# sml2004/CUDA-powered-mesh-handling-and-Iterative-solvers

Measured on AMD Instinct MI355X. Metric: CG iterations/sec + DOFs/sec (assembly+solve), 10M P1-tet Poisson, 1/2/4/8 MI355X, higher is better.
Workload: dtype f64; 1 GPU; 10,110,954-tet P1 poisson Kuhn cube n=119, Jacobi-PCG fixed iterations; tets=10110954, nodes=1728000, dofs=1728000, nnz_blocks=25575838, parallelism=single GPU

## Files before the change

### cuda-powered-mesh-handling-and-iterative-solvers_amd/_capi.py

```python
from __future__ import annotations

import atexit
import ctypes
import functools
import inspect
import os
import threading

import torch

PKG_DIR = os.path.dirname(os.path.abspath(__file__))
LIB_PATH = os.environ.get("FEM355_LIB", os.path.join(PKG_DIR, "lib", "libfem355.so"))

FEM_OK, FEM_EBADTYPE, FEM_ESINGULAR, FEM_EHIP, FEM_ERCCL, FEM_EARG, FEM_ESTATE = range(7)
(PCG_RUNNING, PCG_CONVERGED, PCG_MAXITER, PCG_BREAKDOWN, PCG_ALPHA_NAN, PCG_BETA_NAN, PCG_SYNC_TIMEOUT,
 PCG_BAD_WINDOW) = range(8)
MODE_CG_STABLE, MODE_PCG, MODE_CG_CONSTRAINED = 0, 1, 2
TUNE_UPD1 = 1024
TUNE_U2_HOLD, TUNE_U2_SMALL = 2048, 4096
TUNE_MF_GATHER = 8192
TUNE_PK_GV = 16384
TUNE_DEFAULT = 1 | 2 | 4 | 8 | 128 | TUNE_UPD1
KIND_ELASTIC, KIND_POISSON, KIND_MASS = 0, 1, 2
ISO_SUM, ISO_STACK, ISO_VOLUME, ISO_MASS = 0, 1, 2, 3
MASS_SELL, MASS_DIAG = 0, 1
MODAL_OUT_GM, MODAL_OUT_NORMS, MODAL_OUT_LEN = 576, 1152, 1168

_P = ctypes.c_void_p
_I = ctypes.c_int
_L = ctypes.c_int64
_D = ctypes.c_double

SIGNATURES = {
    "fem_last_error": (ctypes.c_char_p, []),
    "fem_version": (_I, []),
    "fem_tet4_ke": (_I, [_P, _P, _L, _D, _D, _I, _P, _P, _P]),
    "fem_tet4_geom": (_I, [_P, _P, _L, _P, _P, _P, _P, _P]),
    "fem_iso_ke": (_I, [_P, _P, _L, _I, _D, _D, _P, _P, _I, _I, _P, _P]),
    "fem_iso_geom": (_I, [_P, _P, _L, _I, _P, _P, _P, _P, _P]),
    "fem_ke_sym_stride": (_I, [_I]),
    "fem_iso_ke_sym": (_I, [_P, _P, _L, _I, _D, _D, _P, _P, _I, _I, _P, _P]),
    "fem_assemble_from_ke_sym": (_I, [_P, _P, _I, _P, _P, _L, _P, _P, _P, _I, _I, _I, _P, _P]),
    "fem_assemble_from_ke_mass_sl": (_I, [_P, _P, _P, _I, _P, _P, _L, _P, _P, _P, _I, _I, _P, _P, _P]),
    "fem_iso_mass": (_I, [_P, _P, _L, _I, _D, _P, _P, _P, _I, _P, _P]),
    "fem_iso_mass_scalar": (_I, [_P, _P, _L, _I, _D, _P, _P, _P, _I, _P, _P]),
    "fem_pcg_scalars": (_I, [_P, ctypes.POINTER(_D)]),
    "fem_scan_work_len": (_L, [_L]),
    "fem_incidence_work_bytes": (_L, [_L, _L]),
    "fem_incidence": (_I, [_P, _L, _I, _L, _P, _P, _P, _P]),
    "fem_incidence_checked": (_I, [_P, _L, _I, _L, _P, _P, _P, _P, _P]),
    "fem_rcm_work_len": (_L, [_L]),
    "fem_rcm": (_I, [_P, _P, _L, _P, _P, _P, _P, _P]),
    "fem_graph_count": (_I, [_P, _I, _P, _P, _L, _P, _P, _P]),
    "fem_graph_fill": (_I, [_P, _I, _P, _P, _L, _P, _P, _P, _P]),
    "fem_graph_tmp_len": (_L, [_L]),
    "fem_graph_count2": (_I, [_P, _I, _P, _P, _L, _P, _P, _P, _P]),
    "fem_graph_fill2": (_I, [_P, _I, _P, _P, _L, _P, _P, _P, _P, _P]),
    "fem_graph_sell_fill": (_I, [_P, _I, _P, _P, _L, _P, _P, _P, _P, _P, _P, _P, _P, _P, _P]),
    "fem_graph_sell_fill_sl": (_I, [_P, _I, _P, _P, _L, _P, _P, _P, _P, _P, _P, _P, _I, _P, _P, _P, _P, _P]),
    "fem_scan_i32": (_I, [_P, _L, _P, _P, _P]),
    "fem_scan_i64": (_I, [_P, _L, _P, _P, _P]),
    "fem_sell_widths": (_I, [_P, _L, _P, _P]),
    "fem_graph_sizes": (_I, [_P, _P, _P, _L, _P, _P, _P, _P]),
    "fem_sell_fill": (_I, [_P, _P, _L, _P, _P, _P, _P]),
    "fem_sell_csr2sell": (_I, [_P, _L, _P, _P, _P]),
    "fem_assemble_from_ke": (_I, [_P, _P, _I, _I, _P, _P, _L, _P, _P, _P, _P, _P, _P]),
    "fem_assemble_from_ke_ex": (_I, [_P, _P, _I, _I, _P, _P, _L, _P, _P, _P, _P, _L, _L, _I, _P, _P]),
    "fem_assemble_from_ke_ex2": (_I, [_P, _P, _I, _I, _P, _P, _L, _P, _P, _P, _P, _L, _L, _I, _I, _P, _P]),
    "fem_assemble_tet4": (_I, [_P, _P, _D, _D, _I, _P, _P, _L, _P, _P, _P, _P, _P, _P, _P]),
    "fem_assemble_tet4_ex": (_I, [_P, _P, _D, _D, _I, _P, _P, _L, _P, _P, _P, _P, _I, _P, _P, _P]),
    "fem_assemble_tet4_ex2": (_I, [_P, _P, _D, _D, _I, _P, _P, _L, _P, _P, _P, _P, _I, _I, _P, _P, _P]),
    "fem_sell_to_csr_vals": (_I, [_P, _I, _P, _L, _P, _P, _P, _P]),
    "fem_jacobi": (_I, [_P, _I, _P, _P, _P, _P, _L, _P, _P, _P]),
    "fem_ebe_apply": (_I, [_P, _P, _I, _I, _P, _P, _L, _P, _P, _P]),
    "fem_ebe_diag": (_I, [_P, _P, _I, _I, _P, _P, _L, _I, _P, _P]),
    "fem_invert_diag": (_I, [_P, _L, _P, _P]),
    "fem_tet4_stress": (_I, [_P, _P, _L, _P, _D, _D, _P, _P, _P, _P]),
    "fem_iso_stress": (_I, [_P, _P, _L, _I, _P, _D, _D, _P, _P, _I, _I, _P, _P, _P]),
    "fem_voigt_to_tensor": (_I, [_P, _L, _P, _P]),
    "fem_von_mises": (_I, [_P, _L, _P, _P]),
    "fem_node_average": (_I, [_P, _I, _P, _P, _L, _P, _P]),
    "fem_face_forces": (_I, [_P, _P, _L, _I, _P, _P]),
    "fem_shared_face_sum": (_I, [_P, _P, _I, _L, _P, _P]),
    "fem_topo_create": (_I, [_P, _L, _I, _P, _I, _I, _L, _P, ctypes.POINTER(_P)]),
    "fem_topo_counts": (_I, [_P, ctypes.POINTER(_L), ctypes.POINTER(_L), ctypes.POINTER(_L)]),
    "fem_topo_pairs": (_I, [_P, _P]),
    "fem_topo_unique": (_I, [_P, _P]),
    "fem_topo_boundary": (_I, [_P, _P, _I, _P, _P, _P, _P, _P, ctypes.POINTER(_L)]),
    "fem_topo_destroy": (None, [_P]),
    "fem_sub_elements": (_I, [_P, _L, _I, _P, _I, _I, _P, _P]),
    "fem_element_face_normals": (_I, [_P, _P, _L, _I, _P, _P, _P, _P, _I, _D, _I, _I, _P, _P]),
    "fem_surface_normals": (_I, [_P, _P, _P, _L, _I, _I, _P, _P]),
    "fem_solid_ke": (_I, [_I, _P, _P, _L, _D, _D, _P, _P, _I, _I, _P, _P]),
    "fem_csr_pattern": (_I, [_P, _L, _I, _I, _L, _P, _P, _P, ctypes.POINTER(_L), _P]),
    "fem_csr_fill": (_I, [_P, _P, _L, _I, _I, _L, _P, _P, _P, _P]),
    "fem_spmv_csr": (_I, [_P, _P, _P, _P, _P, _L, _P]),
    "fem_pcg_csr": (_I, [_P, _P, _P, _L, _P, _P, _P, _P, _D, _I, _D, _I, ctypes.POINTER(_I), ctypes.POINTER(_I), _P,
                         _P]),
    "fem_vtk_read": (_I, [ctypes.c_char_p, ctypes.POINTER(_P)]),
    "fem_vtk_sizes": (_I, [_P, ctypes.POINTER(_L), ctypes.POINTER(_L), ctypes.POINTER(_L), ctypes.POINTER(_L)]),
    "fem_vtk_copy": (_I, [_P, _P, _P, _P]),
    "fem_vtk_free": (None, [_P]),
    "fem_spmv": (_I, [_L, _I, _P, _P, _P, _P, _P, _P]),
    "fem_sell_delta16": (_I, [_P, _L, _P, _P, _P, _P]),
    "fem_spmv16": (_I, [_L, _I, _P, _P, _P, _P, _P, _P]),
    "fem_pcg_set_cols16": (_I, [_P, _P]),
    "fem_pcg_set_tuning": (_I, [_P, _I]),
    "fem_stream_copy": (_I, [_P, _P, _L, _I, _P]),
    "fem_stream_read": (_I, [_P, _P, _L, _I, _P]),
    "fem_pcg_create": (_I, [_L, _I, _P, _P, _P, _P, _P, _P, _I, _D, _D, _P, _L, _P, ctypes.POINTER(_P)]),
    "fem_pcg_start": (_I, [_P]),
    "fem_pcg_iterate": (_I, [_P, _I]),
    "fem_pcg_poll": (_I, [_P, ctypes.POINTER(_I), ctypes.POINTER(_I), ctypes.POINTER(_D)]),
    "fem_pcg_sync_site": (_I, [_P, ctypes.POINTER(_I)]),
    "fem_pcg_debug_window": (_I, [_P, _I, _I, _I]),
    "fem_pcg_solve": (_I, [_P, _I, _I, ctypes.POINTER(_I), ctypes.POINTER(_I), ctypes.POINTER(_D)]),
    "fem_pcg_use_graph": (_I, [_P, _I]),
    "fem_pcg_set_schedule": (_I, [_P, _I]),
    "fem_pcg_set_entries": (_I, [_P, _L]),
    "fem_pcg_get_schedule": (_I, [_P]),
    "fem_pcg_uniform_slices": (_I, [_P, _L, _L, _P, _P, _P]),
    "fem_pcg_persist_build": (_I, [_P, ctypes.POINTER(_I), ctypes.POINTER(_I), ctypes.POINTER(_I)]),
    "fem_pcg_pipelined": (_I, [_P, ctypes.POINTER(_I)]),
    "fem_sell_sl_pattern": (_I, [_L, _P, _P, _I, _P, _P, _P, _P, _P]),
    "fem_assemble_tet4_sl": (_I, [_P, _P, _D, _D, _I, _P, _P, _L, _P, _P, _P, _P, _P, _I, _I, _P, _P, _P]),
    "fem_assemble_from_ke_sl": (_I, [_P, _P, _I, _P, _P, _L, _P, _P, _P, _I, _I, _P, _P]),
    "fem_jacobi_sl": (_I, [_P, _I, _P, _P, _P, _P, _P, _L, _P, _P, _P]),
    "fem_spmv_sl": (_I, [_L, _I, _P, _P, _P, _P, _P, _P, _P, _P]),
    "fem_sell_sl_unpair": (_I, [_L, _I, _P, _P, _P, _P, _P, _P, _P, _P]),
    "fem_pcg_set_layout": (_I, [_P, _P, _P, _P, _P, _P, _I]),
    "fem_pcg_persist_profile": (_I, [_P, _I, _P, ctypes.POINTER(_I)]),
    "fem_pcg_set_constraints": (_I, [_P, _I, _L, _P, _P, _L, _P, _P, _L, _P, _P, _P, _P, _P]),
    "fem_enforce_constraints": (_I, [_P, _P, _L, _I, _L, _P, _P, _L, _P, _P, _L, _P, _P, _P, _P, _P, _P]),
    "fem_pcg_finish": (_I, [_P]),
    "fem_pcg_profile": (_I, [_P, _I, _I, ctypes.POINTER(_D), ctypes.POINTER(_I)]),
    "fem_pcg_destroy": (None, [_P]),
    "fem_pcg_release_cache": (_I, []),
    "fem_release_scratch": (_I, []),
    "fem_pcg_set_rows": (_I, [_P, _I, _I, _P, _I]),
    "fem_pcg_comm_block": (_I, [_P, ctypes.POINTER(_P), ctypes.POINTER(_L)]),
    "fem_pcg_col_window": (_I, [_P, ctypes.POINTER(_L), ctypes.POINTER(_L)]),
    "fem_pcg_set_peers": (_I, [_P, _P, _P, _P]),
    "fem_pcg_dist_debug": (_I, [_P, _I, _P, _L]),
    "fem_stream_create_cu": (_I, [_I, _I, ctypes.POINTER(_P)]),
    "fem_stream_destroy": (_I, [_P]),
    "fem_pcg_set_prof": (_I, [_P, _P]),
    "fem_ipc_handle": (_I, [_P, ctypes.c_char_p]),
    "fem_ipc_open": (_I, [ctypes.c_char_p, ctypes.POINTER(_P)]),
    "fem_ipc_close": (_I, [_P]),
    "fem_sell_diag": (_I, [_P, _I, _P, _P, _L, _P, _P]),
    "fem_jacobi_from_diag": (_I, [_P, _L, _P, _P, _P]),
    "fem_mf_create": (_I, [_P, _P, _L, _L, _I, _D, _D, ctypes.POINTER(_L), _P, ctypes.POINTER(_P)]),
    "fem_mf_destroy": (_I, [_P]),
    "fem_mf_apply": (_I, [_P, _P, _P, _P]),
    "fem_mf_diag": (_I, [_P, _P, _P]),
    "fem_mf_info": (_I, [_P, ctypes.POINTER(_L)]),
    "fem_mf_order": (_I, [_P, _P, _P, _P, _P, _P]),
    "fem_pcg_set_operator_mf": (_I, [_P, _P]),
    "fem_comm_unique_id": (_I, [ctypes.c_char_p]),
    "fem_comm_init": (_I, [_I, _I, ctypes.c_char_p, ctypes.POINTER(_P)]),
    "fem_comm_destroy": (_I, [_P]),
    "fem_allreduce_sum": (_I, [_P, _P, _L, _P]),
    "fem_halo_sum": (_I, [_P, _P, _I, _P, _L, _P, _L, _P, _P]),
    "fem_halo_pack": (_I, [_P, _I, _P, _L, _P, _P]),
    "fem_halo_unpack": (_I, [_P, _I, _P, _L, _P, _P]),
    "fem_pcg_set_dist": (_I, [_P, _I, _P, _L, _P, _P, _P]),
    "fem_pcg_set_dist_variant": (_I, [_P, _I]),
    "fem_pcg_set_p2p": (_I, [_P, _I, _I, _P, _P, _P, _P]),
    "fem_pcg_p2p_buffers": (_I, [_P, ctypes.POINTER(_P), ctypes.POINTER(_P), ctypes.POINTER(_L)]),
    "fem_p2p_deliver": (_I, [_P, _I, _P]),
    "fem_pcg_dist_phase": (_I, [_P, _I]),
    "fem_pcg_dist_buffer": (_I, [_P, _I, ctypes.POINTER(_P), ctypes.POINTER(_L)]),
    "fem_group_allreduce": (_I, [_P, _I, _L, _P]),
    "fem_spmm": (_I, [_L, _I, _I, _P, _P, _P, _P, _P, _P, _P]),
    "fem_mpcg_create": (_I, [_L, _I, _I, _I, _P, _P, _P, _P, _P, _P, _P, _I, ctypes.POINTER(_D), _D, _P, _L, _P,
                             ctypes.POINTER(_P)]),
    "fem_mpcg_solve": (_I, [_P, _I, _I, ctypes.POINTER(_I), ctypes.POINTER(_I), ctypes.POINTER(_D)]),
    "fem_mpcg_scalars": (_I, [_P, ctypes.POINTER(_D)]),
    "fem_mpcg_destroy": (None, [_P]),
    "fem_spmm_km": (_I, [_L, _I, _I, _P, _P, _P, _P, _P, _I, _P, _P, _P, _P]),
    "fem_modal_work_len": (_L, []),
    "fem_modal_gram": (_I, [_L, _I, _I, ctypes.POINTER(_P), _P, _P, _P]),
    "fem_modal_residual": (_I, [_L, _I, _P, _P, _P, _P, _P, _P, _P, _P]),
    "fem_modal_rotate": (_I, [_L, _I, _I, ctypes.POINTER(_P), _P, _P]),
    "fem_pcg_set_tol": (_I, [_P, _D]),
    "fem_sell_axpby_mass": (_I, [_L, _I, _I, _L, _P, _P, _P, _P, _P, _I, _D, _D, _P, _P]),
    "fem_newmark_rhs": (_I, [_L, _I, _I, _P, _P, _P, _P, _P, _I, _D, _P, _P, _P, _P]),
    "fem_newmark_update": (_I, [_L, ctypes.POINTER(_D), _I, _P, _P, _P, _P, _P, _P, _P]),
    "fem_transient_work_len": (_L, []),
    "fem_quadform_km": (_I, [_L, _I, _I, _P, _P, _P, _P, _P, _I, _P, _P, _P, _P]),
}

_lib = None
_lock = threading.Lock()


class FemError(RuntimeError):
    pass


def load_library(path: str = LIB_PATH):
    global _lib
    with _lock:
        if _lib is None:
            if not os.path.exists(path):
                raise FemError(f"fem355: HIP library not built: {path} (run `python -c 'import __graft_entry__ as g; g.build()'`)")
            lib = ctypes.CDLL(path)
            for name, (res, args) in SIGNATURES.items():
                fn = getattr(lib, name)
                fn.restype = res
                fn.argtypes = args
            _lib = lib
    return _lib


def lib():
    if not torch.cuda.is_available():
        raise FemError("fem355 requires a HIP (MI355X) device; none is visible. There is no CPU fallback.")
    return load_library()


def check(rc: int, what: str = ""):
    if rc == FEM_OK:
        return
    msg = (_lib.fem_last_error() or b"").decode(errors="replace") if _lib else ""
    if rc == FEM_EBADTYPE:
        raise ValueError(f"{what}: {msg}")
    if rc == FEM_ESINGULAR:
        raise ValueError("Singular matrix encountered while computing B matrix.")
    raise FemError(f"fem355 {what} failed (code {rc}): {msg}")


def ptr(t):
    if t is None:
        return None
    if not t.is_cuda:
        raise FemError(f"fem355: a {t.device} tensor was passed where device memory is required")
    return ctypes.c_void_p(t.data_ptr())


def stream(dev=None):
    return ctypes.c_void_p(torch.cuda.current_stream(dev).cuda_stream)


def compute_device(device=None) -> torch.device:
    if device is not None:
        d = torch.device(device)
        if d.type == "cuda":
            return d if d.index is not None else torch.device("cuda", torch.cuda.current_device())
    return torch.device("cuda", torch.cuda.current_device())


def device_scope(dev):
    d = torch.device(dev)
    if d.type != "cuda" or d.index is None or d.index == torch.cuda.current_device():
        return _NULL_SCOPE
    return torch.cuda.device(d)


class _NullScope:
    def __enter__(self):
        return self

    def __exit__(self, *exc):
        return False


_NULL_SCOPE = _NullScope()


def on_device(fn):
    sig = inspect.signature(fn)
    if "device" not in sig.parameters:
        return fn
# ... 41 lines not shown
```

### cuda-powered-mesh-handling-and-iterative-solvers_amd/csrc/pcg.hip

```cpp
#include <rccl/rccl.h>
#include <stddef.h>

#include <atomic>
#include <mutex>
#include <vector>

#include "sell_pair.hpp"
#include "sell_pair3.hpp"
#include "matfree.hpp"

namespace fem {

template <typename T, bool NT>
__device__ __forceinline__ T ld(const T* p) {
    if constexpr (NT) return __builtin_nontemporal_load(p);
    else return *p;
}

struct VecPlain {
    const double* x;
    __device__ __forceinline__ double operator()(int64_t i) const { return x[i]; }
};
struct VecFusedP {
    const double* r;
// ... 1562 lines not shown
    };
    auto spc = [&]() {
        for (int64_t t = t0; t < c.S; t += 256) {
            x[c.spc_dof[t]] = c.spc_val[t];
            if (r) r[c.spc_dof[t]] = 0.0;
        }
        __syncthreads();
    };
    if (c.order == 0) {
        rbe2();
        spc();
    } else {
        spc();
        rbe2();
        for (int64_t g = 0; g < c.G; ++g) {
            double v = 0.0;
            for (int64_t e = c.r3_ptr[g] + t0; e < c.r3_ptr[g + 1]; e += 256) v += c.r3_w[e] * x[c.r3_slave[e]];
            v = block_sum256(v, lds4);
            if (t0 == 0) x[c.r3_master[g]] = v / (c.r3_wsum[g] + 1e-30);
            __syncthreads();
        }
    }
}

enum { CON_GATHER = 0, CON_SCATTER = 1, CON_SPC = 2 };
template <int PH>
__global__ void __launch_bounds__(256) k_con_phase(double* __restrict__ x, double* __restrict__ r, Constraints c,
                                                   const PcgState* st, int always) {
    if (!always && !st->xupd) return;
    const int64_t m = PH == CON_SPC ? c.S : c.R;
    for (int64_t t = (int64_t)blockIdx.x * 256 + threadIdx.x; t < m; t += (int64_t)gridDim.x * 256) {
        if (PH == CON_GATHER) {
            c.tmp[t] = x[c.rbe2_master[t]];
        } else if (PH == CON_SCATTER) {
            x[c.rbe2_slave[t]] = c.tmp[t];
            if (r) r[c.rbe2_slave[t]] = 0.0;
        } else {
            x[c.spc_dof[t]] = c.spc_val[t];
            if (r) r[c.spc_dof[t]] = 0.0;
        }
    }
}

__global__ void k_check_range(const int64_t* __restrict__ v, int64_t m, int64_t lo, int64_t hi, int* __restrict__ bad) {
    for (int64_t i = (int64_t)blockIdx.x * blockDim.x + threadIdx.x; i < m; i += (int64_t)gridDim.x * blockDim.x)
        if (v[i] < lo || v[i] >= hi) atomicOr(bad, 1);
}

__global__ void k_check_ptr(const int64_t* __restrict__ ptr, int64_t g, int* __restrict__ bad) {
    for (int64_t i = (int64_t)blockIdx.x * blockDim.x + threadIdx.x; i < g; i += (int64_t)gridDim.x * blockDim.x)
        if (ptr[i + 1] < ptr[i] || (i == 0 && ptr[0] != 0)) atomicOr(bad, 1);
}

__global__ void __launch_bounds__(256) k_stream_copy(const double2* __restrict__ src, double2* __restrict__ dst,
                                                     int64_t n2) {
    for (int64_t i = (int64_t)blockIdx.x * 256 + threadIdx.x; i < n2; i += (int64_t)gridDim.x * 256) dst[i] = src[i];
}

__global__ void __launch_bounds__(256) k_stream_read(const double2* __restrict__ src, int64_t n2, double* __restrict__ out) {
    double acc = 0.0;
    for (int64_t i = (int64_t)blockIdx.x * 256 + threadIdx.x; i < n2; i += (int64_t)gridDim.x * 256) {
        const double2 v = src[i];
        acc += v.x + v.y;
    }
    if (acc == 12345.678) out[0] = acc;
}

__global__ void k_zero_fixed(int64_t n, double* __restrict__ x, const double* __restrict__ w) {
    for (int64_t i = (int64_t)blockIdx.x * blockDim.x + threadIdx.x; i < n; i += (int64_t)gridDim.x * blockDim.x)
        if (w[i] == 0.0) x[i] = 0.0;
}

}

using namespace fem;

struct fem_pcg {
    int64_t nrows, nslices, n;
    int bs;
    const int64_t* slice_ptr;
    const int32_t* cols;
    const double* vals;
    const double* b;
    double* x;
    const double* w;
    double* hist;
    int64_t hist_len;
    int mode;
    double tol, eps;
    hipStream_t stream;
    int fused;
    int deferred;
    int64_t launched;
    int64_t sell_ent;
    const int16_t* cols16;
    int has_con;
    int tune;
    int paired;
    double* pvals;
    int16_t* pcols16;
    int32_t* puoff;
    int16_t* pucol;
    int pext;
    const int32_t* pwin_ext;
    int pwin_G;
    Constraints con;
    double* r;
    double* p0;
    double* p1;
    double* q;
    RedBuf red;
    PcgState* st;
    PcgState* st_host;
    int grid_spmv, grid_vec;
    hipGraphExec_t graph;
    int graph_k;
    int max_iter;
    int dist;
    ncclComm_t comm;
    int64_t nI;
    const int32_t* imap;
    const int32_t* ipos;
    const uint8_t* own;
    double* hbuf;
    int cg1;
    double* cg1_s;
    double* cg1_u;
    double* cg1_send;
    double* cg1_recv;
    int p2p;
    int p2p_nranks;
    std::vector<int> peer_rank;
    std::vector<int64_t> peer_off, peer_cnt;
    int64_t p2p_total;
    const int32_t* p2p_csrc;
    const int32_t* p2p_ssrc;
    double* psend;
    double* precv;
    int c1f;
    int c1f_grid;
    int c1f_win_ok;
    int32_t* c1f_win;
    unsigned* c1f_flags;
    int persist_req;
    int persist_fit_only;
    int persist;
    int pk_grid;
    int pk_win_ok;
    int32_t* pk_win;
    double* pk_part;
    unsigned* pk_sync;
    int pk_ovf;
    double* pk_v;
    int pk_coop;
    int pk_gv;
    double* gv_buf;
    int64_t gv_cap;
    int gv_init_pending;
    int64_t pk_epochs;
    hipEvent_t pev[2];
    int pd;
    int pd_rank, pd_nranks, pd_grid_req;
    int64_t pd_split[PK_MAX_RANKS + 1];
    char* pd_block;
    int64_t pd_block_bytes, pd_off_flag, pd_off_red, pd_off_rflag;
    int64_t pd_off_m1;
    char* pd_peer[PK_MAX_RANKS];
    int pd_peers_ok;
    int32_t* pd_pub;
    int pd_init_pending;
    unsigned long long* pd_prof;
    int upd1;
    int u2_grid;
    unsigned* u2_sync;
    fem_mf* mf;
    double* mf_sl;
    int64_t mf_sl_cap;
    int mf_nogather;
    int mf_qfuse;
};

#define FEM_NCCL(call)                                                                         \
    do {                                                                                       \
        ncclResult_t _r = (call);                                                              \
        if (_r != ncclSuccess) {                                                               \
            ::fem::set_error("%s:%d %s -> %s", __FILE__, __LINE__, #call, ncclGetErrorString(_r)); \
            return FEM_ERCCL;                                                                  \
        }                                                                                      \
    } while (0)

static const int16_t* pcols(const fem_pcg* s) { return s->bs == 1 ? s->pcols16 : s->cols16; }

static double* st_red(fem_pcg* s, int k) {
    return reinterpret_cast<double*>(reinterpret_cast<char*>(s->st) + offsetof(PcgState, red)) + k;
}

template <int BS>
__global__ void __launch_bounds__(MF_BLOCK) k_pcg_mf_dot(MfOp op, const double* __restrict__ p,
                                                         double* __restrict__ slots, PcgState* __restrict__ st,
                                                         RedBuf red) {
    __shared__ MfLds<BS> L;
    __shared__ double lds4[MF_BLOCK / 64];
    __shared__ int flag;
    if (blockIdx.x == 0 && threadIdx.x == 0) st->xupd = 0;
    if (st->halt || st->iter >= st->max_iter) return;
    double dot = mf_walk<BS, MF_DOT>(op, p, slots, L);
    dot = block_sum<MF_BLOCK>(dot, lds4);
    double pq;
    if (reduce_grid<MF_BLOCK>(dot, red.part(RED_K1), red.cnt(RED_K1), &pq, lds4, &flag) && threadIdx.x == 0)
        finish_pq(st, pq);
}

template <int BS>
__global__ void __launch_bounds__(MF_BLOCK) k_cg1_mf_slots(MfOp op, const double* __restrict__ u,
                                                           double* __restrict__ slots, const PcgState* __restrict__ st,
                                                           int always, P2PArgs xp, const double* __restrict__ recv,
                                                           const double* __restrict__ send, int64_t off) {
    __shared__ MfLds<BS> L;
    if (!always) {
        const Cg1Step k = cg1_eval(st, cg1_scalar(recv, send, off, 0, xp), cg1_scalar(recv, send, off, 1, xp));
        if (!k.go) return;
    }
    (void)mf_walk<BS, MF_APPLY>(op, u, slots, L);
}

template <int BS>
__global__ void __launch_bounds__(MF_BLOCK) k_cg1_mf_slots_dot(MfOp op, const double* __restrict__ u,
                                                               double* __restrict__ slots, PcgState* __restrict__ st,
                                                               int always, P2PArgs xp, const double* __restrict__ recv,
                                                               const double* __restrict__ send, int64_t off,
                                                               RedBuf red) {
    __shared__ MfLds<BS> L;
    __shared__ double lds4[MF_BLOCK / 64];
    __shared__ int flag;
    if (!always) {
        const Cg1Step k = cg1_eval(st, cg1_scalar(recv, send, off, 0, xp), cg1_scalar(recv, send, off, 1, xp));
        if (!k.go) return;
    }
    double dot = mf_walk<BS, MF_DOT>(op, u, slots, L);
    dot = block_sum<MF_BLOCK>(dot, lds4);
    double d;
    if (reduce_grid<MF_BLOCK>(dot, red.part(RED_K1), red.cnt(RED_K1), &d, lds4, &flag) && threadIdx.x == 0)
        st->red[0] = d;
}

template <int BS>
__global__ void __launch_bounds__(PCG_BLOCK) k_cg1_mf_iface(MfOp op, const double* __restrict__ slots,
                                                            const int32_t* __restrict__ imap, int64_t nI,
                                                            double* __restrict__ send, int64_t off,
                                                            PcgState* __restrict__ st, RedBuf red, int always,
                                                            P2PArgs xp, const double* __restrict__ recv, double* hist,
                                                            int64_t hist_len) {
    __shared__ double lds4[4];
    __shared__ int flag;
    Cg1Step k{};
    if (!always) {
        k = cg1_eval(st, cg1_scalar(recv, send, off, 0, xp), cg1_scalar(recv, send, off, 1, xp));
        if (!k.go) {
            if (blockIdx.x == 0 && threadIdx.x == 0) cg1_commit(st, k, hist, hist_len);
            return;
        }
    }
    for (int64_t j = (int64_t)blockIdx.x * PCG_BLOCK + threadIdx.x; j < nI; j += (int64_t)gridDim.x * PCG_BLOCK) {
        const int32_t a = imap[j];
        if (a < 0) continue;
#pragma unroll
        for (int c = 0; c < BS; ++c) {
            const double o = mf_q_dof<BS>(op, slots, (int64_t)a * BS + c);
            if (xp.P) {
                for (int q = 0; q < xp.P; ++q) {
                    const int dst = xp.csrc[j * xp.P + q];
                    if (dst >= 0) xp.psend[dst + c] = o;
                }
            } else {
                send[j * BS + c] = o;
            }
        }
    }
    double unused;
    if (reduce_grid(0.0, red.part(RED_INIT), red.cnt(RED_INIT), &unused, lds4, &flag) && threadIdx.x == 0) {
        if (!always) cg1_commit(st, k, hist, hist_len);
        const double d = st->red[0];
        send[off] = st->red[1];
        send[off + 1] = d;
        for (int q = 0; q < xp.P; ++q) {
            const int dst = xp.ssrc[q];
            if (dst >= 0) {
                xp.psend[dst] = st->red[1];
                xp.psend[dst + 1] = d;
            }
        }
    }
}

template <int BS>
__global__ void __launch_bounds__(PCG_BLOCK) k_cg1_mf_gather(MfOp op, const double* __restrict__ slots,
                                                             const double* __restrict__ u, double* __restrict__ v,
                                                             const int32_t* __restrict__ ipos, double* __restrict__ send,
                                                             int64_t off, PcgState* __restrict__ st, RedBuf red,
                                                             int always, P2PArgs xp, const double* __restrict__ recv,
                                                             double* hist, int64_t hist_len) {
    __shared__ double lds4[4];
    __shared__ int flag;
    Cg1Step k{};
    if (!always) {
        k = cg1_eval(st, cg1_scalar(recv, send, off, 0, xp), cg1_scalar(recv, send, off, 1, xp));
// ... 804 lines not shown
    }
    FEM_LAUNCHED();
    return FEM_OK;
}

static int make_constraints(const char* fn, int64_t n, hipStream_t stream, int order, int64_t R,
                            const int64_t* rbe2_slave, const int64_t* rbe2_master, int64_t S, const int64_t* spc_dof,
                            const double* spc_val, int64_t G, const int64_t* r3_ptr, const int64_t* r3_master,
                            const double* r3_wsum, const int64_t* r3_slave, const double* r3_w, Constraints* c) {
    if (R < 0 || S < 0 || G < 0 || (R && (!rbe2_slave || !rbe2_master)) || (S && (!spc_dof || !spc_val)) ||
        (G && (!r3_ptr || !r3_master || !r3_wsum)) || (order != 0 && order != 1) || (order == 0 && G)) {
        set_error("%s: bad sizes / pointers / order", fn);
        return FEM_EARG;
    }
    int* bad = nullptr;
    FEM_HIP(::fem::malloc_async((void**)&bad, sizeof(int) * 2, stream));
    FEM_HIP(hipMemsetAsync(bad, 0, sizeof(int) * 2, stream));
    auto chk = [&](const int64_t* v, int64_t m) {
        if (m > 0)
            hipLaunchKernelGGL(k_check_range, dim3(stream_grid(m, 256)), dim3(256), 0, stream, v, m, (int64_t)0, n, bad);
    };
    chk(rbe2_slave, R);
    chk(rbe2_master, R);
    chk(spc_dof, S);
    chk(r3_master, G);
    int64_t E = 0;
    if (G) {
        hipLaunchKernelGGL(k_check_ptr, dim3(stream_grid(G, 256)), dim3(256), 0, stream, r3_ptr, G, bad + 1);
        FEM_HIP(hipMemcpyAsync(&E, r3_ptr + G, sizeof(int64_t), hipMemcpyDeviceToHost, stream));
    }
    int hbad[2] = {0, 0};
    FEM_HIP(hipMemcpyAsync(hbad, bad, sizeof(hbad), hipMemcpyDeviceToHost, stream));
    FEM_HIP(hipStreamSynchronize(stream));
    if (!hbad[1] && E > 0) {
        if (!r3_slave || !r3_w) hbad[1] = 1;
        else {
            chk(r3_slave, E);
            FEM_HIP(hipMemcpyAsync(hbad, bad, sizeof(int), hipMemcpyDeviceToHost, stream));
            FEM_HIP(hipStreamSynchronize(stream));
        }
    }
    FEM_HIP(hipFreeAsync(bad, stream));
    if (hbad[0] || hbad[1]) {
        set_error("%s: %s", fn, hbad[0] ? "a constraint dof is outside [0, n)" : "RBE3 group pointer is not a CSR offset array");
        return FEM_EARG;
    }
    *c = Constraints{};
    c->R = R;
    c->S = S;
    c->G = G;
    c->rbe2_slave = rbe2_slave;
    c->rbe2_master = rbe2_master;
    c->spc_dof = spc_dof;
    c->spc_val = spc_val;
    c->r3_ptr = r3_ptr;
    c->r3_master = r3_master;
    c->r3_wsum = r3_wsum;
    c->r3_slave = r3_slave;
    c->r3_w = r3_w;
    c->order = order;
    return FEM_OK;
}

int fem_pcg_set_constraints(fem_pcg* s, int order, int64_t R, const int64_t* rbe2_slave, const int64_t* rbe2_master,
                            int64_t S, const int64_t* spc_dof, const double* spc_val, int64_t G, const int64_t* r3_ptr,
                            const int64_t* r3_master, const double* r3_wsum, const int64_t* r3_slave,
                            const double* r3_w) {
    if (s->mode != FEM_MODE_CG_CONSTRAINED || s->dist || s->fused || s->deferred || s->graph || s->mf) {
        set_error("fem_pcg_set_constraints: needs a CG_CONSTRAINED, single-GPU, 3-kernel context without a graph "
                  "over an assembled matrix");
        return FEM_EARG;
    }
    Constraints c;
    const int rc = make_constraints("fem_pcg_set_constraints", s->n, s->stream, order, R, rbe2_slave, rbe2_master, S,
                                    spc_dof, spc_val, G, r3_ptr, r3_master, r3_wsum, r3_slave, r3_w, &c);
    if (rc != FEM_OK) return rc;
    if (s->con.tmp) (void)hipFree(s->con.tmp);
    s->con.tmp = nullptr;
    if (R > 0) FEM_HIP(hipMalloc(&c.tmp, sizeof(double) * (size_t)R));
    s->con = c;
    s->has_con = 1;
    return FEM_OK;
}

int fem_enforce_constraints(double* x, double* r, int64_t n, int order, int64_t R, const int64_t* rbe2_slave,
                            const int64_t* rbe2_master, int64_t S, const int64_t* spc_dof, const double* spc_val,
                            int64_t G, const int64_t* r3_ptr, const int64_t* r3_master, const double* r3_wsum,
                            const int64_t* r3_slave, const double* r3_w, fem_stream_t stream) {
    if (!x || n < 0) {
        set_error("fem_enforce_constraints: null x / negative n");
        return FEM_EARG;
    }
    const hipStream_t st = reinterpret_cast<hipStream_t>(stream);
    Constraints c;
    const int rc = make_constraints("fem_enforce_constraints", n, st, order, R, rbe2_slave, rbe2_master, S, spc_dof,
                                    spc_val, G, r3_ptr, r3_master, r3_wsum, r3_slave, r3_w, &c);
    if (rc != FEM_OK) return rc;
    if (R > 0) FEM_HIP(::fem::malloc_async((void**)&c.tmp, sizeof(double) * (size_t)R, st));
    const int lrc = launch_constraints(st, x, r, c, nullptr, 1);
    if (lrc != FEM_OK) return lrc;
    if (c.tmp) FEM_HIP(hipFreeAsync(c.tmp, st));
    return FEM_OK;
}

int fem_pcg_set_tuning(fem_pcg* s, int flags) {
    if (s->graph) {
        set_error("fem_pcg_set_tuning: drop the captured graph first");
        return FEM_EARG;
    }
    s->tune = flags;
    return FEM_OK;
}

int fem_pcg_set_cols16(fem_pcg* s, const int16_t* dcols) {
    if (s->graph) {
        set_error("fem_pcg_set_cols16: drop the captured graph first");
        return FEM_EARG;
    }
    s->cols16 = dcols;
    if (!dcols) s->paired = 0;
    return FEM_OK;
}

int fem_stream_copy(const double* src, double* dst, int64_t n, int grid, fem_stream_t stream) {
    if (grid <= 0) grid = 2048;
    hipLaunchKernelGGL(k_stream_copy, dim3(grid), dim3(256), 0, S(stream), (const double2*)src, (double2*)dst, n / 2);
    FEM_LAUNCHED();
    return FEM_OK;
}

int fem_stream_read(const double* src, double* out, int64_t n, int grid, fem_stream_t stream) {
    if (grid <= 0) grid = 4096;
    hipLaunchKernelGGL(k_stream_read, dim3(grid), dim3(256), 0, S(stream), (const double2*)src, n / 2, out);
    FEM_LAUNCHED();
    return FEM_OK;
}

int fem_pcg_create(int64_t nrows, int bs, const int64_t* slice_ptr, const int32_t* cols, const double* vals,
                   const double* b, double* x, const double* w, int mode, double tol, double eps, double* hist,
                   int64_t hist_len, fem_stream_t stream, fem_pcg** out) {
    if (bs != 1 && bs != 3) {
        set_error("fem_pcg_create: block size %d unsupported", bs);
        return FEM_EARG;
    }
    if (mode != FEM_MODE_CG_STABLE && mode != FEM_MODE_PCG && mode != FEM_MODE_CG_CONSTRAINED) {
        set_error("fem_pcg_create: unknown mode %d", mode);
        return FEM_EARG;
    }
    if (((uintptr_t)b | (uintptr_t)x | (uintptr_t)w) & 15) {
        set_error("fem_pcg_create: vectors must be 16-byte aligned");
        return FEM_EARG;
    }
    fem_pcg* s = new fem_pcg();
    s->tune = FEM_TUNE_REVERSE | FEM_TUNE_PAIR | FEM_TUNE_PK_SC1 | FEM_TUNE_PK_PACK | FEM_TUNE_PK_UNI | FEM_TUNE_UPD1;
    s->nrows = nrows;
    s->bs = bs;
    s->nslices = cdiv(nrows, 64);
    s->n = nrows * bs;
    s->sell_ent = -1;
    s->slice_ptr = slice_ptr;
    s->cols = cols;
    s->vals = vals;
    s->b = b;
    s->x = x;
    s->w = w;
    s->hist = hist;
    s->hist_len = hist ? hist_len : 0;
    s->mode = mode;
    s->tol = tol;
    s->eps = eps;
    s->stream = S(stream);
    s->fused = 0;
    s->graph = nullptr;
    s->graph_k = 0;
    s->max_iter = 0x7fffffff;
    s->grid_spmv = grid_multiple_of_xcd(cdiv(s->nslices, 4), 2048);
    s->grid_vec = grid_multiple_of_xcd(cdiv(s->n / 2 + 1, PCG_BLOCK), 1024);
    size_t vec = sizeof(double) * (size_t)(s->n + 2);
    hipError_t e = hipSuccess;
    if (e == hipSuccess) e = pool_alloc((void**)&s->r, vec, s->stream, s->bs == 1);
    if (e == hipSuccess) e = pool_alloc((void**)&s->p0, vec, s->stream, s->bs == 1);
    if (e == hipSuccess) e = pool_alloc((void**)&s->p1, vec, s->stream, s->bs == 1);
    if (e == hipSuccess) e = pool_alloc((void**)&s->q, vec, s->stream, s->bs == 1);
    if (e == hipSuccess)
        e = pool_alloc((void**)&s->red.partials, sizeof(double) * RED_N * MAX_PARTIALS, s->stream, s->bs == 1);
    if (e == hipSuccess)
        e = pool_alloc((void**)&s->red.counters, sizeof(unsigned) * RED_N * RED_COUNTER_WORDS, s->stream, s->bs == 1);
    if (e == hipSuccess) e = hipMemsetAsync(s->red.counters, 0, sizeof(unsigned) * RED_N * RED_COUNTER_WORDS, s->stream);
    if (e == hipSuccess) e = pool_alloc((void**)&s->st, sizeof(PcgState), s->stream, s->bs == 1);
    if (e == hipSuccess) e = host_state_alloc((void**)&s->st_host, sizeof(PcgState));
    if (e != hipSuccess) {
        set_error("fem_pcg_create: allocation failed: %s", hipGetErrorString(e));
        fem_pcg_destroy(s);
        return FEM_EHIP;
    }
    *out = s;
    return FEM_OK;
}

int fem_pcg_set_operator_mf(fem_pcg* s, fem_mf* m) {
    if (!s || !m || mf_bs(m) != s->bs || mf_nodes(m) != s->nrows) {
        set_error("fem_pcg_set_operator_mf: the operator's block size / node count do not match the context");
        return FEM_EARG;
    }
    if (s->pd || s->has_con || s->graph || s->mode == FEM_MODE_CG_CONSTRAINED) {
        set_error("fem_pcg_set_operator_mf: contexts without constraints (CG_STABLE / PCG mode), the row-partitioned "
                  "schedule or a captured graph only");
        return FEM_EARG;
    }
    if (s->dist && !s->cg1) {
        set_error("fem_pcg_set_operator_mf: a distributed context runs the element-chunk operator in the "
                  "single-reduction variant only (fem_pcg_set_dist_variant(s, 1))");
        return FEM_EARG;
    }
    const int64_t need = (int64_t)mf_bs(m) * (int64_t)mf_nslots(m);
    if (need > s->mf_sl_cap) {
        if (s->mf_sl) FEM_HIP(hipFree(s->mf_sl));
        s->mf_sl = nullptr;
        s->mf_sl_cap = 0;
        FEM_HIP(hipMalloc(&s->mf_sl, sizeof(double) * (size_t)need));
        s->mf_sl_cap = need;
    }
    s->mf = m;
    {
        const char* e = getenv("FEM355_MF_NOGATHER");
        s->mf_nogather = e ? (atoi(e) != 0) : (int)(mf_nodes(m) >= MF_NOGATHER_MIN_NODES);
    }
    s->fused = s->deferred = s->persist_req = s->persist_fit_only = s->persist = 0;
    s->cols16 = nullptr;
    s->pext = 0;
    return FEM_OK;
}

int fem_pcg_set_entries(fem_pcg* s, int64_t entries) {
    if (entries < 0) {
        set_error("fem_pcg_set_entries: negative entry count %lld", (long long)entries);
        return FEM_EARG;
    }
    s->sell_ent = entries;
    return FEM_OK;
}

int fem_pcg_set_tol(fem_pcg* s, double tol) {
    if (!s || !(tol >= 0.0)) {
        set_error("fem_pcg_set_tol: needs a context and a tolerance >= 0");
        return FEM_EARG;
    }
    s->tol = tol;
    return FEM_OK;
}

int fem_pcg_set_schedule(fem_pcg* s, int sched) {
    if (s->graph) {
        set_error("fem_pcg_set_schedule: drop the captured graph first (fem_pcg_use_graph(s, 0))");
        return FEM_EARG;
    }
    if (sched < 0 || sched > 4) {
        set_error("fem_pcg_set_schedule: unknown schedule %d", sched);
        return FEM_EARG;
    }
    if (s->mf) {
        if (sched != 0 && sched != 4) {
            set_error("fem_pcg_set_schedule: the element-chunk operator runs the 3-kernel schedule");
            return FEM_EARG;
        }
        s->fused = s->deferred = s->persist_req = s->persist_fit_only = s->persist = 0;
        return FEM_OK;
    }
    const bool auto3 = sched == 4 && s->bs == 3;
    if (sched == 4) sched = (s->dist || s->mode == FEM_MODE_CG_CONSTRAINED) ? 0 : 3;
    if (sched != 0 && s->dist) {
        set_error("fem_pcg_set_schedule: the distributed path runs the 3-kernel schedule");
        return FEM_EARG;
    }
    if (sched != 0 && s->mode == FEM_MODE_CG_CONSTRAINED) {
        set_error("fem_pcg_set_schedule: the constrained CG runs the 3-kernel schedule (projection after K3)");
        return FEM_EARG;
    }
    s->fused = sched == 1;
    s->deferred = (sched == 2 || sched == 3) && !auto3;
    s->persist_req = sched == 3;
    s->persist_fit_only = auto3 ? 1 : 0;
    s->persist = 0;
    return FEM_OK;
}

int fem_pcg_persist_profile(fem_pcg* s, int k, unsigned long long* host_out, int* grid) {
    if (!s->persist || s->pk_ovf || k <= 0) {
        set_error("fem_pcg_persist_profile: the context does not run the (register-resident) persistent schedule");
        return FEM_EARG;
    }
    const size_t nb = sizeof(unsigned long long) * (size_t)s->pk_grid * (PK_NPROF + PK_WAVES);
    unsigned long long* d = nullptr;
    FEM_HIP(hipMalloc(&d, nb));
    FEM_HIP(hipMemsetAsync(d, 0, nb, s->stream));
    int rc = launch_persist(s, k, d);
    if (!rc) {
        const hipError_t e1 = hipMemcpyAsync(host_out, d, nb, hipMemcpyDeviceToHost, s->stream);
        const hipError_t e2 = hipStreamSynchronize(s->stream);
        if (e1 != hipSuccess || e2 != hipSuccess) {
            set_error("fem_pcg_persist_profile: %s", hipGetErrorString(e1 != hipSuccess ? e1 : e2));
            rc = FEM_EHIP;
        }
    }
    (void)hipFree(d);
    if (grid) *grid = s->pk_grid;
    return rc;
}

int fem_pcg_get_schedule(fem_pcg* s) {
    if (s->persist) return 3;
    if (s->fused) return 1;
    return s->deferred ? 2 : 0;
}

__global__ void k_sell_sl_pattern(int64_t nslices, int64_t nrows, const int64_t* __restrict__ slice_ptr,
                                  const int16_t* __restrict__ cin, int16_t* __restrict__ pout,
                                  int16_t* __restrict__ ucol, int32_t* __restrict__ uoff, int G, int* __restrict__ win,
                                  int2* __restrict__ span);

int fem_sell_sl_pattern(int64_t nrows, const int64_t* slice_ptr, const int16_t* dcols, int G, int16_t* pcols,
                        int16_t* ucol, int32_t* uoff, int32_t* win, fem_stream_t stream) {
    const int64_t ns = cdiv(nrows, 64);
    if (ns <= 0) return FEM_OK;
    hipStream_t st = S(stream);
    int2* span = nullptr;
    if (G > 0) FEM_HIP(::fem::stream_scratch((void**)&span, sizeof(int2) * (size_t)ns, st));
    hipLaunchKernelGGL(k_sell_sl_pattern, dim3((unsigned)cdiv(ns, 4)), dim3(256), 0, st, ns, nrows, slice_ptr,
                       dcols, pcols, ucol, uoff, G > 0 ? G : 0, win, span);
    FEM_LAUNCHED();
    if (G > 0) {
        hipLaunchKernelGGL(k_win_from_spans, dim3((unsigned)cdiv((int64_t)G * 64, 256)), dim3(256), 0, st, G, ns,
                           (const int2*)span, win);
        FEM_LAUNCHED();
    }
    return FEM_OK;
}

int fem_sell_sl_unpair(int64_t nrows, int bs, const int64_t* slice_ptr, const int16_t* dcols, const int32_t* uoff,
                       const int16_t* ucol, const int32_t* rowptr, const double* svals, double* vals,
                       fem_stream_t stream) {
    const int64_t ns = cdiv(nrows, 64);
    if (ns <= 0) return FEM_OK;
    if (bs == 3) {
        hipLaunchKernelGGL(k_sell3_from_a, dim3(stream_grid(ns * 64, 256)), dim3(256), 0, S(stream), ns, slice_ptr,
                           svals, vals);
        FEM_LAUNCHED();
        return FEM_OK;
    }
    hipLaunchKernelGGL(k_sell_sl_unpair, dim3(stream_grid(ns * 64, 256)), dim3(256), 0, S(stream), ns, slice_ptr, dcols,
                       uoff, ucol, rowptr, nrows, svals, vals);
    FEM_LAUNCHED();
    return FEM_OK;
}

int fem_spmv_sl(int64_t nrows, int bs, const int64_t* slice_ptr, const int16_t* pcols, const double* svals,
                const int32_t* uoff, const int16_t* ucol, const double* x, double* y, fem_stream_t stream) {
    const int64_t ns = cdiv(nrows, 64);
    if (ns <= 0) return FEM_OK;
    if (bs == 3) {
        hipLaunchKernelGGL(k_spmv_a, dim3(grid_multiple_of_xcd(cdiv(ns, 4), 2048)), dim3(256), 0, S(stream), ns, nrows,
                           slice_ptr, pcols, svals, x, y);
        FEM_LAUNCHED();
        return FEM_OK;
    }
    hipLaunchKernelGGL(k_spmv_pair<SPMV_UP>, dim3(grid_multiple_of_xcd(cdiv(ns, 4), 2048)), dim3(256), 0, S(stream), ns, nrows,
                       slice_ptr, pcols, svals, uoff, ucol, x, y);
    FEM_LAUNCHED();
    return FEM_OK;
}

int fem_pcg_set_layout(fem_pcg* s, const double* svals, const int16_t* pcols, const int32_t* uoff,
                       const int16_t* ucol, const int32_t* win, int G) {
    if ((s->bs != 1 && s->bs != 3) || !s->cols16 || s->dist || s->pd || (s->bs == 1 && !pcols)) {
        set_error("fem_pcg_set_layout: single-GPU contexts with 16-bit columns only (fem_pcg_set_cols16 first); "
                  "bs = 1 needs the paired columns");
        return FEM_EARG;
    }
    if (!s->pext) {
        pool_free(s->pvals, s->stream);
        pool_free(s->pcols16, s->stream);
        pool_free(s->puoff, s->stream);
        pool_free(s->pucol, s->stream);
    }
    s->pext = 1;
    s->pvals = const_cast<double*>(svals);
    s->pcols16 = s->bs == 1 ? const_cast<int16_t*>(pcols) : nullptr;
    s->puoff = s->bs == 1 ? const_cast<int32_t*>(uoff) : nullptr;
    s->pucol = s->bs == 1 ? const_cast<int16_t*>(ucol) : nullptr;
    s->pwin_ext = win;
    s->pwin_G = win ? G : 0;
    s->pk_win_ok = 0;
    return FEM_OK;
}

int fem_pcg_uniform_slices(fem_pcg* s, int64_t s_begin, int64_t s_end, int64_t* uniform, int64_t* nslices,
                           int64_t* index_bytes) {
    if (s_end < 0 || s_end > s->nslices) s_end = s->nslices;
    if (s_begin < 0) s_begin = 0;
    if (s_begin > s_end) s_begin = s_end;
    *uniform = 0;
    *nslices = s_end - s_begin;
    *index_bytes = 0;
    if (s->nslices == 0) return FEM_OK;
    std::vector<int64_t> sp((size_t)s->nslices + 1);
    std::vector<int32_t> h((size_t)s->nslices, -1);
    FEM_HIP(hipMemcpyAsync(sp.data(), s->slice_ptr, sizeof(int64_t) * sp.size(), hipMemcpyDeviceToHost, s->stream));
    const bool uni = s->paired && s->puoff && (s->tune & FEM_TUNE_PK_UNI) && s->bs == 1;
    if (uni) FEM_HIP(hipMemcpyAsync(h.data(), s->puoff, sizeof(int32_t) * h.size(), hipMemcpyDeviceToHost, s->stream));
    FEM_HIP(hipStreamSynchronize(s->stream));
    const int64_t idx = s->cols16 ? 2 : 4;
    int64_t c = 0, ib = 0;
    for (int64_t i = s_begin; i < s_end; ++i) {
        const int64_t wdt = (sp[i + 1] - sp[i]) / 64;
        if (h[i] >= 0) {
            ++c;
            ib += 2 * ((wdt + 1) & ~int64_t(1));
        } else {
            ib += idx * 64 * wdt;
        }
    }
    *uniform = c;
    *index_bytes = ib;
    return FEM_OK;
}

static size_t pk_sync_words(int G) { return (size_t)(18 + G) * PK_LINE; }

constexpr int PK_MAXS_DIST = 4;
static const void* persist_fn_dist(bool prof, int maxs) {
    if (!prof && maxs <= 1) return (const void*)k_pcg_persist<1, false, true, false, true>;
    if (!prof && maxs == 2) return (const void*)k_pcg_persist<2, false, true, false, true>;
    if (maxs <= PK_MAXS_DIST)
        return prof ? (const void*)k_pcg_persist<PK_MAXS_DIST, true, true, false, true>
                    : (const void*)k_pcg_persist<PK_MAXS_DIST, false, true, false, true>;
    return prof ? (const void*)k_pcg_persist<PK_MAXS, true, true, false, true>
                : (const void*)k_pcg_persist<PK_MAXS, false, true, false, true>;
}
static int dist_maxs(const fem_pcg* s) {
    const int64_t nloc = s->pd_split[s->pd_rank + 1] - s->pd_split[s->pd_rank];
    const int64_t maxL = (nloc + s->pk_grid - 1) / s->pk_grid;
    return (int)((maxL + PK_WAVES - 1) / PK_WAVES);
}

static const void* persist_fn(bool prof, bool gsc1, bool ovf = false, int small = 0) {
    if (small >= 1 && small <= 4 && !prof && !ovf && gsc1)
        return small == 1 ? (const void*)k_pcg_persist<1, false, true>
             : small == 2 ? (const void*)k_pcg_persist<2, false, true>
                          : (const void*)k_pcg_persist<4, false, true>;
    if (ovf) return gsc1 ? (const void*)k_pcg_persist<PK_MAXS, false, true, true>
                         : (const void*)k_pcg_persist<PK_MAXS, false, false, true>;
    if (prof) return gsc1 ? (const void*)k_pcg_persist<PK_MAXS, true, true> : (const void*)k_pcg_persist<PK_MAXS, true, false>;
    return gsc1 ? (const void*)k_pcg_persist<PK_MAXS, false, true> : (const void*)k_pcg_persist<PK_MAXS, false, false>;
}

static const void* persist3_fn(bool ovf, bool dist) {
    if (dist) return (const void*)k_pcg_persist3<P3_MAXS, false, true>;
    return ovf ? (const void*)k_pcg_persist3<P3_MAXS, true> : (const void*)k_pcg_persist3<P3_MAXS, false>;
}
static size_t persist_lds(const fem_pcg* s) { return s->bs == 3 ? P3_LDS : PK_LDS; }
static int persist_maxs(const fem_pcg* s) { return s->bs == 3 ? P3_MAXS : PK_MAXS; }

static int persist_setup_dist(fem_pcg* s);

static int persist_setup(fem_pcg* s) {
    s->persist = 0;
    if (s->pd) return persist_setup_dist(s);
    if (!s->persist_req) return FEM_OK;
    if ((s->bs != 1 && s->bs != 3) || !s->paired || s->dist || s->mode == FEM_MODE_CG_CONSTRAINED || s->nslices == 0)
        return FEM_OK;
    int dev = 0, ncu = 0;
    FEM_HIP(hipGetDevice(&dev));
    FEM_HIP(hipDeviceGetAttribute(&ncu, hipDeviceAttributeMultiprocessorCount, dev));
    const int G = (ncu / NXCD) * NXCD;
    if (G < NXCD) return FEM_OK;
    const bool ovf = s->nslices > (int64_t)G * PK_WAVES * persist_maxs(s);
    if (ovf && (!(s->tune & FEM_TUNE_PK_PACK) || s->persist_fit_only)) return FEM_OK;
    static std::mutex occ_mu;
    static int occ_cache[2][64] = {};
    int occ;
    {
        std::lock_guard<std::mutex> lk(occ_mu);
        int& slot = occ_cache[s->bs == 3][dev & 63];
        if (slot == 0) {
            int res = 1;
            for (int v = 0; v < (s->bs == 3 ? 2 : 9) && res == 1; ++v) {
                const void* f = s->bs == 3 ? persist3_fn(v == 1, false)
                              : v >= 6 ? persist_fn(false, true, false, v == 8 ? 4 : v - 5)
                                       : persist_fn((v & 1) && v < 4, v & 2, v >= 4);
                FEM_HIP(hipFuncSetAttribute(f, hipFuncAttributeMaxDynamicSharedMemorySize, (int)persist_lds(s)));
                int nb = 0;
                FEM_HIP(hipOccupancyMaxActiveBlocksPerMultiprocessor(&nb, f, PK_T, persist_lds(s)));
                if (nb < 1) res = 2;
            }
            slot = res;
        }
        occ = slot;
    }
    if (occ != 1) return FEM_OK;
    if (s->pk_grid != G) {
        pool_free(s->pk_win, s->stream);
        pool_free(s->pk_part, s->stream);
        pool_free(s->pk_sync, s->stream);
        s->pk_win = nullptr;
        s->pk_part = nullptr;
        s->pk_sync = nullptr;
        FEM_HIP(pool_alloc((void**)&s->pk_win, sizeof(int32_t) * 2 * G, s->stream, s->bs == 1));
        FEM_HIP(pool_alloc((void**)&s->pk_part, sizeof(double) * 4 * G, s->stream, s->bs == 1));
        FEM_HIP(pool_alloc((void**)&s->pk_sync, sizeof(unsigned) * pk_sync_words(G), s->stream, s->bs == 1));
        s->pk_grid = G;
        s->pk_win_ok = 0;
    }
    if (!s->pk_win_ok && s->pwin_ext && s->pwin_G == G) {
        FEM_HIP(hipMemcpyAsync(s->pk_win, s->pwin_ext, sizeof(int32_t) * 2 * G, hipMemcpyDeviceToDevice, s->stream));
        s->pk_win_ok = 1;
    }
    if (!s->pk_win_ok) {
        hipLaunchKernelGGL(k_pk_window_init, dim3(cdiv(G, 256)), dim3(256), 0, s->stream, G, G, s->pk_win);
        FEM_LAUNCHED();
        hipLaunchKernelGGL(k_pk_window, dim3(stream_grid(s->nslices * 64, 256)), dim3(256), 0, s->stream, s->nslices,
                           s->nrows, s->slice_ptr, s->cols16, G, s->pk_win, s->pk_win + G);
        FEM_LAUNCHED();
        s->pk_win_ok = 1;
    }
    if (ovf && !s->pk_v) FEM_HIP(pool_alloc((void**)&s->pk_v, sizeof(double) * (size_t)s->n, s->stream, s->bs == 1));
    s->pk_ovf = ovf ? 1 : 0;
    s->persist = 1;
    s->pk_gv = 0;
    if ((s->tune & FEM_TUNE_PK_GV) && (s->tune & FEM_TUNE_PK_SC1) && s->bs == 1 && !ovf && s->mode == FEM_MODE_PCG) {
        const int64_t maxL = (s->nslices + G - 1) / G;
        const int pack = (int)((maxL + PK_WAVES - 1) / PK_WAVES);
        if (pack <= GV_MAXS) {
            static std::mutex gv_mu;
            static int gv_ok[64] = {};
            std::lock_guard<std::mutex> lk(gv_mu);
            int& slot = gv_ok[dev & 63];
            if (slot == 0) {
                int res = 1;
                for (int v = 0; v < 2 && res == 1; ++v) {
                    const void* f = v ? (const void*)k_pcg_persist_gv<2> : (const void*)k_pcg_persist_gv<1>;
                    FEM_HIP(hipFuncSetAttribute(f, hipFuncAttributeMaxDynamicSharedMemorySize, (int)GV_LDS));
                    int nb = 0;
                    FEM_HIP(hipOccupancyMaxActiveBlocksPerMultiprocessor(&nb, f, PK_T, GV_LDS));
                    if (nb < 1) res = 2;
                }
                slot = res;
            }
            s->pk_gv = slot == 1;
        }
    }
    return FEM_OK;
}

static int persist_setup_dist(fem_pcg* s) {
    if ((s->bs != 1 && s->bs != 3) || !s->paired || s->dist || s->mode == FEM_MODE_CG_CONSTRAINED) {
        set_error("distributed persistent PCG: needs bs = 1 or 3, 16-bit columns with the paired copy, no element "
                  "partition, no constraints");
        return FEM_EARG;
    }
    if (!s->pd_peers_ok) {
        set_error("distributed persistent PCG: fem_pcg_set_peers first");
        return FEM_EARG;
    }
    const int G = s->pk_grid;
    const int64_t nloc = s->pd_split[s->pd_rank + 1] - s->pd_split[s->pd_rank];
    if ((nloc + G - 1) / G > (int64_t)PK_WAVES * persist_maxs(s)) {
        set_error("distributed persistent PCG: %lld slices on this rank exceed the register capacity of %d workgroups",
                  (long long)nloc, G);
        return FEM_EARG;
    }
    for (int v = 0; v < (s->bs == 3 ? 1 : 2); ++v) {
        const void* f = s->bs == 3 ? persist3_fn(false, true) : persist_fn_dist(v == 1, dist_maxs(s));
        FEM_HIP(hipFuncSetAttribute(f, hipFuncAttributeMaxDynamicSharedMemorySize, (int)persist_lds(s)));
        int nb = 0;
        FEM_HIP(hipOccupancyMaxActiveBlocksPerMultiprocessor(&nb, f, PK_T, persist_lds(s)));
        if (nb < 1) {
            set_error("distributed persistent PCG: kernel does not fit one workgroup per CU");
            return FEM_EARG;
        }
    }
    s->pk_ovf = 0;
    s->persist = 1;
    s->pk_gv = 0;
    if (s->pd_off_m1 > 0 && s->mode == FEM_MODE_PCG && dist_maxs(s) <= GV_MAXS) {
        int res = 1;
        for (int v = 0; v < 2 && res == 1; ++v) {
            const void* f = v ? (const void*)k_pcg_persist_gv<2, true> : (const void*)k_pcg_persist_gv<1, true>;
            FEM_HIP(hipFuncSetAttribute(f, hipFuncAttributeMaxDynamicSharedMemorySize, (int)GV_LDS));
            int nb = 0;
            FEM_HIP(hipOccupancyMaxActiveBlocksPerMultiprocessor(&nb, f, PK_T, GV_LDS));
            if (nb < 1) res = 2;
        }
        s->pk_gv = res == 1;
    }
    return FEM_OK;
}

static int persist_reset_sync(fem_pcg* s) {
    FEM_HIP(hipMemsetAsync(s->pk_sync, 0, sizeof(unsigned) * pk_sync_words(s->pk_grid), s->stream));
    FEM_HIP(hipMemsetAsync(&s->st->pk_epoch, 0, sizeof(unsigned), s->stream));
    s->pk_epochs = 0;
    return FEM_OK;
}

static int launch_persist(fem_pcg* s, int k, unsigned long long* prof) {
    const int G = s->pk_grid;
    if (s->pk_epochs + k + 1 > (int64_t(1) << 24)) {
        if (s->pd) {
            set_error("distributed persistent PCG: 2^24 iterations since fem_pcg_start; restart the solve");
            return FEM_EARG;
        }
        const int rc = persist_reset_sync(s);
        if (rc) return rc;
    }
    s->pk_epochs += k + 1;
    PkArgs a;
    a.nslices = s->nslices;
    a.nrows = s->nrows;
    a.slice_ptr = s->slice_ptr;
    a.cols = s->pcols16;
    a.vals = s->pvals;
    const bool uni = (s->tune & FEM_TUNE_PK_UNI) && s->puoff;
    a.uoff = uni ? s->puoff : nullptr;
    a.ucol = uni ? s->pucol : nullptr;
    a.x = s->x;
    a.r = s->r;
    a.p = s->p0;
    a.s = s->p1;
    a.u = s->q;
    a.w = s->w;
    a.win = s->pk_win;
    a.part = s->pk_part;
    a.sync = s->pk_sync;
    a.st = s->st;
    a.hist = s->hist;
    a.hist_len = s->hist_len;
    a.kmax = k;
    a.rev = (s->tune & FEM_TUNE_REVERSE) ? 1 : 0;
    a.prof = prof;
    a.v = s->pk_ovf ? s->pk_v : nullptr;
    {
        const int64_t maxL = (s->nslices + G - 1) / G;
        a.pack = (s->tune & FEM_TUNE_PK_PACK) ? (int)((maxL + PK_WAVES - 1) / PK_WAVES) : 0;
    }
    a.sbase = 0;
    a.rank = 0;
    a.nranks = 1;
    for (int q = 0; q < PK_MAX_RANKS; ++q) a.peer[q] = nullptr;
    a.off_flag = a.off_red = a.off_rflag = 0;
    a.pub = nullptr;
    a.b = s->b;
    a.init = 0;
    if (s->pd) {
        const int64_t S0 = s->pd_split[s->pd_rank], S1 = s->pd_split[s->pd_rank + 1];
        a.nslices = S1 - S0;
        a.sbase = S0;
        a.rank = s->pd_rank;
        a.nranks = s->pd_nranks;
        for (int q = 0; q < s->pd_nranks; ++q) a.peer[q] = s->pd_peer[q];
        a.off_flag = s->pd_off_flag;
        a.off_red = s->pd_off_red;
        a.off_rflag = s->pd_off_rflag;
        a.pub = s->pd_pub;
        a.u = reinterpret_cast<double*>(s->pd_block);
        a.init = s->pd_init_pending;
        s->pd_init_pending = 0;
        const int64_t maxL = (a.nslices + G - 1) / G;
        a.pack = (int)((maxL + PK_WAVES - 1) / PK_WAVES);
    }
    if (s->pk_gv && s->bs == 1) {
        if (prof) {
            set_error("persistent PCG: no instrumented (PROF) build of the pipelined iteration");
            return FEM_EARG;
        }
        if (!s->pd) {
            const int64_t maxL = (s->nslices + G - 1) / G;
            a.pack = (int)((maxL + PK_WAVES - 1) / PK_WAVES);
        }
        const int64_t n = s->n;
        GvArgs g;
        g.u = s->gv_buf;
        g.w = s->gv_buf + n;
        g.q = s->gv_buf + 2 * n;
        g.z = s->gv_buf + 3 * n;
        if (s->pd) {
            g.m[0] = reinterpret_cast<double*>(s->pd_block);
            g.m[1] = reinterpret_cast<double*>(s->pd_block + s->pd_off_m1);
            g.moff[0] = 0;
            g.moff[1] = s->pd_off_m1;
            g.init = 0;
        } else {
            g.m[0] = s->gv_buf + 4 * n;
            g.m[1] = s->gv_buf + 5 * n;
            g.moff[0] = g.moff[1] = 0;
            g.init = s->gv_init_pending;
            s->gv_init_pending = 0;
        }
        s->pk_epochs += 2;
        void* gargs[] = {&a, &g};
        const void* gfn = s->pd ? (a.pack <= 1 ? (const void*)k_pcg_persist_gv<1, true> : (const void*)k_pcg_persist_gv<2, true>)
                                : (a.pack <= 1 ? (const void*)k_pcg_persist_gv<1> : (const void*)k_pcg_persist_gv<2>);
        if (s->pk_coop || (s->tune & FEM_TUNE_PK_COOP))
            FEM_HIP(hipLaunchCooperativeKernel(gfn, dim3(G), dim3(PK_T), gargs, GV_LDS, s->stream));
        else
            FEM_HIP(hipLaunchKernel(gfn, dim3(G), dim3(PK_T), gargs, GV_LDS, s->stream));
        FEM_LAUNCHED();
        s->launched += k;
        return FEM_OK;
    }
    void* args[] = {&a};
    if (s->pd && !prof && s->pd_prof) a.prof = prof = s->pd_prof;
    if (s->bs == 3) {
        if (prof && !s->pd) {
            set_error("persistent PCG: no instrumented (PROF) build for bs = 3");
            return FEM_EARG;
        }
        a.cols = s->cols16;
        a.uoff = nullptr;
        a.ucol = nullptr;
        a.prof = nullptr;
        if (!s->pd) {
            const int64_t maxL = (s->nslices + G - 1) / G;
            a.pack = (int)((maxL + PK_WAVES - 1) / PK_WAVES);
        }
    }
    const void* fn = s->bs == 3 ? persist3_fn(s->pk_ovf != 0, s->pd != 0)
                   : s->pd ? persist_fn_dist(prof != nullptr, a.pack)
                           : persist_fn(prof != nullptr && !s->pk_ovf, (s->tune & FEM_TUNE_PK_SC1) != 0, s->pk_ovf != 0,
                                        (a.pack <= 4 && !(s->tune & FEM_TUNE_PK_WIDE)) ? a.pack : 0);
    if (s->pk_coop || (s->tune & FEM_TUNE_PK_COOP))
        FEM_HIP(hipLaunchCooperativeKernel(fn, dim3(G), dim3(PK_T), args, persist_lds(s), s->stream));
    else
        FEM_HIP(hipLaunchKernel(fn, dim3(G), dim3(PK_T), args, persist_lds(s), s->stream));
    FEM_LAUNCHED();
    s->launched += k;
    return FEM_OK;
}

int fem_pcg_pipelined(fem_pcg* s, int* on) {
    *on = (s && s->persist && s->pk_gv) ? 1 : 0;
    return FEM_OK;
}

int fem_pcg_persist_build(fem_pcg* s, int* slots, int* overflow, int* pack) {
    *slots = 0;
    *overflow = 0;
    *pack = 0;
    if (!s->persist || s->pk_grid <= 0) return FEM_OK;
    const int G = s->pk_grid;
    int64_t ns = s->nslices;
    if (s->pd) ns = s->pd_split[s->pd_rank + 1] - s->pd_split[s->pd_rank];
    const int64_t maxL = (ns + G - 1) / G;
    const int pk = (int)((maxL + PK_WAVES - 1) / PK_WAVES);
    *overflow = s->pk_ovf;
    *pack = (s->bs == 3 || s->pd || (s->tune & FEM_TUNE_PK_PACK)) ? pk : 0;
    if (s->bs == 3) {
        *slots = P3_MAXS;
    } else if (s->pd) {
        *slots = pk <= 1 ? 1 : pk == 2 ? 2 : pk <= PK_MAXS_DIST ? PK_MAXS_DIST : PK_MAXS;
    } else {
        const int small = (*pack <= 4 && !(s->tune & FEM_TUNE_PK_WIDE)) ? *pack : 0;
        *slots = (small >= 1 && small <= 4 && !s->pk_ovf && (s->tune & FEM_TUNE_PK_SC1))
                     ? (small == 1 ? 1 : small == 2 ? 2 : 4) : PK_MAXS;
    }
    return FEM_OK;
}

__global__ void __launch_bounds__(256) k_sell_sl_pattern(int64_t nslices, int64_t nrows,
                                                         const int64_t* __restrict__ slice_ptr,
                                                         const int16_t* __restrict__ cin, int16_t* __restrict__ pout,
                                                         int16_t* __restrict__ ucol, int32_t* __restrict__ uoff, int G,
                                                         int* __restrict__ win, int2* __restrict__ span) {
    __shared__ int cand_all[4][SU_MAXW];
    const int64_t s = ((int64_t)blockIdx.x * blockDim.x + threadIdx.x) >> 6;
    if (s >= nslices) return;
    const int l = threadIdx.x & 63;
    const int64_t p0 = slice_ptr[s];
    sl_pattern_slice(s, l, nslices, nrows, slice_ptr, [&](int k) { return (int)cin[p0 + 64 * k + l]; }, pout, ucol,
                     uoff, G, win, cand_all[(threadIdx.x >> 6) & 3], span);
}

static PcgState state_view(const fem_pcg* s) {
    PcgState h = *s->st_host;
    if (s->deferred && !s->dist && !s->persist) {
        const PcgState::Bank& b = h.bank[s->launched & 1];
        h.iter = b.iter;
        h.status = b.status;
        h.halt = b.halt;
        h.stop_iter = b.stop_iter;
        h.rz = b.rz;
        h.rz_new = b.rz_new;
        h.pq = b.pq;
        h.alpha = b.alpha;
        h.beta = b.beta;
    }
    return h;
}

static int refresh_pairing(fem_pcg* s) {
    const bool want = (s->bs == 1 || s->bs == 3) && s->cols16 && (s->tune & FEM_TUNE_PAIR) && !s->fused;
    s->paired = 0;
    if (s->pext) {
        if (!want) {
            set_error("PCG: a solver-layout matrix needs the paired schedules (FEM_TUNE_PAIR, 16-bit columns, not fused)");
            return FEM_EARG;
        }
        s->paired = 1;
        return FEM_OK;
    }
    if (!want || s->nslices == 0) return FEM_OK;
    int64_t ent = s->sell_ent;
    if (ent < 0) {
        FEM_HIP(hipMemcpyAsync(&ent, s->slice_ptr + s->nslices, sizeof(int64_t), hipMemcpyDeviceToHost, s->stream));
        FEM_HIP(hipStreamSynchronize(s->stream));
    }
    if (s->bs == 3) {
        if (!s->pvals) FEM_HIP(pool_alloc((void**)&s->pvals, sizeof(double) * 9 * (size_t)ent, s->stream, s->bs == 1));
        s->pcols16 = nullptr;
        hipLaunchKernelGGL(k_sell3_to_a, dim3(stream_grid(s->nslices * 64, 256)), dim3(256), 0, s->stream, s->nslices,
                           s->slice_ptr, s->vals, s->pvals);
        FEM_LAUNCHED();
        s->paired = 1;
        return FEM_OK;
    }
    if (!s->pvals) {
        FEM_HIP(pool_alloc((void**)&s->pvals, sizeof(double) * (size_t)ent, s->stream, s->bs == 1));
        FEM_HIP(pool_alloc((void**)&s->pcols16, sizeof(int16_t) * (size_t)ent, s->stream, s->bs == 1));
    }
    s->paired = 1;
    if ((s->tune & FEM_TUNE_PK_UNI) && 2 * (ent / 64) + 2 < (int64_t)INT32_MAX) {
        if (!s->puoff) {
            FEM_HIP(pool_alloc((void**)&s->puoff, sizeof(int32_t) * (size_t)s->nslices, s->stream, true));
            FEM_HIP(pool_alloc((void**)&s->pucol, sizeof(int16_t) * (size_t)(2 * (ent / 64) + 2), s->stream, true));
        }
        hipLaunchKernelGGL(k_sell_uniform, dim3((unsigned)cdiv(s->nslices, 4)), dim3(256), 0, s->stream, s->nslices,
                           s->nrows, s->slice_ptr, s->vals, s->cols16, s->pvals, s->pcols16, s->pucol, s->puoff, 1);
        FEM_LAUNCHED();
        return FEM_OK;
    }
    hipLaunchKernelGGL(k_sell_pair, dim3(stream_grid(s->nslices * 64, 256)), dim3(256), 0, s->stream, s->nslices,
                       s->slice_ptr, s->vals, s->cols16, s->pvals, s->pcols16);
    FEM_LAUNCHED();
    return FEM_OK;
}

int fem_pcg_start(fem_pcg* s) {
    if (s->mf && s->dist && !s->cg1) {
        set_error("fem_pcg_start: a distributed element-chunk context needs the single-reduction variant "
                  "(fem_pcg_set_dist_variant(s, 1))");
        return FEM_EARG;
    }
    {
        int prc = refresh_pairing(s);
        if (!prc) prc = persist_setup(s);
        if (!prc) prc = c1f_setup(s);
        if (!prc) prc = u2_setup(s);
        if (prc) return prc;
    }
    PcgState h{};
    h.tol = s->tol;
    h.eps = s->eps;
    h.mode = s->mode;
    h.max_iter = s->max_iter;
    h.x_done = 1;
    h.dist = s->dist;
    *s->st_host = h;
    FEM_HIP(hipMemcpyAsync(s->st, s->st_host, sizeof(PcgState), hipMemcpyHostToDevice, s->stream));
    int rc;
    if (s->dist) {
        if (!s->comm) return FEM_OK;
        if (s->cg1) {
            if ((rc = dist_phase(s, 10)) || (rc = dist_exchange(s, 10)) || (rc = dist_phase(s, 20)) ||
                (rc = dist_exchange(s, 20)))
                return rc;
            return FEM_OK;
        }
        if ((rc = dist_phase(s, 10)) || (rc = dist_exchange(s, 10)) || (rc = dist_phase(s, 11)) ||
            (rc = dist_exchange(s, 11)) || (rc = dist_phase(s, 12)))
            return rc;
        return FEM_OK;
    }
    if (s->mode == FEM_MODE_CG_STABLE) {
// ... 621 lines not shown
            set_error("fem_pcg_set_peers: no comm block for rank %d", q);
            return FEM_EARG;
        }
    }
    const int64_t S0 = s->pd_split[r], nloc = s->pd_split[r + 1] - S0;
    auto owner = [&](int64_t row) {
        const int64_t sl = row >> 6;
        int q = 0;
        while (q + 1 < N && s->pd_split[q + 1] <= sl) ++q;
        const int64_t S = s->pd_split[q + 1] - s->pd_split[q], tl = sl - s->pd_split[q];
        const int64_t L = ((tl + 1) * G - 1) / S;
        return (int64_t)q * G + (L < G ? L : G - 1);
    };
    std::vector<int32_t> pub((size_t)G * N * 2, -1);
    for (int q = 0; q < N && !(s->tune & FEM_TUNE_DIST_DROP); ++q) {
        if (q == r || need_hi[q] < need_lo[q]) continue;
        const int64_t glo = owner(need_lo[q]), ghi = owner(need_hi[q]);
        for (int L = 0; L < G; ++L) {
            const int64_t Lg = (int64_t)r * G + L;
            if (Lg < glo || Lg > ghi) continue;
            const int64_t rlo = (S0 + (int64_t)L * nloc / G) * 64;
            const int64_t rhi = std::min<int64_t>((S0 + (int64_t)(L + 1) * nloc / G) * 64, s->nrows);
            const int64_t lo = std::max<int64_t>(rlo, need_lo[q]), hi = std::min<int64_t>(rhi, need_hi[q] + 1);
            pub[((size_t)L * N + q) * 2] = (int32_t)std::max<int64_t>(lo, 0);
            pub[((size_t)L * N + q) * 2 + 1] = (int32_t)std::max<int64_t>(hi, std::max<int64_t>(lo, 0));
        }
    }
    if (!s->pd_pub) FEM_HIP(hipMalloc((void**)&s->pd_pub, sizeof(int32_t) * pub.size()));
    FEM_HIP(hipMemcpyAsync(s->pd_pub, pub.data(), sizeof(int32_t) * pub.size(), hipMemcpyHostToDevice, s->stream));
    FEM_HIP(hipStreamSynchronize(s->stream));
    s->pd_peers_ok = 1;
    return FEM_OK;
}

int fem_pcg_dist_debug(fem_pcg* s, int which, int32_t* host_out, int64_t n) {
    if (!s->pd) {
        set_error("fem_pcg_dist_debug: not a distributed persistent context");
        return FEM_EARG;
    }
    const int G = s->pk_grid, N = s->pd_nranks;
    if (which == 0) {
        FEM_HIP(hipMemcpyAsync(host_out, s->pk_win, sizeof(int32_t) * std::min<int64_t>(n, 2 * G + 2),
                               hipMemcpyDeviceToHost, s->stream));
    } else if (which == 1) {
        for (int64_t i = 0; i < std::min<int64_t>(n, (int64_t)N * G); ++i)
            FEM_HIP(hipMemcpyAsync(host_out + i, s->pd_block + s->pd_off_flag + i * sizeof(unsigned) * PK_LINE,
                                   sizeof(int32_t), hipMemcpyDeviceToHost, s->stream));
    } else if (which == 2) {
        FEM_HIP(hipMemcpyAsync(host_out, s->pd_pub, sizeof(int32_t) * std::min<int64_t>(n, (int64_t)G * N * 2),
                               hipMemcpyDeviceToHost, s->stream));
    } else if (which == 3) {
        for (int64_t i = 0; i < std::min<int64_t>(n, (int64_t)N * NXCD); ++i)
            FEM_HIP(hipMemcpyAsync(host_out + i, s->pd_block + s->pd_off_rflag + i * sizeof(unsigned) * PK_LINE,
                                   sizeof(int32_t), hipMemcpyDeviceToHost, s->stream));
    } else if (which == 4) {
        for (int64_t i = 0; i < std::min<int64_t>(n, 18); ++i)
            FEM_HIP(hipMemcpyAsync(host_out + i, s->pk_sync + i * PK_LINE, sizeof(int32_t), hipMemcpyDeviceToHost,
                                   s->stream));
    }
    FEM_HIP(hipStreamSynchronize(s->stream));
    return FEM_OK;
}

int fem_stream_create_cu(int part, int nparts, void** stream) {
    int dev = 0, ncu = 0;
    FEM_HIP(hipGetDevice(&dev));
    FEM_HIP(hipDeviceGetAttribute(&ncu, hipDeviceAttributeMultiprocessorCount, dev));
    if (nparts < 1 || part < 0 || part >= nparts) {
        set_error("fem_stream_create_cu: part %d of %d", part, nparts);
        return FEM_EARG;
    }
    std::vector<uint32_t> mask((size_t)(ncu + 31) / 32, 0u);
    for (int cu = 0; cu < ncu; ++cu)
        if (cu % nparts == part) mask[(size_t)cu / 32] |= 1u << (cu % 32);
    hipStream_t st = nullptr;
    FEM_HIP(hipExtStreamCreateWithCUMask(&st, (uint32_t)mask.size(), mask.data()));
    *stream = st;
    return FEM_OK;
}

int fem_stream_destroy(void* stream) {
    FEM_HIP(hipStreamDestroy(reinterpret_cast<hipStream_t>(stream)));
    return FEM_OK;
}

int fem_pcg_set_prof(fem_pcg* s, unsigned long long* dev_buf) {
    if (!s->pd) {
        set_error("fem_pcg_set_prof: distributed persistent contexts only (single GPU: fem_pcg_persist_profile)");
        return FEM_EARG;
    }
    s->pd_prof = dev_buf;
    return FEM_OK;
}

int fem_ipc_handle(void* ptr, char* out64) {
    hipIpcMemHandle_t h;
    FEM_HIP(hipIpcGetMemHandle(&h, ptr));
    static_assert(sizeof(h) <= 64, "IPC handle size");
    memset(out64, 0, 64);
    memcpy(out64, &h, sizeof h);
    return FEM_OK;
}

int fem_ipc_open(const char* h64, void** ptr) {
    hipIpcMemHandle_t h;
    memcpy(&h, h64, sizeof h);
    FEM_HIP(hipIpcOpenMemHandle(ptr, h, hipIpcMemLazyEnablePeerAccess));
    return FEM_OK;
}

int fem_ipc_close(void* ptr) {
    FEM_HIP(hipIpcCloseMemHandle(ptr));
    return FEM_OK;
}

void fem_pcg_destroy(fem_pcg* s) {
    if (!s) return;
    if (s->pev[0]) (void)hipEventDestroy(s->pev[0]);
    if (s->pd_block) (void)hipFree(s->pd_block);
    if (s->pd_pub) (void)hipFree(s->pd_pub);
    if (s->pev[1]) (void)hipEventDestroy(s->pev[1]);
    if (s->graph) (void)hipGraphExecDestroy(s->graph);
    pool_free(s->r, s->stream);
    pool_free(s->p0, s->stream);
    pool_free(s->p1, s->stream);
    pool_free(s->q, s->stream);
    pool_free(s->red.partials, s->stream);
    pool_free(s->red.counters, s->stream);
    if (s->hbuf) (void)hipFree(s->hbuf);
    if (s->cg1_s) (void)hipFree(s->cg1_s);
    if (s->cg1_u) (void)hipFree(s->cg1_u);
    if (s->cg1_send) (void)hipFree(s->cg1_send);
    if (s->cg1_recv) (void)hipFree(s->cg1_recv);
    if (s->psend) (void)hipFree(s->psend);
    if (s->precv) (void)hipFree(s->precv);
    if (s->c1f_win) (void)hipFree(s->c1f_win);
    if (s->c1f_flags) (void)hipFree(s->c1f_flags);
    if (s->con.tmp) (void)hipFree(s->con.tmp);
    if (s->mf_sl) (void)hipFree(s->mf_sl);
    if (s->pext) {
        s->pvals = nullptr;
        s->pcols16 = nullptr;
        s->puoff = nullptr;
        s->pucol = nullptr;
    }
    pool_free(s->pvals, s->stream);
    pool_free(s->pcols16, s->stream);
    pool_free(s->puoff, s->stream);
    pool_free(s->pucol, s->stream);
    pool_free(s->pk_win, s->stream);
    pool_free(s->pk_part, s->stream);
    pool_free(s->pk_sync, s->stream);
    pool_free(s->pk_v, s->stream);
    pool_free(s->gv_buf, s->stream);
    pool_free(s->u2_sync, s->stream);
    pool_free(s->st, s->stream);
    host_state_free(s->st_host, s->stream);
    delete s;
}

}
```

### cuda-powered-mesh-handling-and-iterative-solvers_amd/csrc/pcg_persist.hpp

```cpp
#pragma once
#include "sell_pair.hpp"

namespace fem {

constexpr int PK_MAXS = 7;
constexpr int PK_U = 2;
template <int MAXS, bool PROF>
constexpr int pk_u() { return MAXS <= 1 ? 8 : (MAXS <= 4 && !PROF) ? 4 : PK_U; }
constexpr int PK_LINE = 32;
enum { PK_GRP = 0, PK_TOP = 8 * PK_LINE, PK_GEN = 9 * PK_LINE, PK_TMO = 17 * PK_LINE, PK_UFLAG = 18 * PK_LINE };
constexpr uint64_t PK_WAIT_TICKS = 200000000ull;
constexpr uint64_t PK_RANK_WAIT_TICKS = 500000000ull;
__device__ __forceinline__ uint64_t pk_now() { return __builtin_amdgcn_s_memrealtime(); }
__device__ __forceinline__ bool pk_expired(uint64_t t0, uint64_t ticks) { return pk_now() - t0 > ticks; }
constexpr int PK_NPROF = 8;
constexpr size_t PK_LDS_HEAD = 256;
constexpr int PK_VL = 5;
constexpr size_t PK_LDS = PK_LDS_HEAD + sizeof(double) * (2 * PK_MAXS + PK_VL) * PK_WAVES * 64;
static_assert(PK_LDS <= 160 * 1024, "persistent PCG: LDS over the 160 KB of a CU");

template <class T>
__device__ __forceinline__ T* pk_launder(T* p) {
    __attribute__((address_space(1))) T* q = (__attribute__((address_space(1))) T*)p;
    asm volatile("" : "+s"(q));
    return (T*)q;
}

__device__ __forceinline__ unsigned pk_ld(const unsigned* p) {
    return __hip_atomic_load(p, __ATOMIC_RELAXED, __HIP_MEMORY_SCOPE_AGENT);
}
__device__ __forceinline__ void pk_st(unsigned* p, unsigned v) {
    __hip_atomic_store(p, v, __ATOMIC_RELAXED, __HIP_MEMORY_SCOPE_AGENT);
}

__device__ __forceinline__ bool pk_wait_ge(const unsigned* p, unsigned target, unsigned* tmo) {
    const uint64_t t0 = pk_now();
    for (unsigned spins = 0;; ++spins) {
        if (pk_ld(p) >= target) return true;
        if ((spins & 63) == 63 && pk_ld(tmo)) return false;
        if ((spins & 63) == 63 && pk_expired(t0, PK_WAIT_TICKS)) {
            pk_st(tmo, 1u + 16u * (target / NXCD));
            return false;
        }
        __builtin_amdgcn_s_sleep(2);
    }
}

__device__ __forceinline__ double pk_sum(const double* part, int n) {
    const int lane = threadIdx.x & 63;
    double v = 0.0;
    for (int i = lane; i < n; i += 64) v += __hip_atomic_load(part + i, __ATOMIC_RELAXED, __HIP_MEMORY_SCOPE_AGENT);
    return wave_sum(v);
}

__device__ __forceinline__ bool pk_barrier(unsigned* sy, int grp, unsigned nper, unsigned e, int* lds_ok,
                                           const double* pd, const double* pg, int G, double* out,
                                           bool entry_sync = true) {
    if (entry_sync) __syncthreads();
    if (threadIdx.x < 64) {
        int okv = 0;
        if (threadIdx.x == 0) {
            asm volatile("s_waitcnt vmcnt(0)" ::: "memory");
            unsigned* tmo = sy + PK_TMO;
            bool ok;
            const unsigned old = __hip_atomic_fetch_add(sy + PK_GRP + grp * PK_LINE, 1u, __ATOMIC_RELAXED,
                                                        __HIP_MEMORY_SCOPE_AGENT);
            if (old == e * nper - 1)
                for (int r = 0; r < NXCD; ++r)
                    __hip_atomic_fetch_add(sy + PK_GEN + r * PK_LINE, 1u, __ATOMIC_RELAXED, __HIP_MEMORY_SCOPE_AGENT);
            ok = pk_wait_ge(sy + PK_GEN + grp * PK_LINE, e * NXCD, tmo);
            okv = ok ? 1 : 0;
        }
        okv = __builtin_amdgcn_readfirstlane(okv);
        if (okv && pd) {
            const int lane = threadIdx.x & 63;
            double vd = 0.0, vg = 0.0;
            if (pg) {
#pragma unroll 4
                for (int i = lane; i < G; i += 64) {
                    const double a = __hip_atomic_load(pd + i, __ATOMIC_RELAXED, __HIP_MEMORY_SCOPE_AGENT);
                    const double b = __hip_atomic_load(pg + i, __ATOMIC_RELAXED, __HIP_MEMORY_SCOPE_AGENT);
                    vd += a;
                    vg += b;
                }
            } else {
#pragma unroll 4
                for (int i = lane; i < G; i += 64) vd += __hip_atomic_load(pd + i, __ATOMIC_RELAXED, __HIP_MEMORY_SCOPE_AGENT);
            }
            const double d = wave_sum(vd);
            const double g = pg ? wave_sum(vg) : 0.0;
            if (threadIdx.x == 0) {
                out[0] = d;
                out[1] = g;
            }
        }
        if (threadIdx.x == 0) *lds_ok = okv;
    }
    __syncthreads();
    return *lds_ok != 0;
}

__device__ __forceinline__ double pk_block_sum(double v, double* lds16) {
    v = wave_sum(v);
    const int w = threadIdx.x >> 6;
    if ((threadIdx.x & 63) == 0) lds16[w] = v;
    __syncthreads();
    double t = 0.0;
    if (threadIdx.x == 0) {
#pragma unroll
        for (int i = 0; i < PK_WAVES; ++i) t += lds16[i];
    }
    return t;
}

constexpr int PK_MAX_RANKS = 8;

struct PkArgs {
    int64_t nslices, nrows;
    const int64_t* slice_ptr;
    const int16_t* cols;
    const double* vals;
    const int32_t* uoff;
    const int16_t* ucol;
    double* x;
    double* r;
    double* p;
    double* s;
    double* u;
    const double* w;
    const int32_t* win;
    double* part;
    unsigned* sync;
    PcgState* st;
    double* hist;
    int64_t hist_len;
    int kmax;
    int rev;
    int pack;
    double* v;
    unsigned long long* prof;
    int64_t sbase;
    int rank, nranks;
    char* peer[PK_MAX_RANKS];
    int64_t off_flag, off_red, off_rflag;
    const int32_t* pub;
    const double* b;
    int init;
};

__device__ __forceinline__ bool pk_barrier_dist(const PkArgs& a, unsigned* sy, int grp, unsigned nper, unsigned e,
                                                int* lds_ok, const double* pd, const double* pg, int G, double* out,
                                                bool entry_sync = true) {
    if (entry_sync) __syncthreads();
    if (threadIdx.x < 64) {
        const int lane = threadIdx.x;
        unsigned* tmo = sy + PK_TMO;
        int last = 0;
        if (lane == 0) {
            asm volatile("s_waitcnt vmcnt(0)" ::: "memory");
            const unsigned old = __hip_atomic_fetch_add(sy + PK_GRP + grp * PK_LINE, 1u, __ATOMIC_RELAXED,
                                                        __HIP_MEMORY_SCOPE_AGENT);
            if (old == e * nper - 1) {
                const unsigned old2 = __hip_atomic_fetch_add(sy + PK_GEN, 1u, __ATOMIC_RELAXED, __HIP_MEMORY_SCOPE_AGENT);
                last = old2 == e * NXCD - 1;
            }
        }
        last = __builtin_amdgcn_readfirstlane(last);
        const int bank = (int)(e & 1u);
        if (last) {
            double vd = 0.0, vg = 0.0;
#pragma unroll 4
            for (int i = lane; i < G; i += 64) {
                vd += __hip_atomic_load(pd + i, __ATOMIC_RELAXED, __HIP_MEMORY_SCOPE_AGENT);
                if (pg) vg += __hip_atomic_load(pg + i, __ATOMIC_RELAXED, __HIP_MEMORY_SCOPE_AGENT);
            }
            const double d = wave_sum(vd), g = wave_sum(vg);
            if (lane < a.nranks) {
                double* red = reinterpret_cast<double*>(a.peer[lane] + a.off_red) + (bank * PK_MAX_RANKS + a.rank) * 2;
                __hip_atomic_store(red, d, __ATOMIC_RELAXED, __HIP_MEMORY_SCOPE_SYSTEM);
                __hip_atomic_store(red + 1, g, __ATOMIC_RELAXED, __HIP_MEMORY_SCOPE_SYSTEM);
            }
            __builtin_amdgcn_fence(__ATOMIC_RELEASE, "");
            asm volatile("s_waitcnt vmcnt(0)" ::: "memory");
            if (lane < a.nranks * NXCD)
                __hip_atomic_store(reinterpret_cast<unsigned*>(a.peer[lane / NXCD] + a.off_rflag) +
                                       (a.rank * NXCD + lane % NXCD) * PK_LINE,
                                   e, __ATOMIC_RELAXED, __HIP_MEMORY_SCOPE_SYSTEM);
        }
        const unsigned* rf = reinterpret_cast<const unsigned*>(a.peer[a.rank] + a.off_rflag);
        int okv = 1;
        bool done = lane >= a.nranks;
        const uint64_t t0 = pk_now();
        for (unsigned spins = 0; !__all(done); ++spins) {
            if (!done)
                done = __hip_atomic_load(rf + (lane * NXCD + grp) * PK_LINE, __ATOMIC_RELAXED,
                                         __HIP_MEMORY_SCOPE_SYSTEM) >= e;
            if ((spins & 63) == 63 && pk_ld(tmo)) {
                okv = 0;
                break;
            }
            if ((spins & 63) == 63 && pk_expired(t0, PK_RANK_WAIT_TICKS)) {
                pk_st(tmo, 3u + 16u * e);
                okv = 0;
                break;
            }
            __builtin_amdgcn_s_sleep(1);
        }
        if (okv) {
            const double* red = reinterpret_cast<const double*>(a.peer[a.rank] + a.off_red) + bank * PK_MAX_RANKS * 2;
            double d = 0.0, g = 0.0;
            for (int q = 0; q < a.nranks; ++q) {
                d += __hip_atomic_load(red + 2 * q, __ATOMIC_RELAXED, __HIP_MEMORY_SCOPE_SYSTEM);
                g += __hip_atomic_load(red + 2 * q + 1, __ATOMIC_RELAXED, __HIP_MEMORY_SCOPE_SYSTEM);
            }
            if (lane == 0) {
                out[0] = d;
                out[1] = g;
            }
        }
        if (lane == 0) *lds_ok = okv;
    }
    __syncthreads();
    return *lds_ok != 0;
}

__device__ __forceinline__ void pk_publish_row(const PkArgs& a, int L, unsigned pubmask, unsigned row, double v) {
    for (int q = 0; q < a.nranks; ++q) {
        if (!(pubmask & (1u << q))) continue;
        const int32_t* pr = a.pub + (L * a.nranks + q) * 2;
        if ((int)row >= pr[0] && (int)row < pr[1])
            __hip_atomic_store(reinterpret_cast<double*>(a.peer[q]) + row, v, __ATOMIC_RELAXED,
                               __HIP_MEMORY_SCOPE_SYSTEM);
    }
}

__device__ __forceinline__ void pk_publish_flag(const PkArgs& a, int Lg, unsigned pubmask, unsigned e) {
    for (int q = 0; q < a.nranks; ++q)
        if (pubmask & (1u << q))
            __hip_atomic_store(reinterpret_cast<unsigned*>(a.peer[q] + a.off_flag) + Lg * PK_LINE, e, __ATOMIC_RELAXED,
                               __HIP_MEMORY_SCOPE_SYSTEM);
}


#define PK_ON(j) ((j) < nreg && lane < nrows - (s0 + (j)) * 64)

template <int MAXS, bool PROF, bool GSC1, bool OVF = false, bool DIST = false>
__global__ void __launch_bounds__(PK_T) k_pcg_persist(PkArgs a) {
    static_assert(!DIST || (GSC1 && !OVF), "distributed persistent PCG: sc1 gathers, no overflow build");
    unsigned long long pacc[PROF ? PK_NPROF : 1] = {};
    unsigned long long pt = 0, wspmv = 0;
    if constexpr (PROF) pt = __builtin_amdgcn_s_memtime();
#define PK_MARK(i)                                                         \
    __builtin_amdgcn_sched_barrier(0);                                     \
    if constexpr (PROF) {                                                  \
        const unsigned long long now = __builtin_amdgcn_s_memtime();       \
        pacc[i] += now - pt;                                               \
        pt = now;                                                          \
    }
    extern __shared__ __attribute__((aligned(16))) double pk_lds_raw[];
    double* lds16 = pk_lds_raw;
    int& lds_ok = *reinterpret_cast<int*>(pk_lds_raw + PK_WAVES);
    double* lds_dg = pk_lds_raw + PK_WAVES + 2;
    double* pk_lds = pk_lds_raw + PK_LDS_HEAD / sizeof(double);
    const int G = gridDim.x;
    const unsigned nper = (unsigned)(G / NXCD);
    const int L = (blockIdx.x % NXCD) * (G / NXCD) + blockIdx.x / NXCD;
    const int grp = L / (int)nper;
    const int lane = threadIdx.x & 63;
    const int wv = __builtin_amdgcn_readfirstlane(threadIdx.x >> 6);
    int s0, nsl;
    if (a.pack) {
        const int m = a.pack;
        const int sL0 = (int)((int64_t)L * a.nslices / G);
        const int nL = (int)((int64_t)(L + 1) * a.nslices / G) - sL0;
        const int lo = wv * m < nL ? wv * m : nL;
        s0 = sL0 + lo + (DIST ? (int)a.sbase : 0);
        nsl = nL - lo < m ? nL - lo : m;
    } else {
        const int64_t W = (int64_t)G * PK_WAVES;
        const int64_t gw = (int64_t)L * PK_WAVES + wv;
        s0 = (int)(gw * a.nslices / W);
        nsl = (int)((gw + 1) * a.nslices / W) - s0;
    }
    const int nreg = (OVF && nsl > MAXS) ? MAXS : nsl;
    const int nov = nsl - nreg;
    const int nrows = (int)a.nrows;
    const unsigned rb = (unsigned)s0 * 64u + (unsigned)lane;
    double* xl = pk_lds + wv * MAXS * 64 + lane;
    double* wl = pk_lds + PK_WAVES * MAXS * 64 + wv * MAXS * 64 + lane;
    double* vl = pk_lds + 2 * PK_WAVES * MAXS * 64 + wv * PK_VL * 64 + lane;
    unsigned* sy = a.sync;
    PcgState* st = a.st;
    unsigned* uf = DIST ? reinterpret_cast<unsigned*>(a.peer[a.rank] + a.off_flag) : sy + PK_UFLAG;
    const int Lg = DIST ? a.rank * G + L : L;
    const int olo = DIST ? (int)(a.sbase * 64) : 0;
    const int ohi = DIST ? (int)((a.sbase + a.nslices) * 64 < a.nrows ? (a.sbase + a.nslices) * 64 : a.nrows) : 0;
    unsigned pubmask = 0;
    bool ghost = false;
    if constexpr (DIST) {
        for (int q = 0; q < a.nranks; ++q)
            if (q != a.rank && a.pub[(L * a.nranks + q) * 2] >= 0) pubmask |= 1u << q;
        ghost = a.win[L] < a.rank * G || a.win[G + L] >= (a.rank + 1) * G;
    }

    const bool cg = st->mode != FEM_MODE_PCG;
    const double tol = st->tol, eps = st->eps;
    const int max_iter = st->max_iter;
    int it = st->iter, halt = st->halt, status = st->status, stop_iter = st->stop_iter;
    double rz = st->rz, alpha_prev = st->alpha, beta = st->beta, pq = st->pq, rz_new = st->rz_new;
    double g = st->red[1];
    unsigned ebase = st->pk_epoch;
    unsigned elast = ebase;

    double rr[MAXS], pp[MAXS], ss[MAXS], vv[MAXS], uo[MAXS];
#pragma unroll
    for (int j = 0; j < MAXS; ++j) {
        const unsigned row = rb + 64u * j;
        const bool on = PK_ON(j);
        rr[j] = on ? a.r[row] : 0.0;
        pp[j] = on ? a.p[row] : 0.0;
        ss[j] = on ? a.s[row] : 0.0;
        vv[j] = 0.0;
        xl[j * 64] = on ? a.x[row] : 0.0;
        if (j < PK_VL) vl[j * 64] = 0.0;
        const double wj = on ? a.w[row] : 0.0;
        wl[j * 64] = wj;
        uo[j] = wj * rr[j];
    }
    const int nflags = (DIST ? a.nranks : 1) * G;
    const int wraw0 = a.win[L], wraw1 = a.win[G + L];
    const int wlo = max(wraw0, 0), whi = min(wraw1, nflags - 1);
    bool fail = false;
    if (pk_window_bad(wraw0, wraw1, nflags)) {
        if (threadIdx.x == 0) pk_st(sy + PK_TMO, PK_SITE_WINDOW);
        fail = true;
    }
    bool st_loaded = !halt;
    int k = 0;
    if constexpr (DIST) {
        if (a.init && !halt) {
            const int64_t* slp = pk_launder(a.slice_ptr);
            const int16_t* cop = pk_launder(a.cols);
            const double* vap = pk_launder(a.vals);
            const double* xvp = pk_launder(a.x);
            double gp = 0.0;
#pragma unroll
            for (int j = 0; j < MAXS; ++j) {
                if (j < nreg) {
                    const double q = sell_row_pair<pk_u<MAXS, PROF>(), 0>(s0 + j, lane, slp, cop, vap, xvp, 0, 0, a.uoff, a.ucol);
                    const unsigned row = rb + 64u * j;
                    const bool on = PK_ON(j);
                    double rv = on ? a.b[row] - q : 0.0;
                    const double wj = wl[j * 64];
                    if (cg && wj == 0.0) rv = 0.0;
                    rr[j] = rv;
                    pp[j] = 0.0;
                    ss[j] = 0.0;
                    xl[j * 64] = on ? a.x[row] : 0.0;
                    const double ui = wj * rv;
                    uo[j] = ui;
                    gp += rv * ui;
                    if (on) {
                        __hip_atomic_store(a.u + row, ui, __ATOMIC_RELAXED, __HIP_MEMORY_SCOPE_AGENT);
                        if (pubmask) pk_publish_row(a, L, pubmask, row, ui);
                    }
                }
                asm volatile("" ::: "memory");
            }
            {
                const double gw = wave_sum(gp);
                if (lane == 0) lds16[wv] = gw;
            }
            asm volatile("s_waitcnt vmcnt(0)" ::: "memory");
            __syncthreads();
            const unsigned e0 = ebase + 1;
            double* pg0 = a.part + 2 * (size_t)G;
            if (threadIdx.x == 0) {
                double gsum = 0.0;
#pragma unroll
                for (int i = 0; i < PK_WAVES; ++i) gsum += lds16[i];
                __hip_atomic_store(pg0 + L, gsum, __ATOMIC_RELAXED, __HIP_MEMORY_SCOPE_AGENT);
                pk_st(uf + Lg * PK_LINE, e0);
                if (pubmask) {
                    __builtin_amdgcn_fence(__ATOMIC_RELEASE, "");
                    asm volatile("s_waitcnt vmcnt(0)" ::: "memory");
                    pk_publish_flag(a, Lg, pubmask, e0);
                }
            }
            st_loaded = true;
            if (!pk_barrier_dist(a, sy, grp, nper, e0, &lds_ok, pg0, nullptr, G, lds_dg)) {
                fail = true;
            } else {
                g = lds_dg[0];
                rz = g;
                ebase = e0;
                elast = e0;
            }
        }
    }
    if constexpr (PROF) {
        __syncthreads();
        const unsigned long long now = __builtin_amdgcn_s_memtime();
        pacc[6] += now - pt;
        pt = now;
    }
    if (!halt && !fail) {
        for (k = 0; k < a.kmax; ++k) {
            const unsigned e = ebase + (unsigned)k + 1;
            if (k > 0 || (DIST && a.init)) {
                if (wv == 0) {
                    bool ok = true;
                    for (int b0 = wlo; b0 <= whi && ok; b0 += 64) {
                        const int jw = b0 + lane;
                        bool done = jw > whi;
                        const uint64_t t0 = pk_now();
                        for (unsigned spins = 0; !__all(done); ++spins) {
                            if (!done)
                                done = (DIST ? __hip_atomic_load(uf + jw * PK_LINE, __ATOMIC_RELAXED,
                                                                 __HIP_MEMORY_SCOPE_SYSTEM)
                                             : pk_ld(uf + jw * PK_LINE)) >= e - 1;
                            if ((spins & 63) == 63 && pk_ld(sy + PK_TMO)) {
                                ok = false;
                                break;
                            }
                            if ((spins & 63) == 63 && pk_expired(t0, PK_WAIT_TICKS)) {
                                pk_st(sy + PK_TMO, 2u + 16u * e);
                                ok = false;
                                break;
                            }
                            __builtin_amdgcn_s_sleep(1);
                        }
                    }
                    if (lane == 0) {
                        lds_ok = ok;
                        if constexpr (!GSC1) __builtin_amdgcn_fence(__ATOMIC_ACQUIRE, "agent");
                        asm volatile("s_waitcnt vmcnt(0)" ::: "memory");
                    }
                }
                __syncthreads();
                if (!lds_ok) {
                    fail = true;
                    break;
                }
            }
            PK_MARK(0);
            const bool rv = a.rev && ((it & 1) != 0);
            unsigned long long tw0 = 0;
            if constexpr (PROF) tw0 = __builtin_amdgcn_s_memtime();
            const int64_t* slp = pk_launder(a.slice_ptr);
            const int16_t* cop = pk_launder(a.cols);
            const double* vap = pk_launder(a.vals);
            const double* uvp = pk_launder(a.u);
            const int32_t* uop = a.uoff ? pk_launder(a.uoff) : nullptr;
            const int16_t* ucp = a.uoff ? pk_launder(a.ucol) : nullptr;
#define PK_SPMV(MODE)                                                                              \
    if (!rv) {                                                                                     \
        _Pragma("unroll") for (int j = 0; j < MAXS; ++j) {                                         \
            if (j < nreg) {                                                                        \
                const double v = sell_row_pair<pk_u<MAXS, PROF>(), MODE>(s0 + j, lane, slp, cop, vap, uvp, olo, ohi, uop, ucp); \
                if (j < PK_VL) vl[j * 64] = v; else vv[j] = v;                                     \
            }                                                                                      \
            asm volatile("" ::: "memory");                                                         \
        }                                                                                          \
    } else {                                                                                       \
        _Pragma("unroll") for (int jj = 0; jj < MAXS; ++jj) {                                      \
            const int j = MAXS - 1 - jj;                                                           \
            if (j < nreg) {                                                                        \
                const double v = sell_row_pair<pk_u<MAXS, PROF>(), MODE>(s0 + j, lane, slp, cop, vap, uvp, olo, ohi, uop, ucp); \
                if (j < PK_VL) vl[j * 64] = v; else vv[j] = v;                                     \
            }                                                                                      \
            asm volatile("" ::: "memory");                                                         \
        }                                                                                          \
    }
            if (DIST && ghost) {
                PK_SPMV(3)
            } else {
                PK_SPMV((GSC1 ? 1 : 0))
            }
#undef PK_SPMV
            if constexpr (PROF) {
                asm volatile("s_waitcnt vmcnt(0) lgkmcnt(0)" ::: "memory");
                wspmv += __builtin_amdgcn_s_memtime() - tw0;
            }
            double dp = 0.0;
#pragma unroll
            for (int j = 0; j < MAXS; ++j) dp += uo[j] * (j < PK_VL ? vl[j * 64] : vv[j]);
            if constexpr (OVF) {
                __builtin_amdgcn_sched_barrier(0);
                for (int q = 0; q < nov; ++q) {
                    const int sq = s0 + MAXS + q;
                    const double v = sell_row_pair<pk_u<MAXS, PROF>(), GSC1>(sq, lane, slp, cop, vap, uvp, 0, 0, uop, ucp);
                    const int row = sq * 64 + lane;
                    if (row < nrows) {
                        a.v[row] = v;
                        dp += a.u[row] * v;
                    }
                }
            }
            const int bank = k & 1;
            double* pd = a.part + (size_t)bank * 2 * G;
            PK_MARK(1);
            const double dsum = pk_block_sum(dp, lds16);
            PK_MARK(2);
            if (threadIdx.x == 0) __hip_atomic_store(pd + L, dsum, __ATOMIC_RELAXED, __HIP_MEMORY_SCOPE_AGENT);
            if (!(DIST ? pk_barrier_dist(a, sy, grp, nper, e, &lds_ok, pd, k > 0 ? pd + G : nullptr, G, lds_dg, false)
                       : pk_barrier(sy, grp, nper, e, &lds_ok, pd, k > 0 ? pd + G : nullptr, G, lds_dg, false))) {
                fail = true;
                break;
            }
            elast = e;
            const double d = lds_dg[0];
            if (k > 0) g = lds_dg[1];
            PK_MARK(3);
            double bnew = 0.0;
            bool stop = false;
            if (it > 0) {
                rz_new = g;
                const double nrm = sqrt(g);
                if (L == 0 && threadIdx.x == 0 && a.hist && it - 1 < a.hist_len) a.hist[it - 1] = nrm;
                if (nrm < tol) {
                    status = FEM_PCG_CONVERGED;
                    stop_iter = it;
                    stop = true;
                } else {
                    bnew = cg ? g / (rz + eps) : g / rz;
                    if (cg && (isnan(bnew) || isinf(bnew))) {
                        status = FEM_PCG_BETA_NAN;
                        stop_iter = it;
                        stop = true;
                    }
                }
            }
            if (!stop && it >= max_iter) stop = true;
            double al = 0.0;
            if (!stop) {
                pq = (it == 0) ? d : d - bnew * g / alpha_prev;
                if (cg) {
                    if (fabs(pq) < eps || pq < 0.0) {
                        status = FEM_PCG_BREAKDOWN;
                        stop_iter = it + 1;
                        stop = true;
                    } else {
                        al = g / (pq + eps);
                        if (isnan(al) || isinf(al)) {
                            status = FEM_PCG_ALPHA_NAN;
                            stop_iter = it + 1;
                            stop = true;
                        }
                    }
                } else {
                    al = g / pq;
                }
            }
            if (stop) {
                halt = 1;
                break;
            }
            rz = g;
            alpha_prev = al;
            beta = bnew;
            it += 1;
            PK_MARK(4);
            double gp = 0.0;
            unsigned rbi = rb;
            double* ust = pk_launder(a.u);
            asm volatile("" : "+v"(rbi));
#pragma unroll
            for (int j = 0; j < MAXS; ++j) {
                if (j < nreg) {
                    const double pi = uo[j] + bnew * pp[j];
                    const double si = (j < PK_VL ? vl[j * 64] : vv[j]) + bnew * ss[j];
                    pp[j] = pi;
                    ss[j] = si;
                    xl[j * 64] += al * pi;
                    double ri = rr[j] - al * si;
                    const double wi = wl[j * 64];
                    if (cg && wi == 0.0) ri = 0.0;
                    rr[j] = ri;
                    const double ui = wi * ri;
                    uo[j] = ui;
                    if (PK_ON(j)) {
                        __hip_atomic_store(ust + (rbi + 64u * j), ui, __ATOMIC_RELAXED, __HIP_MEMORY_SCOPE_AGENT);
                        if constexpr (DIST) {
                            if (pubmask) pk_publish_row(a, L, pubmask, rbi + 64u * j, ui);
                        }
                    }
                    gp += ri * ui;
                }
            }
            if constexpr (OVF) {
                __builtin_amdgcn_sched_barrier(0);
                for (int q = 0; q < nov; ++q) {
                    const int row = (s0 + MAXS + q) * 64 + lane;
                    if (row < nrows) {
                        const double pi = a.u[row] + bnew * a.p[row];
                        const double si = a.v[row] + bnew * a.s[row];
                        a.p[row] = pi;
                        a.s[row] = si;
                        a.x[row] += al * pi;
                        double ri = a.r[row] - al * si;
                        const double wi = a.w[row];
                        if (cg && wi == 0.0) ri = 0.0;
                        a.r[row] = ri;
                        const double ui = wi * ri;
                        __hip_atomic_store(ust + row, ui, __ATOMIC_RELAXED, __HIP_MEMORY_SCOPE_AGENT);
                        gp += ri * ui;
                    }
                }
            }
            {
                const double gw = wave_sum(gp);
                if (lane == 0) lds16[wv] = gw;
            }
            asm volatile("s_waitcnt vmcnt(0)" ::: "memory");
            __syncthreads();
            if (threadIdx.x == 0) {
                double gsum = 0.0;
#pragma unroll
                for (int i = 0; i < PK_WAVES; ++i) gsum += lds16[i];
                __hip_atomic_store(a.part + (size_t)(bank ^ 1) * 2 * G + G + L, gsum, __ATOMIC_RELAXED,
                                   __HIP_MEMORY_SCOPE_AGENT);
                pk_st(uf + Lg * PK_LINE, e);
                if constexpr (DIST) {
                    if (pubmask) {
                        __builtin_amdgcn_fence(__ATOMIC_RELEASE, "");
                        asm volatile("s_waitcnt vmcnt(0)" ::: "memory");
                        pk_publish_flag(a, Lg, pubmask, e);
                    }
                }
            }
            PK_MARK(5);
        }
    }
    auto store_state = [&]() {
        if (!st_loaded) return;
#pragma unroll
        for (int j = 0; j < MAXS; ++j) {
            if (PK_ON(j)) {
                const unsigned row = rb + 64u * j;
                a.r[row] = rr[j];
                a.p[row] = pp[j];
                a.s[row] = ss[j];
                a.x[row] = xl[j * 64];
            }
        }
    };
    if (wv != 0) store_state();
    if (!fail && !halt && k == a.kmax && a.kmax > 0) {
        const unsigned e = ebase + (unsigned)a.kmax + 1;
        const double* pgl = a.part + (size_t)(a.kmax & 1) * 2 * G + G;
        const bool okb = DIST ? pk_barrier_dist(a, sy, grp, nper, e, &lds_ok, pgl, nullptr, G, lds_dg)
                              : pk_barrier(sy, grp, nper, e, &lds_ok, pgl, nullptr, G, lds_dg);
        if (!okb) {
            fail = true;
        } else {
            elast = e;
            g = lds_dg[0];
            if (it > 0) {
                const double nrm = sqrt(g);
                const bool conv = nrm < tol;
                rz_new = g;
                if (conv || it >= max_iter) {
                    if (L == 0 && threadIdx.x == 0 && a.hist && it - 1 < a.hist_len) a.hist[it - 1] = nrm;
                    if (conv) {
                        status = FEM_PCG_CONVERGED;
                        stop_iter = it;
                    }
                    halt = 1;
                }
            }
        }
    }
    if (wv == 0) store_state();
    if constexpr (PROF) {
        asm volatile("s_waitcnt vmcnt(0)" ::: "memory");
        __syncthreads();
        pacc[7] += __builtin_amdgcn_s_memtime() - pt;
        if (threadIdx.x == 0)
            for (int i = 0; i < PK_NPROF; ++i) a.prof[(size_t)L * PK_NPROF + i] = pacc[i];
        if (lane == 0) a.prof[(size_t)G * PK_NPROF + (size_t)L * PK_WAVES + wv] = wspmv;
    }
    if (L == 0 && threadIdx.x == 0) {
        if (fail) {
            stop_iter = (int)pk_ld(sy + PK_TMO);
            status = pk_fail_status((unsigned)stop_iter);
            halt = 1;
        }
        st->iter = it;
        st->halt = halt;
        st->status = status;
        st->stop_iter = stop_iter;
        st->rz = rz;
        st->rz_new = rz_new;
        st->alpha = alpha_prev;
        st->beta = beta;
        st->pq = pq;
        st->red[1] = g;
        st->pk_epoch = elast;
    }
}
#undef PK_ON
#undef PK_MARK

__global__ void k_pk_window_init(int G, int lo_empty, int* __restrict__ win) {
    const int i = blockIdx.x * blockDim.x + threadIdx.x;
    if (i < G) {
        win[i] = lo_empty;
        win[G + i] = -1;
    }
}

__global__ void k_pk_window(int64_t nslices, int64_t nrows, const int64_t* __restrict__ slice_ptr,
                            const int16_t* __restrict__ dcols, int G, int* __restrict__ lo, int* __restrict__ hi) {
    const int64_t W = (int64_t)G * PK_WAVES;
    for (int64_t t = (int64_t)blockIdx.x * blockDim.x + threadIdx.x; t < nslices * 64;
         t += (int64_t)gridDim.x * blockDim.x) {
        const int64_t s = t >> 6;
        const int l = (int)(t & 63);
        const int64_t row = s * 64 + l;
        const int64_t p0 = slice_ptr[s];
        const int w = (int)((slice_ptr[s + 1] - p0) >> 6);
        int dmin = 0, dmax = 0;
        if (row < nrows) {
#pragma unroll 8
            for (int kk = 0; kk < w; ++kk) {
                const int d = dcols[p0 + 64 * kk + l];
                dmin = d < dmin ? d : dmin;
                dmax = d > dmax ? d : dmax;
            }
        }
        int64_t cmin, cmax;
        pk_slice_span(s, nrows, dmin, dmax, &cmin, &cmax);
        auto owner = [&](int64_t r) {
            const int64_t sl = r >> 6;
            const int64_t gw = ((sl + 1) * W - 1) / nslices;
            return (int)(gw / PK_WAVES);
        };
        if (l == 0) {
            const int me = owner(row);
            atomicMin(lo + me, owner(cmin));
            atomicMax(hi + me, owner(cmax));
        }
    }
}

struct PkSplit {
    int64_t b[PK_MAX_RANKS + 1];
};
__global__ void k_pk_window_dist(int64_t sbase, int64_t nloc, int64_t nrows, const int64_t* __restrict__ slice_ptr,
                                 const int32_t* __restrict__ cols, int G, PkSplit split, int nranks,
                                 int* __restrict__ lo, int* __restrict__ hi, int* __restrict__ cwin) {
    for (int64_t t = (int64_t)blockIdx.x * blockDim.x + threadIdx.x; t < nloc * 64; t += (int64_t)gridDim.x * blockDim.x) {
        const int64_t s = sbase + (t >> 6);
        const int l = (int)(t & 63);
        const int64_t row = s * 64 + l;
        const int64_t p0 = slice_ptr[s];
        const int w = (int)((slice_ptr[s + 1] - p0) >> 6);
        int dmin = 0, dmax = 0;
        if (row < nrows)
            for (int kk = 0; kk < w; ++kk) {
                const int d = (int)(cols[p0 + 64 * kk + l] - row);
                dmin = d < dmin ? d : dmin;
                dmax = d > dmax ? d : dmax;
            }
        int64_t cmin, cmax;
        pk_slice_span(s, nrows, dmin, dmax, &cmin, &cmax);
        auto owner = [&](int64_t r) {
            const int64_t sl = r >> 6;
            int q = 0;
            while (q + 1 < nranks && split.b[q + 1] <= sl) ++q;
            const int64_t S = split.b[q + 1] - split.b[q];
            const int64_t tl = sl - split.b[q];
            const int64_t L = S > 0 ? ((tl + 1) * G - 1) / S : 0;
            return (int)(q * G + (L < G ? L : G - 1));
        };
        const int me = owner(s * 64) - (int)(owner(sbase * 64) / G) * G;
        if (l == 0) {
            atomicMin(lo + me, owner(cmin));
            atomicMax(hi + me, owner(cmax));
            atomicMin(cwin, (int)cmin);
            atomicMax(cwin + 1, (int)cmax);
        }
    }
}

}
```

### cuda-powered-mesh-handling-and-iterative-solvers_amd/csrc/sell_pair.hpp

```cpp
#pragma once
#include "common.hpp"

namespace fem {

static __global__ void k_sell_pair(int64_t nslices, const int64_t* __restrict__ slice_ptr, const double* __restrict__ vin,
                            const int16_t* __restrict__ cin, double* __restrict__ vout, int16_t* __restrict__ cout) {
    for (int64_t t = (int64_t)blockIdx.x * blockDim.x + threadIdx.x; t < nslices * 64;
         t += (int64_t)gridDim.x * blockDim.x) {
        const int64_t s = t >> 6;
        const int l = (int)(t & 63);
        const int64_t p0 = slice_ptr[s];
        const int w = (int)((slice_ptr[s + 1] - p0) >> 6);
        const int np = w >> 1;
        for (int k = 0; k < w; ++k) {
            const int64_t src = p0 + 64 * k + l;
            const int64_t dst = k < 2 * np ? p0 + (int64_t)(k >> 1) * 128 + 2 * l + (k & 1) : p0 + (int64_t)np * 128 + l;
            vout[dst] = vin[src];
            cout[dst] = cin[src];
        }
    }
}


template <int SC1>
// ... 159 lines not shown
                                                             const int64_t* __restrict__ slice_ptr,
                                                             const double* __restrict__ vin,
                                                             const int16_t* __restrict__ cin, double* __restrict__ vout,
                                                             int16_t* __restrict__ cout, int16_t* __restrict__ ucol,
                                                             int32_t* __restrict__ uoff, int pair_rest) {
    __shared__ int cand_all[4][SU_MAXW];
    const int64_t s = ((int64_t)blockIdx.x * blockDim.x + threadIdx.x) >> 6;
    const int l = threadIdx.x & 63;
    int* cand = cand_all[(threadIdx.x >> 6) & 3];
    if (s >= nslices) return;
    const int64_t p0 = slice_ptr[s];
    const int w = (int)((slice_ptr[s + 1] - p0) >> 6);
    const int64_t row = s * 64 + l;
    bool ok = (s + 1) * 64 <= nrows && w > 0 && w <= SU_MAXW;
    int len = 0;
    if (ok) {
        int prev = -(1 << 30);
        for (int k = 0; k < w; ++k) {
            const int d = cin[p0 + 64 * k + l];
            if (len == k && d > prev) {
                ++len;
                prev = d;
            } else if (d != 0 || vin[p0 + 64 * k + l] != 0.0) {
                ok = false;
            }
        }
    }
    ok = __all(ok);
    const unsigned long long full = __ballot(ok && len == w);
    if (ok && full) {
        const int c = __builtin_ctzll(full);
        for (int k = 0; k < w; ++k) {
            const int d = __shfl((int)cin[p0 + 64 * k + l], c, 64);
            if (l == 0) cand[k] = d;
            const int64_t col = row + d;
            if (col < 0 || col >= nrows) ok = false;
        }
        __builtin_amdgcn_fence(__ATOMIC_RELEASE, "wavefront");
        __builtin_amdgcn_wave_barrier();
        __builtin_amdgcn_fence(__ATOMIC_ACQUIRE, "wavefront");
        int i = 0;
        for (int k = 0; k < len && ok; ++k) {
            const int d = cin[p0 + 64 * k + l];
            while (i < w && cand[i] < d) ++i;
            if (i == w || cand[i] != d) ok = false;
            ++i;
        }
    } else {
        ok = false;
    }
    ok = __all(ok);
    const int32_t uo = (int32_t)(2 * (p0 >> 6));
    const int np = w >> 1;
    if (!ok) {
        if (l == 0) uoff[s] = -1;
        if (pair_rest) {
            for (int k = 0; k < w; ++k) {
                const int64_t src = p0 + 64 * k + l;
                const int64_t dst = k < 2 * np ? p0 + (int64_t)(k >> 1) * 128 + 2 * l + (k & 1) : p0 + (int64_t)np * 128 + l;
                vout[dst] = vin[src];
                cout[dst] = cin[src];
            }
        }
        return;
    }
    int kr = 0;
    for (int k = 0; k < w; ++k) {
        const int d = cand[k];
        double v = 0.0;
        if (kr < len && (int)cin[p0 + 64 * kr + l] == d) {
            v = vin[p0 + 64 * kr + l];
            ++kr;
        }
        const int64_t dst = k < 2 * np ? p0 + (int64_t)(k >> 1) * 128 + 2 * l + (k & 1) : p0 + (int64_t)np * 128 + l;
        vout[dst] = v;
        cout[dst] = (int16_t)d;
    }
    for (int k = l; k < w; k += 64) ucol[uo + k] = (int16_t)cand[k];
    if (l == 0) uoff[s] = uo;
}

__attribute__((unused)) static __global__ void __launch_bounds__(256) k_sell_sl_unpair(int64_t nslices,
                                                               const int64_t* __restrict__ slice_ptr,
                                                               const int16_t* __restrict__ cin,
                                                               const int32_t* __restrict__ uoff,
                                                               const int16_t* __restrict__ ucol,
                                                               const int32_t* __restrict__ rowptr, int64_t nrows,
                                                               const double* __restrict__ vin,
                                                               double* __restrict__ vout) {
    for (int64_t t = (int64_t)blockIdx.x * blockDim.x + threadIdx.x; t < nslices * 64;
         t += (int64_t)gridDim.x * blockDim.x) {
        const int64_t s = t >> 6;
        const int l = (int)(t & 63);
        const int64_t p0 = slice_ptr[s];
        const int w = (int)((slice_ptr[s + 1] - p0) >> 6);
        const int64_t row = s * 64 + l;
        const int len = row < nrows ? rowptr[row + 1] - rowptr[row] : 0;
        const int uo = uoff[s];
        int u = 0;
        for (int k = 0; k < w; ++k) {
            double v = 0.0;
            if (k < len) {
                int pos = k;
                if (uo >= 0) {
                    const int d = cin[p0 + 64 * k + l];
                    while (u < w && (int)ucol[uo + u] < d) ++u;
                    pos = u++;
                }
                v = vin[p0 + pair_pos(pos, w, l)];
            }
            vout[p0 + 64 * k + l] = v;
        }
    }
}

template <int U, int SC1, bool UNI>
__device__ __forceinline__ double sell_row_pair_body(int64_t p0, int w, int base, int lane,
                                                     const int16_t* __restrict__ cols, const int16_t* __restrict__ ucl,
                                                     const double* __restrict__ vals, const double* __restrict__ x,
                                                     int own_lo, int own_hi) {
    const int np = w >> 1;
    const double2* v2 = reinterpret_cast<const double2*>(vals + p0) + lane;
    const int32_t* c2 = UNI ? reinterpret_cast<const int32_t*>(ucl) : reinterpret_cast<const int32_t*>(cols + p0) + lane;
    double acc = 0.0;
    for (int j0 = 0; j0 < np; j0 += U) {
        int32_t cc[U];
        double2 vv[U];
        double x0[U], x1[U];
#pragma unroll
        for (int j = 0; j < U; ++j) cc[j] = (j0 + j < np) ? c2[UNI ? (j0 + j) : 64 * (j0 + j)] : 0;
#pragma unroll
        for (int j = 0; j < U; ++j) vv[j] = (j0 + j < np) ? v2[64 * (j0 + j)] : double2{0.0, 0.0};
#pragma unroll
        for (int j = 0; j < U; ++j) {
            const int lo = (int)(int16_t)(cc[j] & 0xffff), hi = (int)(int16_t)(cc[j] >> 16);
            x0[j] = (j0 + j < np) ? ldx_col<SC1>(x, base + lo, own_lo, own_hi) : 0.0;
            x1[j] = (j0 + j < np) ? ldx_col<SC1>(x, base + hi, own_lo, own_hi) : 0.0;
        }
#pragma unroll
        for (int j = 0; j < U; ++j)
            if (j0 + j < np) {
                acc += vv[j].x * x0[j];
                acc += vv[j].y * x1[j];
            }
    }
    if (w & 1) {
        const int64_t t = p0 + (int64_t)np * 128 + lane;
        const int d = UNI ? (int)ucl[w - 1] : (int)cols[t];
        acc += vals[t] * ldx_col<SC1>(x, base + d, own_lo, own_hi);
    }
    return acc;
}

template <int U, int SC1 = 0>
__device__ __forceinline__ double sell_row_pair(int64_t s, int lane, const int64_t* __restrict__ slice_ptr,
                                                const int16_t* __restrict__ cols, const double* __restrict__ vals,
                                                const double* __restrict__ x, int own_lo = 0, int own_hi = 0,
                                                const int32_t* __restrict__ uoff = nullptr,
                                                const int16_t* __restrict__ ucol = nullptr) {
    const int64_t p0 = slice_ptr[s];
    const int w = (int)((slice_ptr[s + 1] - p0) >> 6);
    const int base = (int)(s * 64 + lane);
    if (uoff) {
        const int uo = __builtin_amdgcn_readfirstlane(uoff[s]);
        if (uo >= 0) return sell_row_pair_body<U, SC1, true>(p0, w, base, lane, cols, ucol + uo, vals, x, own_lo, own_hi);
    }
    return sell_row_pair_body<U, SC1, false>(p0, w, base, lane, cols, nullptr, vals, x, own_lo, own_hi);
}

}
```

### cuda-powered-mesh-handling-and-iterative-solvers_amd/system.py

```python
from __future__ import annotations

import ctypes
import os
from dataclasses import dataclass

import torch

from . import _capi as C

I32, I64, F64 = torch.int32, torch.int64, torch.float64


def _scoped(cls):
    import functools

    def wrap(fn):
        @functools.wraps(fn)
        def w(self, *args, **kwargs):
            dev = getattr(self, "device", None)
            if dev is None:
                a0 = args[0] if args else None
                dev = getattr(a0, "device", None) or getattr(getattr(a0, "cols", None), "device", None)
            if dev is None or not torch.cuda.is_available():
                return fn(self, *args, **kwargs)
# ... 937 lines not shown
        d = self.diag()
        w = torch.empty_like(d)
        C.check(C.lib().fem_jacobi_from_diag(C.ptr(d), self.n, C.ptr(fixed_mask), C.ptr(w), C.stream(self.device)),
                "fem_jacobi_from_diag")
        return w

    def check_singular(self):
        return None

    def create_context(self, b, x, w, mode, tol, eps, hist, hist_len, stream, h):
        lib = C.lib()
        if mode == C.MODE_CG_CONSTRAINED:
            raise ValueError("the element-chunk operator has no constrained CG (SPC / RBE2 / RBE3 projections need "
                             "the assembled matrix: SellMatrix.pcg(..., constraints=...))")
        C.check(lib.fem_pcg_create(self.n_nodes, self.bs, None, None, None, C.ptr(b), C.ptr(x), C.ptr(w), mode,
                                   float(tol), float(eps), C.ptr(hist), hist_len, stream, ctypes.byref(h)),
                "fem_pcg_create")
        rc = lib.fem_pcg_set_operator_mf(h, self.h)
        if rc != C.FEM_OK:
            lib.fem_pcg_destroy(h)
            C.check(rc, "fem_pcg_set_operator_mf")

    def pcg(self, b, x0=None, w=None, mode=C.MODE_PCG, tol=1e-8, max_iter=1000, eps=1e-30, history=False, chunk=32):
        lib = C.lib()
        b = b.to(device=self.device, dtype=F64).contiguous().view(-1)
        x = (torch.zeros(self.n, dtype=F64, device=self.device) if x0 is None
             else x0.to(device=self.device, dtype=F64).clone().contiguous().view(-1))
        w = w.to(device=self.device, dtype=F64).contiguous().view(-1)
        hist = torch.full((max(max_iter, 1),), float("nan"), dtype=F64, device=self.device) if history else None
        h = ctypes.c_void_p()
        self.create_context(b, x, w, mode, tol, eps, hist, hist.numel() if hist is not None else 0,
                            C.stream(self.device), h)
        try:
            it, stt, rz = ctypes.c_int(), ctypes.c_int(), ctypes.c_double()
            C.check(lib.fem_pcg_solve(h, int(max_iter), int(chunk), ctypes.byref(it), ctypes.byref(stt),
                                      ctypes.byref(rz)), "fem_pcg_solve")
            sc = (ctypes.c_double * 6)()
            C.check(lib.fem_pcg_scalars(h, sc), "fem_pcg_scalars")
            ran = int(lib.fem_pcg_get_schedule(h))
            _check_sync(stt.value)
        finally:
            lib.fem_pcg_destroy(h)
        if hist is not None:
            hist = hist[: min(it.value, hist.numel())]
        return PcgResult(x, it.value, stt.value, rz.value, sc[1], hist, ran)

    def close(self):
        if getattr(self, "h", None):
            C.lib().fem_mf_destroy(self.h)
            self.h = ctypes.c_void_p()

    def __del__(self):
        try:
            self.close()
        except Exception:
            pass


def _check_sync(status):
    if status == C.PCG_SYNC_TIMEOUT:
        raise RuntimeError("persistent PCG: an in-launch wait gave up (grid synchronisation timed out); "
                           "the iterate is not meaningful")


class _DistMarker:
    """Mixin marking distributed runners (they run the 3-kernel schedule)."""


@_scoped
class PcgRunner:

    def __init__(self, A: SellMatrix, b, w, x0=None, mode=C.MODE_PCG, tol=0.0, eps=1e-30, fused=False,
                 schedule=None, constraints=None, tune=None):
        self.lib = C.lib()
        self.A = A
        self.device = A.device
        self.b = b.to(device=A.device, dtype=F64).contiguous().view(-1)
        self.w = w.to(device=A.device, dtype=F64).contiguous().view(-1)
        self.x = (torch.zeros(A.n, dtype=F64, device=A.device) if x0 is None
                  else x0.to(device=A.device, dtype=F64).clone().contiguous().view(-1))
        self.stream = torch.cuda.Stream(device=A.device)
        self.stream.wait_stream(torch.cuda.current_stream(A.device))
        self.h = ctypes.c_void_p()
        if getattr(A, "is_matfree", False):
            if constraints is not None:
                raise ValueError("the element-chunk operator has no constrained CG (constraints= needs a SellMatrix)")
            if fused or (schedule is not None and int(schedule) not in (SCHED_THREE, SCHED_AUTO)):
                raise ValueError("the element-chunk operator runs the three-kernel schedule (no fused / deferred / "
                                 "persistent form)")
        self.schedule = (0 if isinstance(self, _DistMarker) or getattr(A, "is_matfree", False)
                         else _schedule(fused, schedule, A.bs))
        self.constraints = constraints
        self._mode, self._tol, self._eps = mode, float(tol), float(eps)
        self._create(isinstance(self, _DistMarker) or self.schedule == SCHED_FUSED or constraints is not None)
        if tune is not None:
            self.set_tuning(tune)

    def _create(self, plain):
        A = self.A
        if getattr(A, "is_matfree", False):
            A.create_context(self.b, self.x, self.w, self._mode, self._tol, self._eps, None, 0,
                             ctypes.c_void_p(self.stream.cuda_stream), self.h)
            self._sl = False
            self.stream.wait_stream(torch.cuda.current_stream(A.device))
            return
        C.check(self.lib.fem_pcg_create(A.g.n_nodes, A.bs, C.ptr(A.g.slice_ptr), C.ptr(A.g.cols),
                                        A.solver_vals_ptr(plain), C.ptr(self.b), C.ptr(self.x), C.ptr(self.w),
                                        self._mode, self._tol, self._eps, None, 0,
                                        ctypes.c_void_p(self.stream.cuda_stream), ctypes.byref(self.h)),
                "fem_pcg_create")
        C.check(self.lib.fem_pcg_set_schedule(self.h, self.schedule), "fem_pcg_set_schedule")
        C.check(self.lib.fem_pcg_set_entries(self.h, A.g.sell_entries), "fem_pcg_set_entries")
        A.attach_cols16(self.h)
        A.attach_layout(self.h, plain)
        self._sl = A.solver_layout and not plain
        if self.constraints is not None:
            C.check(self.lib.fem_pcg_set_constraints(self.h, *self.constraints.args()), "fem_pcg_set_constraints")
        self.stream.wait_stream(torch.cuda.current_stream(A.device))

    def set_tuning(self, flags):
        if self._sl and not (int(flags) & 2):
            self.lib.fem_pcg_destroy(self.h)
            self.h = ctypes.c_void_p()
            self._create(True)
        C.check(self.lib.fem_pcg_set_tuning(self.h, int(flags)), "fem_pcg_set_tuning")

    def finish(self):
        C.check(self.lib.fem_pcg_finish(self.h), "fem_pcg_finish")

    def start(self):
        C.check(self.lib.fem_pcg_start(self.h), "fem_pcg_start")

    def use_graph(self, k):
        C.check(self.lib.fem_pcg_use_graph(self.h, int(k)), "fem_pcg_use_graph")

    def iterate(self, k):
        C.check(self.lib.fem_pcg_iterate(self.h, int(k)), "fem_pcg_iterate")

    def poll(self):
        it, stt, rz = ctypes.c_int(), ctypes.c_int(), ctypes.c_double()
        C.check(self.lib.fem_pcg_poll(self.h, ctypes.byref(it), ctypes.byref(stt), ctypes.byref(rz)), "fem_pcg_poll")
        _check_sync(stt.value)
        return it.value, stt.value, rz.value

    def debug_window(self, L, lo, hi):
        C.check(self.lib.fem_pcg_debug_window(self.h, int(L), int(lo), int(hi)), "fem_pcg_debug_window")

    def effective_schedule(self):
        return int(self.lib.fem_pcg_get_schedule(self.h))

    def uniform_slices(self, s_begin=0, s_end=-1):
        return uniform_slices(self.lib, self.h, s_begin, s_end)

    def pipelined(self):
        on = ctypes.c_int()
        C.check(self.lib.fem_pcg_pipelined(self.h, ctypes.byref(on)), "fem_pcg_pipelined")
        return bool(on.value)

    def persist_build(self):
        sl, ov, pk = ctypes.c_int(), ctypes.c_int(), ctypes.c_int()
        C.check(self.lib.fem_pcg_persist_build(self.h, ctypes.byref(sl), ctypes.byref(ov), ctypes.byref(pk)),
                "fem_pcg_persist_build")
        return sl.value, ov.value, pk.value

    def profile(self, k, every=1):
        ms = (ctypes.c_double * 3)()
        n = (ctypes.c_int * 3)()
        C.check(self.lib.fem_pcg_profile(self.h, int(k), int(every), ms, n), "fem_pcg_profile")
        return list(ms), list(n)

    def close(self):
        if self.h:
            self.lib.fem_pcg_destroy(self.h)
            self.h = ctypes.c_void_p()

    def __del__(self):
        try:
            self.close()
        except Exception:
            pass


def newmark_constants(dt, beta=0.25, gamma=0.5, damping=(0.0, 0.0)):
    dt, beta, gamma = float(dt), float(beta), float(gamma)
    if not dt > 0.0:
        raise ValueError(f"Newmark: dt must be > 0, got {dt}")
    if not beta > 0.0 or not gamma >= 0.5:
        raise ValueError(f"Newmark: needs beta > 0 and gamma >= 1/2 (the explicit beta = 0 scheme is out of scope), "
                         f"got beta = {beta}, gamma = {gamma}")
    try:
        alpha, beta_r = (float(d) for d in damping)
    except (TypeError, ValueError):
        raise ValueError(f"Newmark: damping must be the pair (alpha, beta_R), got {damping!r}") from None
    if not alpha >= 0.0 or not beta_r >= 0.0:
        raise ValueError(f"Newmark: the Rayleigh factors must be >= 0, got alpha = {alpha}, beta_R = {beta_r}")
    a0, a1, a2 = 1.0 / (beta * dt * dt), gamma / (beta * dt), 1.0 / (beta * dt)
    a3, a4, a5 = 1.0 / (2.0 * beta) - 1.0, gamma / beta - 1.0, 0.5 * dt * (gamma / beta - 2.0)
    c = dict(dt=dt, beta=beta, gamma=gamma, alpha=alpha, beta_r=beta_r, a0=a0, a1=a1, a2=a2, a3=a3, a4=a4, a5=a5,
             cK=1.0 + a1 * beta_r, cM=a0 + a1 * alpha)
    c["coef"] = [a0, a2, a3, dt * (1.0 - gamma), dt * gamma,
                 a0 + alpha * a1, a2 + alpha * a4, a3 + alpha * a5,
                 beta_r * a1, beta_r * a4, beta_r * a5, dt]
    return c


@dataclass
class TransientResult:
    times: torch.Tensor
    iterations: list
    status: list
    steps_done: int
    rec_u: torch.Tensor = None
    rec_v: torch.Tensor = None
    rec_a: torch.Tensor = None
    energy_steps: list = None
    energies: torch.Tensor = None

    @property
    def converged(self):
        return all(s == C.PCG_CONVERGED for s in self.status)


@_scoped
class NewmarkIntegrator:

    def __init__(self, A: SellMatrix, mass, fixed_mask, dt, beta=0.25, gamma=0.5, damping=(0.0, 0.0), tol=1e-8,
                 rtol=None, max_iter=1000, schedule=None, predictor=False, chunk=32):
        self.c = newmark_constants(dt, beta, gamma, damping)
        self.form, mass = A._mass_form("NewmarkIntegrator", mass)
        if rtol is not None and not float(rtol) > 0.0:
            raise ValueError(f"NewmarkIntegrator: rtol must be > 0, got {rtol}")
        self.lib = C.lib()
        self.A, self.mass, self.device = A, mass, A.device
        self.tol, self.rtol, self.max_iter, self.chunk = float(tol), rtol, int(max_iter), int(chunk)
        self.predictor = bool(predictor)
        self.events = None
        dev, n = A.device, A.n
        self._mv = A._mass_values(self.form, mass)
        self._kv, self._la = A._held_values()
        self.Keff = A.scaled_add_mass(mass, self.c["cK"], self.c["cM"])
        fixed_mask = fixed_mask.to(device=dev, dtype=torch.uint8).contiguous().view(-1)
        if fixed_mask.numel() != n:
            raise ValueError(f"NewmarkIntegrator: fixed_mask must hold {n} values, got {fixed_mask.numel()}")
        self.fixed_mask = fixed_mask
        self.w = self.Keff.jacobi(fixed_mask)
        self.free = self.w != 0
        z = lambda *s: torch.zeros(s, dtype=F64, device=dev)
        self.b, self.x, self.u, self.v, self.a, self.Y = z(n), z(n), z(n), z(n), z(n), z(n, 2)
        self._coef = (ctypes.c_double * 12)(*self.c["coef"])
        self.t, self.step_no = 0.0, 0
        self.h = ctypes.c_void_p()
        K = self.Keff
        self.schedule = _schedule(False, schedule, K.bs)
        plain = self.schedule == SCHED_FUSED
        self._stream = C.stream(dev)
        C.check(self.lib.fem_pcg_create(K.g.n_nodes, K.bs, C.ptr(K.g.slice_ptr), C.ptr(K.g.cols),
                                        K.solver_vals_ptr(plain), C.ptr(self.b), C.ptr(self.x), C.ptr(self.w),
                                        C.MODE_PCG, self.tol, 1e-30, None, 0, self._stream, ctypes.byref(self.h)),
                "fem_pcg_create")
        C.check(self.lib.fem_pcg_set_schedule(self.h, self.schedule), "fem_pcg_set_schedule")
        C.check(self.lib.fem_pcg_set_entries(self.h, K.g.sell_entries), "fem_pcg_set_entries")
        K.attach_cols16(self.h)
        K.attach_layout(self.h, plain)

    def _vec(self, x, what):
        if x is None:
            return torch.zeros(self.A.n, dtype=F64, device=self.device)
        x = x.to(device=self.device, dtype=F64).reshape(-1)
        if x.numel() != self.A.n:
            raise ValueError(f"NewmarkIntegrator: {what} must hold {self.A.n} values, got {x.numel()}")
        return x

    def _mass_times(self, x):
        if self.form == C.MASS_DIAG:
            return self._mv * x
        bs, N = self.A.bs, self.A.g.n_nodes
        return self.mass.matvec_multi(x.view(N, bs).contiguous()).reshape(-1)

    def start(self, u0=None, v0=None, f0=None):
        A, c, free = self.A, self.c, self.free
        u0, v0, f0 = self._vec(u0, "u0") * free, self._vec(v0, "v0") * free, self._vec(f0, "f0")
        r = f0 - A.matvec(u0 + c["beta_r"] * v0)
        if c["alpha"] != 0.0:
            r = r - c["alpha"] * self._mass_times(v0)
        r = r * free
        if self.form == C.MASS_DIAG:
            a0 = torch.where(free, r / self._mv, torch.zeros_like(r))
        else:
            bs, N = A.bs, A.g.n_nodes
            fm = self.fixed_mask.view(N, bs)
            if bs > 1 and bool((fm != fm[:, :1]).any()):
                raise ValueError("NewmarkIntegrator: with the SELL mass a node is fixed in all its components or none")
            wm = self.mass.jacobi(fm[:, 0].contiguous())
            R = r.view(N, bs).contiguous()
            nrm = torch.sqrt((R * (wm[:, None] * R)).sum(0)).cpu()
            a0 = torch.zeros_like(R)
            nz = [j for j in range(bs) if float(nrm[j]) > 0.0]
            if nz:
                res = self.mass.pcg_multi(R[:, nz].contiguous(), None, w=wm, mode=C.MODE_PCG,
                                          tol=[1e-12 * float(nrm[j]) for j in nz], max_iter=10000)
                if any(s != C.PCG_CONVERGED for s in res.status):
                    raise C.FemError(f"NewmarkIntegrator: the mass solve for a_0 stopped with status {res.status}")
                a0[:, nz] = res.x
            a0 = a0.reshape(-1) * free
        self.u.copy_(u0)
        self.v.copy_(v0)
# ... 134 lines not shown
```

### include/fem355.h

```cpp
#ifndef FEM355_H
#define FEM355_H

#include <stdint.h>

#ifdef __cplusplus
extern "C" {
#endif

typedef void* fem_stream_t;

enum {
    FEM_OK = 0,
    FEM_EBADTYPE = 1,
    FEM_ESINGULAR = 2,
    FEM_EHIP = 3,
    FEM_ERCCL = 4,
    FEM_EARG = 5,
    FEM_ESTATE = 6,
};

enum {
    FEM_PCG_RUNNING = 0,
    FEM_PCG_CONVERGED = 1,
    FEM_PCG_MAXITER = 2,
// ... 35 lines not shown
                  int32_t* work, fem_stream_t stream);
int fem_incidence_checked(const int64_t* conn, int64_t M, int npe, int64_t N, int32_t* inc_ptr, int32_t* inc,
                          int32_t* work, int32_t* bad, fem_stream_t stream);

int fem_graph_count(const int64_t* conn, int npe, const int32_t* inc_ptr, const int32_t* inc, int64_t N,
                    int32_t* row_len, int32_t* overflow, fem_stream_t stream);
int fem_graph_fill(const int64_t* conn, int npe, const int32_t* inc_ptr, const int32_t* inc, int64_t N,
                   const int32_t* rowptr, int32_t* colidx, int32_t* diagpos, fem_stream_t stream);
int64_t fem_graph_tmp_len(int64_t N);
int fem_graph_count2(const int64_t* conn, int npe, const int32_t* inc_ptr, const int32_t* inc, int64_t N,
                     int32_t* row_len, int32_t* tmp, int32_t* overflow, fem_stream_t stream);
int fem_graph_fill2(const int64_t* conn, int npe, const int32_t* inc_ptr, const int32_t* inc, int64_t N,
                    const int32_t* rowptr, const int32_t* tmp, int32_t* colidx, int32_t* diagpos,
                    fem_stream_t stream);
int fem_graph_sell_fill(const int64_t* conn, int npe, const int32_t* inc_ptr, const int32_t* inc, int64_t N,
                        const int32_t* rowptr, const int32_t* tmp, const int64_t* slice_ptr, int32_t* colidx,
                        int32_t* diagpos, int32_t* cols, int16_t* dcols, int64_t* csr2sell, int32_t* overflow,
                        fem_stream_t stream);
int fem_graph_sell_fill_sl(const int64_t* conn, int npe, const int32_t* inc_ptr, const int32_t* inc, int64_t N,
                           const int32_t* rowptr, const int32_t* tmp, const int64_t* slice_ptr, int32_t* colidx,
                           int32_t* diagpos, int32_t* cols, int16_t* dcols, int G, int16_t* pcols, int16_t* ucol,
                           int32_t* uoff, int32_t* win, fem_stream_t stream);
int fem_scan_i32(const int32_t* in, int64_t n, int32_t* out, int32_t* work, fem_stream_t stream);

int fem_sell_widths(const int32_t* rowptr, int64_t nrows, int64_t* width, fem_stream_t stream);
int fem_graph_sizes(const int32_t* rowptr, const int64_t* slice_ptr, const int64_t* width, int64_t N,
                    const int32_t* bad, const int32_t* ovf, int64_t* out5, fem_stream_t stream);
int fem_sell_csr2sell(const int32_t* rowptr, int64_t nrows, const int64_t* slice_ptr, int64_t* csr2sell,
                      fem_stream_t stream);
int fem_scan_i64(const int64_t* in, int64_t n, int64_t* out, int64_t* work, fem_stream_t stream);
int fem_sell_fill(const int32_t* rowptr, const int32_t* colidx, int64_t nrows, const int64_t* slice_ptr,
                  int32_t* cols, int64_t* csr2sell, fem_stream_t stream);

int64_t fem_rcm_work_len(int64_t N);
int fem_rcm(const int32_t* rowptr, const int32_t* colidx, int64_t N, int32_t* perm, int32_t* inv, int32_t* work,
            int* levels_out, fem_stream_t stream);

int fem_assemble_from_ke(const double* Ke, const int64_t* conn, int npe, int bs, const int32_t* inc_ptr,
                         const int32_t* inc, int64_t N, const int32_t* rowptr, const int32_t* colidx,
                         const int64_t* csr2sell, const int64_t* slice_ptr, double* vals, fem_stream_t stream);
int fem_assemble_from_ke_ex(const double* Ke, const int64_t* conn, int npe, int bs, const int32_t* inc_ptr,
                            const int32_t* inc, int64_t N, const int32_t* rowptr, const int32_t* colidx,
                            const int64_t* csr2sell, const int64_t* slice_ptr, int64_t nnz, int64_t ent, int store,
                            double* vals, fem_stream_t stream);
int fem_assemble_from_ke_ex2(const double* Ke, const int64_t* conn, int npe, int bs, const int32_t* inc_ptr,
                             const int32_t* inc, int64_t N, const int32_t* rowptr, const int32_t* colidx,
                             const int64_t* csr2sell, const int64_t* slice_ptr, int64_t nnz, int64_t ent, int store,
                             int max_width, double* vals, fem_stream_t stream);
int fem_assemble_tet4(const double* coords, const int64_t* conn, double E, double nu, int bs,
                      const int32_t* inc_ptr, const int32_t* inc, int64_t N, const int32_t* rowptr,
                      const int32_t* colidx, const int64_t* csr2sell, const int64_t* slice_ptr, double* vals,
                      int64_t* bad_idx, fem_stream_t stream);
int fem_assemble_tet4_ex(const double* coords, const int64_t* conn, double E, double nu, int bs,
                         const int32_t* inc_ptr, const int32_t* inc, int64_t N, const int32_t* rowptr,
                         const int32_t* colidx, const int64_t* csr2sell, const int64_t* slice_ptr, int store,
                         double* vals, int64_t* bad_idx, fem_stream_t stream);
int fem_assemble_tet4_ex2(const double* coords, const int64_t* conn, double E, double nu, int bs,
                          const int32_t* inc_ptr, const int32_t* inc, int64_t N, const int32_t* rowptr,
                          const int32_t* colidx, const int64_t* csr2sell, const int64_t* slice_ptr, int store,
                          int max_width, double* vals, int64_t* bad_idx, fem_stream_t stream);

int fem_sell_to_csr_vals(const double* vals, int bs, const int32_t* rowptr, int64_t nrows,
                         const int64_t* csr2sell, const int64_t* slice_ptr, double* csr_vals,
                         fem_stream_t stream);

int fem_jacobi(const double* vals, int bs, const int32_t* rowptr, const int32_t* diagpos,
               const int64_t* csr2sell, const int64_t* slice_ptr, int64_t nrows, const uint8_t* mask,
               double* w, fem_stream_t stream);

int fem_sell_diag(const double* vals, int bs, const int32_t* diagpos, const int64_t* csr2sell, int64_t nrows,
                  double* diag, fem_stream_t stream);
int fem_jacobi_from_diag(const double* diag, int64_t n, const uint8_t* mask, double* w, fem_stream_t stream);

int fem_ebe_apply(const double* Ke, const int64_t* conn, int npe, int dpn, const int32_t* inc_ptr,
                  const int32_t* inc, int64_t N, const double* u, double* y, fem_stream_t stream);
int fem_ebe_diag(const double* Ke, const int64_t* conn, int npe, int dpn, const int32_t* inc_ptr,
                 const int32_t* inc, int64_t N, int colzero, double* diag, fem_stream_t stream);
int fem_invert_diag(const double* in, int64_t n, double* out, fem_stream_t stream);

int fem_tet4_stress(const double* coords, const int64_t* conn, int64_t M, const double* u, double E, double nu,
                    double* sig, double* vm, int64_t* bad_idx, fem_stream_t stream);
int fem_iso_stress(const double* coords, const int64_t* conn, int64_t M, int npe, const double* u, double E, double nu,
                   const double* dN, const double* w, int n_ip, int layout, double* sig, double* vm,
                   fem_stream_t stream);
int fem_voigt_to_tensor(const double* voigt, int64_t M, double* tensor, fem_stream_t stream);
int fem_von_mises(const double* tensor, int64_t M, double* vm, fem_stream_t stream);
int fem_node_average(const double* ev, int npe, const int32_t* inc_ptr, const int32_t* inc, int64_t N, double* out,
                     fem_stream_t stream);
int fem_face_forces(const double* normals, const double* sig, int64_t M, int F, double* out, fem_stream_t stream);
int fem_shared_face_sum(const int64_t* idx, const double* face_forces, int F, int64_t S, double* out,
                        fem_stream_t stream);

typedef struct fem_topo fem_topo;
int fem_topo_create(const int64_t* conn, int64_t M, int npe, const int32_t* ftab, int F, int fpn, int64_t N,
                    fem_stream_t stream, fem_topo** out);
int fem_topo_counts(const fem_topo* t, int64_t* n_unique, int64_t* n_single, int64_t* n_pair);
int fem_topo_pairs(fem_topo* t, int64_t* out);
int fem_topo_unique(fem_topo* t, int64_t* out);
int fem_topo_boundary(fem_topo* t, const int64_t* conn, int Fs, const int32_t* smap, const int32_t* stab,
                      const int32_t* xtab, int64_t* faces, int64_t* extra, int64_t* count);
void fem_topo_destroy(fem_topo* t);
int fem_sub_elements(const int64_t* conn, int64_t M, int npe, const int32_t* tab, int T, int spe, int64_t* out,
                     fem_stream_t stream);
int fem_element_face_normals(const double* coords, const int64_t* conn, int64_t M, int npe, const int32_t* edges,
                             const int32_t* cen, const int32_t* ncen, const int32_t* extra, int F, double scale,
                             int flip, int unit, double* out, fem_stream_t stream);
int fem_surface_normals(const double* coords, const int64_t* faces, const int64_t* extra, int64_t K, int fpn, int v2,
                        double* out, fem_stream_t stream);

typedef struct fem_vtk fem_vtk;
int fem_vtk_read(const char* path, fem_vtk** out);
int fem_vtk_sizes(const fem_vtk* v, int64_t* n_points, int64_t* n_cells, int64_t* cells_len, int64_t* n_types);
int fem_vtk_copy(const fem_vtk* v, double* points, int64_t* cells, int64_t* types);
void fem_vtk_free(fem_vtk* v);

int fem_solid_ke(int type, const double* coords, const int64_t* conn, int64_t M, double E, double nu, const double* ip,
                 const double* w, int n_ip, int single, double* Ke, fem_stream_t stream);
int fem_csr_pattern(const int64_t* conn, int64_t M, int npe, int dofs_per_node, int64_t n_nodes, int32_t* rowptr,
                    int32_t* colidx, int32_t* diagpos, int64_t* nnz_out, fem_stream_t stream);
int fem_csr_fill(const double* Ke, const int64_t* conn, int64_t M, int npe, int dpn, int64_t n_nodes,
                 const int32_t* rowptr, const int32_t* colidx, double* vals, fem_stream_t stream);
int fem_spmv_csr(const int32_t* rowptr, const int32_t* colidx, const double* vals, const double* x, double* y,
                 int64_t n, fem_stream_t stream);
int fem_pcg_csr(const int32_t* rowptr, const int32_t* colidx, const double* vals, int64_t n, const double* b,
                double* x, const double* dinv, const uint8_t* fixed_mask, double tol, int max_iter, double eps,
                int mode, int* iters_out, int* status_out, double* res_hist_out, fem_stream_t stream);

int fem_spmv(int64_t nrows, int bs, const int64_t* slice_ptr, const int32_t* cols, const double* vals,
             const double* x, double* y, fem_stream_t stream);
int fem_sell_delta16(const int32_t* cols, int64_t nrows, const int64_t* slice_ptr, int16_t* dcols, int32_t* overflow,
                     fem_stream_t stream);
int fem_spmv16(int64_t nrows, int bs, const int64_t* slice_ptr, const int16_t* dcols, const double* vals,
               const double* x, double* y, fem_stream_t stream);
int fem_stream_copy(const double* src, double* dst, int64_t n, int grid, fem_stream_t stream);
int fem_stream_read(const double* src, double* out, int64_t n, int grid, fem_stream_t stream);

typedef struct fem_pcg fem_pcg;
int fem_pcg_create(int64_t nrows, int bs, const int64_t* slice_ptr, const int32_t* cols, const double* vals,
                   const double* b, double* x, const double* w, int mode, double tol, double eps,
                   double* hist, int64_t hist_len, fem_stream_t stream, fem_pcg** out);
int fem_pcg_start(fem_pcg* s);
int fem_pcg_iterate(fem_pcg* s, int k);
int fem_pcg_poll(fem_pcg* s, int* iters, int* status, double* rz);
int fem_pcg_debug_window(fem_pcg* s, int L, int lo, int hi);
int fem_pcg_sync_site(fem_pcg* s, int* site);
int fem_pcg_scalars(fem_pcg* s, double* out6);
int fem_pcg_solve(fem_pcg* s, int max_iter, int chunk, int* iters, int* status, double* rz);
int fem_pcg_set_schedule(fem_pcg* s, int sched);
int fem_pcg_set_entries(fem_pcg* s, int64_t entries);
int fem_pcg_set_tol(fem_pcg* s, double tol);
int fem_pcg_get_schedule(fem_pcg* s);
int fem_pcg_uniform_slices(fem_pcg* s, int64_t s_begin, int64_t s_end, int64_t* uniform, int64_t* nslices,
                           int64_t* index_bytes);
int fem_sell_sl_pattern(int64_t nrows, const int64_t* slice_ptr, const int16_t* dcols, int G, int16_t* pcols,
                        int16_t* ucol, int32_t* uoff, int32_t* win, fem_stream_t stream);
int fem_assemble_tet4_sl(const double* coords, const int64_t* conn, double E, double nu, int bs,
                         const int32_t* inc_ptr, const int32_t* inc, int64_t N, const int32_t* rowptr,
                         const int32_t* colidx, const int64_t* slice_ptr, const int32_t* uoff, const int16_t* ucol,
                         int store, int max_width, double* svals, int64_t* bad_idx, fem_stream_t stream);
int fem_assemble_from_ke_sl(const double* Ke, const int64_t* conn, int npe, const int32_t* inc_ptr, const int32_t* inc,
                            int64_t N, const int32_t* rowptr, const int32_t* colidx, const int64_t* slice_ptr,
                            int store, int max_width, double* svals, fem_stream_t stream);
int fem_assemble_from_ke_sym(const double* Kp, const int64_t* conn, int npe, const int32_t* inc_ptr,
                             const int32_t* inc, int64_t N, const int32_t* rowptr, const int32_t* colidx,
                             const int64_t* slice_ptr, int store, int max_width, int layout_a, double* vals,
                             fem_stream_t stream);
int fem_assemble_from_ke_mass_sl(const double* Ke, const double* Me, const int64_t* conn, int npe,
                                 const int32_t* inc_ptr, const int32_t* inc, int64_t N, const int32_t* rowptr,
                                 const int32_t* colidx, const int64_t* slice_ptr, int store, int max_width,
                                 double* svals, double* mvals, fem_stream_t stream);
int fem_jacobi_sl(const double* svals, int bs, const int32_t* rowptr, const int32_t* diagpos,
                  const int64_t* slice_ptr, const int32_t* uoff, const int16_t* ucol, int64_t nrows,
                  const uint8_t* mask, double* w, fem_stream_t stream);
int fem_spmv_sl(int64_t nrows, int bs, const int64_t* slice_ptr, const int16_t* pcols, const double* svals,
                const int32_t* uoff, const int16_t* ucol, const double* x, double* y, fem_stream_t stream);
int fem_sell_sl_unpair(int64_t nrows, int bs, const int64_t* slice_ptr, const int16_t* dcols, const int32_t* uoff,
                       const int16_t* ucol, const int32_t* rowptr, const double* svals, double* vals,
                       fem_stream_t stream);
int fem_pcg_set_layout(fem_pcg* s, const double* svals, const int16_t* pcols, const int32_t* uoff,
                       const int16_t* ucol, const int32_t* win, int G);
int fem_pcg_persist_build(fem_pcg* s, int* slots, int* overflow, int* pack);
int fem_pcg_pipelined(fem_pcg* s, int* on);
int fem_pcg_persist_profile(fem_pcg* s, int k, unsigned long long* host_out, int* grid);
int fem_pcg_set_constraints(fem_pcg* s, int order, int64_t R, const int64_t* rbe2_slave, const int64_t* rbe2_master,
                            int64_t S, const int64_t* spc_dof, const double* spc_val, int64_t G,
                            const int64_t* r3_ptr, const int64_t* r3_master, const double* r3_wsum,
                            const int64_t* r3_slave, const double* r3_w);
int fem_enforce_constraints(double* x, double* r, int64_t n, int order, int64_t R, const int64_t* rbe2_slave,
                            const int64_t* rbe2_master, int64_t S, const int64_t* spc_dof, const double* spc_val,
                            int64_t G, const int64_t* r3_ptr, const int64_t* r3_master, const double* r3_wsum,
                            const int64_t* r3_slave, const double* r3_w, fem_stream_t stream);
enum { FEM_TUNE_REVERSE = 1, FEM_TUNE_PAIR = 2, FEM_TUNE_PK_SC1 = 4, FEM_TUNE_PK_PACK = 8, FEM_TUNE_C1F = 16,
       FEM_TUNE_PK_COOP = 32, FEM_TUNE_DIST_FINE = 64, FEM_TUNE_PK_UNI = 128, FEM_TUNE_PK_WIDE = 256,
       FEM_TUNE_DIST_DROP = 512, FEM_TUNE_UPD1 = 1024, FEM_TUNE_U2_HOLD = 2048, FEM_TUNE_U2_SMALL = 4096,
       FEM_TUNE_MF_GATHER = 8192, FEM_TUNE_PK_GV = 16384 };
int fem_pcg_set_tuning(fem_pcg* s, int flags);
int fem_pcg_set_cols16(fem_pcg* s, const int16_t* dcols);
int fem_pcg_finish(fem_pcg* s);
int fem_pcg_use_graph(fem_pcg* s, int k);
int fem_pcg_profile(fem_pcg* s, int k, int every, double* ms, int* n);
void fem_pcg_destroy(fem_pcg* s);
int fem_pcg_set_rows(fem_pcg* s, int nranks, int rank, const int64_t* slice_split, int grid);
int fem_pcg_comm_block(fem_pcg* s, void** base, int64_t* bytes);
int fem_pcg_col_window(fem_pcg* s, int64_t* lo, int64_t* hi);
int fem_pcg_set_peers(fem_pcg* s, void* const* bases, const int64_t* need_lo, const int64_t* need_hi);
int fem_pcg_dist_debug(fem_pcg* s, int which, int32_t* host_out, int64_t n);
int fem_stream_create_cu(int part, int nparts, void** stream);
int fem_stream_destroy(void* stream);
int fem_pcg_set_prof(fem_pcg* s, unsigned long long* dev_buf);
int fem_ipc_handle(void* ptr, char* out64);
int fem_ipc_open(const char* h64, void** ptr);
int fem_ipc_close(void* ptr);
int fem_pcg_release_cache(void);
int fem_release_scratch(void);

int fem_comm_unique_id(char* out128);
int fem_comm_init(int nranks, int rank, const char* id128, void** comm);
int fem_comm_destroy(void* comm);
int fem_allreduce_sum(void* comm, double* buf, int64_t n, fem_stream_t stream);
int fem_halo_pack(const double* v, int bs, const int32_t* imap, int64_t nI, double* buf, fem_stream_t stream);
int fem_halo_unpack(double* v, int bs, const int32_t* ipos, int64_t nrows, const double* buf, fem_stream_t stream);
int fem_halo_sum(void* comm, double* v, int bs, const int32_t* imap, int64_t nI, const int32_t* ipos, int64_t nrows,
                 double* buf, fem_stream_t stream);
int fem_pcg_set_dist(fem_pcg* s, int enable, void* comm, int64_t nI, const int32_t* imap, const int32_t* ipos,
                     const uint8_t* own);
int fem_pcg_set_dist_variant(fem_pcg* s, int variant);
int fem_pcg_set_p2p(fem_pcg* s, int nranks, int npeer, const int* peer_rank, const int64_t* peer_cnt,
                    const int32_t* csrc, const int32_t* ssrc);
int fem_pcg_p2p_buffers(fem_pcg* s, double** psend, double** precv, int64_t* total);
int fem_p2p_deliver(fem_pcg* const* ctx, int P, fem_stream_t stream);
int fem_pcg_dist_phase(fem_pcg* s, int phase);
int fem_pcg_dist_buffer(fem_pcg* s, int phase, double** ptr, int64_t* n);
int fem_group_allreduce(double* const* dev_ptr_array, int P, int64_t n, fem_stream_t stream);

typedef struct fem_mf fem_mf;
int fem_mf_create(const double* coords, const int64_t* conn, int64_t M, int64_t N, int kind, double E, double nu,
                  int64_t* bad_idx, fem_stream_t stream, fem_mf** out);
int fem_mf_destroy(fem_mf* m);
int fem_mf_apply(fem_mf* m, const double* x, double* y, fem_stream_t stream);
int fem_mf_diag(fem_mf* m, double* d, fem_stream_t stream);
int fem_mf_info(fem_mf* m, int64_t* out6);
int fem_mf_order(fem_mf* m, int32_t* eorder, int32_t* cptr, int32_t* sbase, int32_t* cnode, fem_stream_t stream);
int fem_pcg_set_operator_mf(fem_pcg* s, fem_mf* m);

int fem_spmm(int64_t nrows, int bs, int nv, const int64_t* slice_ptr, const int32_t* cols, const int16_t* dcols,
             const double* vals, const double* X, double* Y, fem_stream_t stream);
typedef struct fem_mpcg fem_mpcg;
int fem_mpcg_create(int64_t nrows, int bs, int nv, int nactive, const int64_t* slice_ptr, const int32_t* cols,
                    const int16_t* dcols, const double* vals, const double* B, double* X, const double* w, int mode,
                    const double* tol, double eps, double* hist, int64_t hist_len, fem_stream_t stream,
                    fem_mpcg** out);
int fem_mpcg_solve(fem_mpcg* s, int max_iter, int chunk, int* iters, int* status, double* rz);
int fem_mpcg_scalars(fem_mpcg* s, double* out);
void fem_mpcg_destroy(fem_mpcg* s);

enum fem_mass_form {
    FEM_MASS_SELL = 0,
    FEM_MASS_DIAG = 1
};
int fem_spmm_km(int64_t nrows, int bs, int nv, const int64_t* slice_ptr, const int32_t* cols, const int16_t* dcols,
                const double* vals, const double* mass, int mass_form, const double* X, double* Y, double* Z,
                fem_stream_t stream);
#define FEM_MODAL_OUT_GM 576
#define FEM_MODAL_OUT_NORMS 1152
#define FEM_MODAL_OUT_LEN 1168
int64_t fem_modal_work_len(void);
int fem_modal_gram(int64_t n, int nv, int a, const double* const* vecs, double* work, double* out,
                   fem_stream_t stream);
int fem_modal_residual(int64_t n, int nv, const double* KX, const double* MX, const double* w, const double* theta,
                       double* W, double* work, double* out, fem_stream_t stream);
int fem_modal_rotate(int64_t n, int nv, int a, double* const* vecs, const double* C, fem_stream_t stream);

int fem_sell_axpby_mass(int64_t nrows, int bs, int layout_a, int64_t entries, const int64_t* slice_ptr,
                        const int32_t* rowptr, const int32_t* diagpos, const double* kvals, const double* mass,
                        int mass_form, double cK, double cM, double* out, fem_stream_t stream);
int fem_newmark_rhs(int64_t nrows, int bs, int layout_a, const int64_t* slice_ptr, const int32_t* cols,
                    const int16_t* dcols, const double* kvals, const double* mass, int mass_form, double amp,
                    const double* F, const double* Y, double* b, fem_stream_t stream);
int fem_newmark_update(int64_t n, const double* coef, int predictor, double* x, double* u, double* v, double* a,
                       const double* w, double* Y, fem_stream_t stream);
int64_t fem_transient_work_len(void);
int fem_quadform_km(int64_t nrows, int bs, int layout_a, const int64_t* slice_ptr, const int32_t* cols,
                    const int16_t* dcols, const double* kvals, const double* mass, int mass_form, const double* X,
                    double* work, double* out, fem_stream_t stream);

#ifdef __cplusplus
}
#endif
#endif
```

Baseline: 22710 CG iterations/s.

## Split diagonal out of SELL stream in persistent PCG kernel

Builds a diagonal-free copy of the paired SELL values and uniform column indices, plus a separate per-row diagonal array that stays in registers. The persistent PCG kernel's SpMV reads the shorter off-diagonal stream, and the diagonal term comes from diag[row] times the locally held preconditioned residual, so the diagonal x gather and the register-resident u copy are no longer needed. The goal is to cut matrix bytes and gathers per iteration. In exchange it costs extra device memory for a second value array, a setup kernel, and more template instantiations. It is enabled by default through a new tuning flag.

```diff
diff --git a/cuda-powered-mesh-handling-and-iterative-solvers_amd/_capi.py b/cuda-powered-mesh-handling-and-iterative-solvers_amd/_capi.py
--- a/cuda-powered-mesh-handling-and-iterative-solvers_amd/_capi.py
+++ b/cuda-powered-mesh-handling-and-iterative-solvers_amd/_capi.py
@@ -20,7 +20,8 @@
 TUNE_U2_HOLD, TUNE_U2_SMALL = 2048, 4096
 TUNE_MF_GATHER = 8192
 TUNE_PK_GV = 16384
-TUNE_DEFAULT = 1 | 2 | 4 | 8 | 128 | TUNE_UPD1
+TUNE_PK_OFFDIAG = 32768
+TUNE_DEFAULT = 1 | 2 | 4 | 8 | 128 | TUNE_UPD1 | TUNE_PK_OFFDIAG
 KIND_ELASTIC, KIND_POISSON, KIND_MASS = 0, 1, 2
 ISO_SUM, ISO_STACK, ISO_VOLUME, ISO_MASS = 0, 1, 2, 3
 MASS_SELL, MASS_DIAG = 0, 1
@@ -120,6 +121,8 @@
     "fem_pcg_set_entries": (_I, [_P, _L]),
     "fem_pcg_get_schedule": (_I, [_P]),
     "fem_pcg_uniform_slices": (_I, [_P, _L, _L, _P, _P, _P]),
+    "fem_pcg_offdiag_slices": (_I, [_P, _P, _P, _P]),
+    "fem_pcg_debug_offdiag": (_I, [_P, _P, _P]),
     "fem_pcg_persist_build": (_I, [_P, ctypes.POINTER(_I), ctypes.POINTER(_I), ctypes.POINTER(_I)]),
     "fem_pcg_pipelined": (_I, [_P, ctypes.POINTER(_I)]),
     "fem_sell_sl_pattern": (_I, [_L, _P, _P, _I, _P, _P, _P, _P, _P]),
diff --git a/cuda-powered-mesh-handling-and-iterative-solvers_amd/csrc/pcg.hip b/cuda-powered-mesh-handling-and-iterative-solvers_amd/csrc/pcg.hip
--- a/cuda-powered-mesh-handling-and-iterative-solvers_amd/csrc/pcg.hip
+++ b/cuda-powered-mesh-handling-and-iterative-solvers_amd/csrc/pcg.hip
@@ -1738,6 +1738,11 @@
     unsigned* pk_sync;
     int pk_ovf;
     double* pk_v;
+    int pk_od;
+    double* pk_ovals;
+    int16_t* pk_oucol;
+    int32_t* pk_kd;
+    double* pk_diag;
     int pk_coop;
     int pk_gv;
     double* gv_buf;
@@ -2848,7 +2853,8 @@
         return FEM_EARG;
     }
     fem_pcg* s = new fem_pcg();
-    s->tune = FEM_TUNE_REVERSE | FEM_TUNE_PAIR | FEM_TUNE_PK_SC1 | FEM_TUNE_PK_PACK | FEM_TUNE_PK_UNI | FEM_TUNE_UPD1;
+    s->tune = FEM_TUNE_REVERSE | FEM_TUNE_PAIR | FEM_TUNE_PK_SC1 | FEM_TUNE_PK_PACK | FEM_TUNE_PK_UNI | FEM_TUNE_UPD1 |
+              FEM_TUNE_PK_OFFDIAG;
     s->nrows = nrows;
     s->bs = bs;
     s->nslices = cdiv(nrows, 64);
@@ -3139,7 +3145,19 @@
     return (int)((maxL + PK_WAVES - 1) / PK_WAVES);
 }
 
-static const void* persist_fn(bool prof, bool gsc1, bool ovf = false, int small = 0) {
+static const void* persist_fn(bool prof, bool gsc1, bool ovf = false, int small = 0, bool od = false) {
+    if (od) {
+        if (small >= 1 && small <= 4 && !prof && !ovf && gsc1)
+            return small == 1 ? (const void*)k_pcg_persist<1, false, true, false, false, true>
+                 : small == 2 ? (const void*)k_pcg_persist<2, false, true, false, false, true>
+                              : (const void*)k_pcg_persist<4, false, true, false, false, true>;
+        if (ovf) return gsc1 ? (const void*)k_pcg_persist<PK_MAXS, false, true, true, false, true>
+                             : (const void*)k_pcg_persist<PK_MAXS, false, false, true, false, true>;
+        if (prof) return gsc1 ? (const void*)k_pcg_persist<PK_MAXS, true, true, false, false, true>
+                              : (const void*)k_pcg_persist<PK_MAXS, true, false, false, false, true>;
+        return gsc1 ? (const void*)k_pcg_persist<PK_MAXS, false, true, false, false, true>
+                    : (const void*)k_pcg_persist<PK_MAXS, false, false, false, false, true>;
+    }
     if (small >= 1 && small <= 4 && !prof && !ovf && gsc1)
         return small == 1 ? (const void*)k_pcg_persist<1, false, true>
              : small == 2 ? (const void*)k_pcg_persist<2, false, true>
@@ -3159,8 +3177,75 @@
 
 static int persist_setup_dist(fem_pcg* s);
 
+static int offdiag_build(fem_pcg* s) {
+    s->pk_od = 0;
+    if (!(s->tune & FEM_TUNE_PK_OFFDIAG) || !s->persist || s->bs != 1 || s->pd || s->pk_gv ||
+        !(s->tune & FEM_TUNE_PK_UNI) || !s->puoff || !s->pucol)
+        return FEM_OK;
+    if (!s->pk_ovals) {
+        int64_t ent = s->sell_ent;
+        if (ent < 0) {
+            FEM_HIP(hipMemcpyAsync(&ent, s->slice_ptr + s->nslices, sizeof(int64_t), hipMemcpyDeviceToHost, s->stream));
+            FEM_HIP(hipStreamSynchronize(s->stream));
+        }
+        FEM_HIP(pool_alloc((void**)&s->pk_ovals, sizeof(double) * (size_t)(ent > 0 ? ent : 1), s->stream, true));
+        FEM_HIP(pool_alloc((void**)&s->pk_oucol, sizeof(int16_t) * (size_t)(2 * (ent / 64) + 2), s->stream, true));
+        FEM_HIP(pool_alloc((void**)&s->pk_kd, sizeof(int32_t) * (size_t)s->nslices, s->stream, true));
+        FEM_HIP(pool_alloc((void**)&s->pk_diag, sizeof(double) * (size_t)s->n, s->stream, true));
+    }
+    hipLaunchKernelGGL(k_sell_offdiag, dim3((unsigned)cdiv(s->nslices, 4)), dim3(256), 0, s->stream, s->nslices,
+                       s->nrows, s->slice_ptr, s->pvals, s->puoff, s->pucol, s->pk_ovals, s->pk_oucol, s->pk_kd,
+                       s->pk_diag);
+    FEM_LAUNCHED();
+    s->pk_od = 1;
+    return FEM_OK;
+}
+
+int fem_pcg_offdiag_slices(fem_pcg* s, int64_t* od_slices, int64_t* nslices, int64_t* bytes) {
+    *od_slices = 0;
+    *nslices = s->nslices;
+    *bytes = 0;
+    if (!s->persist || !s->pk_od || s->nslices == 0) return FEM_OK;
+    std::vector<int32_t> h((size_t)s->nslices);
+    FEM_HIP(hipMemcpyAsync(h.data(), s->pk_kd, sizeof(int32_t) * h.size(), hipMemcpyDeviceToHost, s->stream));
+    FEM_HIP(hipStreamSynchronize(s->stream));
+    int64_t c = 0;
+    if (s->pk_ovf) {
+        const int G = s->pk_grid;
+        const int64_t maxL = (s->nslices + G - 1) / G;
+        const int64_t m = (maxL + PK_WAVES - 1) / PK_WAVES;
+        for (int L = 0; L < G; ++L) {
+            const int64_t sL0 = (int64_t)L * s->nslices / G, nL = (int64_t)(L + 1) * s->nslices / G - sL0;
+            for (int wv = 0; wv < PK_WAVES; ++wv) {
+                const int64_t lo = std::min<int64_t>(wv * m, nL);
+                const int64_t nreg = std::min<int64_t>(std::min<int64_t>(nL - lo, m), PK_MAXS);
+                for (int64_t j = 0; j < nreg; ++j) c += h[(size_t)(sL0 + lo + j)] >= 0;
+            }
+        }
+    } else {
+        for (int32_t k : h) c += k >= 0;
+    }
+    *od_slices = c;
+    *bytes = c * 64 * (int64_t)sizeof(double);
+    return FEM_OK;
+}
+
+int fem_pcg_debug_offdiag(fem_pcg* s, const int32_t* rowptr, double* vals) {
+    if (!s->persist || !s->pk_od || !s->cols16) {
+        set_error("fem_pcg_debug_offdiag: the started context reads no diagonal-free stream");
+        return FEM_EARG;
+    }
+    hipLaunchKernelGGL(k_sell_od_unpair, dim3(stream_grid(s->nslices * 64, 256)), dim3(256), 0, s->stream, s->nslices,
+                       s->slice_ptr, s->cols16, s->puoff, s->pucol, s->pk_kd, s->pk_diag, rowptr, s->nrows,
+                       s->pk_ovals, vals);
+    FEM_LAUNCHED();
+    FEM_HIP(hipStreamSynchronize(s->stream));
+    return FEM_OK;
+}
+
 static int persist_setup(fem_pcg* s) {
     s->persist = 0;
+    s->pk_od = 0;
     if (s->pd) return persist_setup_dist(s);
     if (!s->persist_req) return FEM_OK;
     if ((s->bs != 1 && s->bs != 3) || !s->paired || s->dist || s->mode == FEM_MODE_CG_CONSTRAINED || s->nslices == 0)
@@ -3180,10 +3265,12 @@
         int& slot = occ_cache[s->bs == 3][dev & 63];
         if (slot == 0) {
             int res = 1;
-            for (int v = 0; v < (s->bs == 3 ? 2 : 9) && res == 1; ++v) {
+            for (int vv = 0; vv < (s->bs == 3 ? 2 : 18) && res == 1; ++vv) {
+                const int v = vv % 9;
+                const bool od = vv >= 9;
                 const void* f = s->bs == 3 ? persist3_fn(v == 1, false)
-                              : v >= 6 ? persist_fn(false, true, false, v == 8 ? 4 : v - 5)
-                                       : persist_fn((v & 1) && v < 4, v & 2, v >= 4);
+                              : v >= 6 ? persist_fn(false, true, false, v == 8 ? 4 : v - 5, od)
+                                       : persist_fn((v & 1) && v < 4, v & 2, v >= 4, 0, od);
                 FEM_HIP(hipFuncSetAttribute(f, hipFuncAttributeMaxDynamicSharedMemorySize, (int)persist_lds(s)));
                 int nb = 0;
                 FEM_HIP(hipOccupancyMaxActiveBlocksPerMultiprocessor(&nb, f, PK_T, persist_lds(s)));
@@ -3245,7 +3332,7 @@
             s->pk_gv = slot == 1;
         }
     }
-    return FEM_OK;
+    return offdiag_build(s);
 }
 
 static int persist_setup_dist(fem_pcg* s) {
@@ -3347,6 +3434,15 @@
     a.pub = nullptr;
     a.b = s->b;
     a.init = 0;
+    a.diag = nullptr;
+    a.vals_full = a.vals;
+    a.ucol_full = a.ucol;
+    const bool od = s->pk_od && s->bs == 1 && !s->pd && !s->pk_gv;
+    if (od) {
+        a.vals = s->pk_ovals;
+        a.ucol = s->pk_oucol;
+        a.diag = s->pk_diag;
+    }
     if (s->pd) {
         const int64_t S0 = s->pd_split[s->pd_rank], S1 = s->pd_split[s->pd_rank + 1];
         a.nslices = S1 - S0;
@@ -3423,7 +3519,7 @@
     const void* fn = s->bs == 3 ? persist3_fn(s->pk_ovf != 0, s->pd != 0)
                    : s->pd ? persist_fn_dist(prof != nullptr, a.pack)
                            : persist_fn(prof != nullptr && !s->pk_ovf, (s->tune & FEM_TUNE_PK_SC1) != 0, s->pk_ovf != 0,
-                                        (a.pack <= 4 && !(s->tune & FEM_TUNE_PK_WIDE)) ? a.pack : 0);
+                                        (a.pack <= 4 && !(s->tune & FEM_TUNE_PK_WIDE)) ? a.pack : 0, od);
     if (s->pk_coop || (s->tune & FEM_TUNE_PK_COOP))
         FEM_HIP(hipLaunchCooperativeKernel(fn, dim3(G), dim3(PK_T), args, persist_lds(s), s->stream));
     else
@@ -4351,6 +4447,10 @@
     pool_free(s->pk_part, s->stream);
     pool_free(s->pk_sync, s->stream);
     pool_free(s->pk_v, s->stream);
+    pool_free(s->pk_ovals, s->stream);
+    pool_free(s->pk_oucol, s->stream);
+    pool_free(s->pk_kd, s->stream);
+    pool_free(s->pk_diag, s->stream);
     pool_free(s->gv_buf, s->stream);
     pool_free(s->u2_sync, s->stream);
     pool_free(s->st, s->stream);
diff --git a/cuda-powered-mesh-handling-and-iterative-solvers_amd/csrc/pcg_persist.hpp b/cuda-powered-mesh-handling-and-iterative-solvers_amd/csrc/pcg_persist.hpp
--- a/cuda-powered-mesh-handling-and-iterative-solvers_amd/csrc/pcg_persist.hpp
+++ b/cuda-powered-mesh-handling-and-iterative-solvers_amd/csrc/pcg_persist.hpp
@@ -146,7 +146,16 @@
     const int32_t* pub;
     const double* b;
     int init;
+    const double* diag;
+    const double* vals_full;
+    const int16_t* ucol_full;
 };
+
+__device__ __forceinline__ double pk_mul_rn(double a, double b) {
+    double m = a * b;
+    asm("" : "+v"(m));
+    return m;
+}
 
 __device__ __forceinline__ bool pk_barrier_dist(const PkArgs& a, unsigned* sy, int grp, unsigned nper, unsigned e,
                                                 int* lds_ok, const double* pd, const double* pg, int G, double* out,
@@ -244,9 +253,10 @@
 
 #define PK_ON(j) ((j) < nreg && lane < nrows - (s0 + (j)) * 64)
 
-template <int MAXS, bool PROF, bool GSC1, bool OVF = false, bool DIST = false>
+template <int MAXS, bool PROF, bool GSC1, bool OVF = false, bool DIST = false, bool OD = false>
 __global__ void __launch_bounds__(PK_T) k_pcg_persist(PkArgs a) {
     static_assert(!DIST || (GSC1 && !OVF), "distributed persistent PCG: sc1 gathers, no overflow build");
+    static_assert(!(DIST && OD), "distributed persistent PCG: no diagonal-free stream");
     unsigned long long pacc[PROF ? PK_NPROF : 1] = {};
     unsigned long long pt = 0, wspmv = 0;
     if constexpr (PROF) pt = __builtin_amdgcn_s_memtime();
@@ -312,7 +322,10 @@
     unsigned ebase = st->pk_epoch;
     unsigned elast = ebase;
 
-    double rr[MAXS], pp[MAXS], ss[MAXS], vv[MAXS], uo[MAXS];
+    double rr[MAXS], pp[MAXS], ss[MAXS], vv[MAXS];
+    double uo[OD ? 1 : MAXS];
+    double dg[OD ? MAXS : 1];
+#define PK_UO(j) (OD ? pk_mul_rn(wl[(j) * 64], rr[j]) : uo[OD ? 0 : (j)])
 #pragma unroll
     for (int j = 0; j < MAXS; ++j) {
         const unsigned row = rb + 64u * j;
@@ -325,7 +338,8 @@
         if (j < PK_VL) vl[j * 64] = 0.0;
         const double wj = on ? a.w[row] : 0.0;
         wl[j * 64] = wj;
-        uo[j] = wj * rr[j];
+        if constexpr (OD) dg[j] = on ? a.diag[row] : 0.0;
+        else uo[j] = wj * rr[j];
     }
     const int nflags = (DIST ? a.nranks : 1) * G;
     const int wraw0 = a.win[L], wraw1 = a.win[G + L];
@@ -358,7 +372,7 @@
                     ss[j] = 0.0;
                     xl[j * 64] = on ? a.x[row] : 0.0;
                     const double ui = wj * rv;
-                    uo[j] = ui;
+                    if constexpr (!OD) uo[j] = ui;
                     gp += rv * ui;
                     if (on) {
                         __hip_atomic_store(a.u + row, ui, __ATOMIC_RELAXED, __HIP_MEMORY_SCOPE_AGENT);
@@ -453,11 +467,15 @@
             const double* uvp = pk_launder(a.u);
             const int32_t* uop = a.uoff ? pk_launder(a.uoff) : nullptr;
             const int16_t* ucp = a.uoff ? pk_launder(a.ucol) : nullptr;
+#define PK_ROW(MODE, j)                                                                                             \
+    (OD ? sell_row_pair_od<pk_u<MAXS, PROF>(), (MODE) == 3 ? 1 : (MODE)>(s0 + (j), lane, slp, cop, vap, uvp, uop, ucp,      \
+                                       [&](double acc) { return acc + dg[OD ? (j) : 0] * PK_UO(j); })              \
+        : sell_row_pair<pk_u<MAXS, PROF>(), MODE>(s0 + (j), lane, slp, cop, vap, uvp, olo, ohi, uop, ucp))
 #define PK_SPMV(MODE)                                                                              \
     if (!rv) {                                                                                     \
         _Pragma("unroll") for (int j = 0; j < MAXS; ++j) {                                         \
             if (j < nreg) {                                                                        \
-                const double v = sell_row_pair<pk_u<MAXS, PROF>(), MODE>(s0 + j, lane, slp, cop, vap, uvp, olo, ohi, uop, ucp); \
+                const double v = PK_ROW(MODE, j);                                                  \
                 if (j < PK_VL) vl[j * 64] = v; else vv[j] = v;                                     \
             }                                                                                      \
             asm volatile("" ::: "memory");                                                         \
@@ -466,7 +484,7 @@
         _Pragma("unroll") for (int jj = 0; jj < MAXS; ++jj) {                                      \
             const int j = MAXS - 1 - jj;                                                           \
             if (j < nreg) {                                                                        \
-                const double v = sell_row_pair<pk_u<MAXS, PROF>(), MODE>(s0 + j, lane, slp, cop, vap, uvp, olo, ohi, uop, ucp); \
+                const double v = PK_ROW(MODE, j);                                                  \
                 if (j < PK_VL) vl[j * 64] = v; else vv[j] = v;                                     \
             }                                                                                      \
             asm volatile("" ::: "memory");                                                         \
@@ -478,18 +496,20 @@
                 PK_SPMV((GSC1 ? 1 : 0))
             }
 #undef PK_SPMV
+#undef PK_ROW
             if constexpr (PROF) {
                 asm volatile("s_waitcnt vmcnt(0) lgkmcnt(0)" ::: "memory");
                 wspmv += __builtin_amdgcn_s_memtime() - tw0;
             }
             double dp = 0.0;
 #pragma unroll
-            for (int j = 0; j < MAXS; ++j) dp += uo[j] * (j < PK_VL ? vl[j * 64] : vv[j]);
+            for (int j = 0; j < MAXS; ++j) dp += PK_UO(j) * (j < PK_VL ? vl[j * 64] : vv[j]);
             if constexpr (OVF) {
                 __builtin_amdgcn_sched_barrier(0);
                 for (int q = 0; q < nov; ++q) {
                     const int sq = s0 + MAXS + q;
-                    const double v = sell_row_pair<pk_u<MAXS, PROF>(), GSC1>(sq, lane, slp, cop, vap, uvp, 0, 0, uop, ucp);
+                    const double v = sell_row_pair<pk_u<MAXS, PROF>(), GSC1>(sq, lane, slp, cop, OD ? a.vals_full : vap, uvp, 0, 0,
+                                                                             uop, OD ? a.ucol_full : ucp);
                     const int row = sq * 64 + lane;
                     if (row < nrows) {
                         a.v[row] = v;
@@ -568,7 +588,7 @@
 #pragma unroll
             for (int j = 0; j < MAXS; ++j) {
                 if (j < nreg) {
-                    const double pi = uo[j] + bnew * pp[j];
+                    const double pi = PK_UO(j) + bnew * pp[j];
                     const double si = (j < PK_VL ? vl[j * 64] : vv[j]) + bnew * ss[j];
                     pp[j] = pi;
                     ss[j] = si;
@@ -578,7 +598,7 @@
                     if (cg && wi == 0.0) ri = 0.0;
                     rr[j] = ri;
                     const double ui = wi * ri;
-                    uo[j] = ui;
+                    if constexpr (!OD) uo[j] = ui;
                     if (PK_ON(j)) {
                         __hip_atomic_store(ust + (rbi + 64u * j), ui, __ATOMIC_RELAXED, __HIP_MEMORY_SCOPE_AGENT);
                         if constexpr (DIST) {
@@ -701,6 +721,7 @@
 }
 #undef PK_ON
 #undef PK_MARK
+#undef PK_UO
 
 __global__ void k_pk_window_init(int G, int lo_empty, int* __restrict__ win) {
     const int i = blockIdx.x * blockDim.x + threadIdx.x;
diff --git a/cuda-powered-mesh-handling-and-iterative-solvers_amd/csrc/sell_pair.hpp b/cuda-powered-mesh-handling-and-iterative-solvers_amd/csrc/sell_pair.hpp
--- a/cuda-powered-mesh-handling-and-iterative-solvers_amd/csrc/sell_pair.hpp
+++ b/cuda-powered-mesh-handling-and-iterative-solvers_amd/csrc/sell_pair.hpp
@@ -335,6 +335,145 @@
     return acc;
 }
 
+__attribute__((unused)) static __global__ void __launch_bounds__(256) k_sell_offdiag(int64_t nslices, int64_t nrows,
+                                                             const int64_t* __restrict__ slice_ptr,
+                                                             const double* __restrict__ pvals,
+                                                             const int32_t* __restrict__ uoff,
+                                                             const int16_t* __restrict__ ucol,
+                                                             double* __restrict__ ovals, int16_t* __restrict__ oucol,
+                                                             int32_t* __restrict__ kd, double* __restrict__ diag) {
+    const int64_t s = ((int64_t)blockIdx.x * blockDim.x + threadIdx.x) >> 6;
+    const int l = threadIdx.x & 63;
+    if (s >= nslices) return;
+    const int64_t p0 = slice_ptr[s];
+    const int w = (int)((slice_ptr[s + 1] - p0) >> 6);
+    const int uo = uoff[s];
+    const int64_t row = s * 64 + l;
+    int kdv = -1;
+    if (uo >= 0) {
+        const unsigned long long z = __ballot(l < w && ucol[uo + l] == 0);
+        if (z) kdv = __builtin_ctzll(z);
+    }
+    if (l == 0) {
+        kd[s] = kdv;
+        if (uo >= 0) oucol[uo + 2 * w - 1] = (int16_t)kdv;
+    }
+    if (kdv < 0) {
+        for (int k = 0; k < w; ++k) ovals[p0 + 64 * k + l] = pvals[p0 + 64 * k + l];
+        if (uo >= 0)
+            for (int k = l; k < w; k += 64) oucol[uo + k] = ucol[uo + k];
+        if (row < nrows) diag[row] = 0.0;
+        return;
+    }
+    diag[row] = pvals[p0 + pair_pos(kdv, w, l)];
+    const int w1 = w - 1, np1 = w1 >> 1;
+    double2* o2 = reinterpret_cast<double2*>(ovals + p0) + l;
+    for (int j = 0; j < np1; ++j) {
+        const int k0 = 2 * j + (2 * j >= kdv), k1 = 2 * j + 1 + (2 * j + 1 >= kdv);
+        o2[64 * j] = double2{pvals[p0 + pair_pos(k0, w, l)], pvals[p0 + pair_pos(k1, w, l)]};
+    }
+    if (w1 & 1) ovals[p0 + (int64_t)np1 * 128 + l] = pvals[p0 + pair_pos(w1 - 1 + (w1 - 1 >= kdv), w, l)];
+    for (int k = l; k < w1; k += 64) oucol[uo + k] = ucol[uo + k + (k >= kdv)];
+}
+
+__attribute__((unused)) static __global__ void __launch_bounds__(256) k_sell_od_unpair(int64_t nslices,
+                                                               const int64_t* __restrict__ slice_ptr,
+                                                               const int16_t* __restrict__ cin,
+                                                               const int32_t* __restrict__ uoff,
+                                                               const int16_t* __restrict__ ucol,
+                                                               const int32_t* __restrict__ kd,
+                                                               const double* __restrict__ diag,
+                                                               const int32_t* __restrict__ rowptr, int64_t nrows,
+                                                               const double* __restrict__ ovals,
+                                                               double* __restrict__ vout) {
+    for (int64_t t = (int64_t)blockIdx.x * blockDim.x + threadIdx.x; t < nslices * 64;
+         t += (int64_t)gridDim.x * blockDim.x) {
+        const int64_t s = t >> 6;
+        const int l = (int)(t & 63);
+        const int64_t p0 = slice_ptr[s];
+        const int w = (int)((slice_ptr[s + 1] - p0) >> 6);
+        const int64_t row = s * 64 + l;
+        const int len = row < nrows ? rowptr[row + 1] - rowptr[row] : 0;
+        const int uo = uoff[s];
+        const int kdv = kd[s];
+        int u = 0;
+        for (int k = 0; k < w; ++k) {
+            double v = 0.0;
+            if (k < len) {
+                int pos = k;
+                if (uo >= 0) {
+                    const int d = cin[p0 + 64 * k + l];
+                    while (u < w && (int)ucol[uo + u] < d) ++u;
+                    pos = u++;
+                }
+                if (kdv < 0) v = ovals[p0 + pair_pos(pos, w, l)];
+                else if (pos == kdv) v = diag[row];
+                else v = ovals[p0 + pair_pos(pos - (pos > kdv), w - 1, l)];
+            }
+            vout[p0 + 64 * k + l] = v;
+        }
+    }
+}
+
+template <int U, int SC1, class Diag>
+__device__ __forceinline__ double sell_row_pair_od_body(int64_t p0, int w1, int base, int lane,
+                                                        const int16_t* __restrict__ ucl,
+                                                        const double* __restrict__ vals, const double* __restrict__ x,
+                                                        int own_lo, int own_hi, int kd, const Diag& diag) {
+    const int np = w1 >> 1;
+    const double2* v2 = reinterpret_cast<const double2*>(vals + p0) + lane;
+    const int32_t* c2 = reinterpret_cast<const int32_t*>(ucl);
+    double acc = 0.0;
+    for (int j0 = 0; j0 < np; j0 += U) {
+        int32_t cc[U];
+        double2 vv[U];
+        double x0[U], x1[U];
+#pragma unroll
+        for (int j = 0; j < U; ++j) cc[j] = (j0 + j < np) ? c2[j0 + j] : 0;
+#pragma unroll
+        for (int j = 0; j < U; ++j) vv[j] = (j0 + j < np) ? v2[64 * (j0 + j)] : double2{0.0, 0.0};
+#pragma unroll
+        for (int j = 0; j < U; ++j) {
+            const int lo = (int)(int16_t)(cc[j] & 0xffff), hi = (int)(int16_t)(cc[j] >> 16);
+            x0[j] = (j0 + j < np) ? ldx_col<SC1>(x, base + lo, own_lo, own_hi) : 0.0;
+            x1[j] = (j0 + j < np) ? ldx_col<SC1>(x, base + hi, own_lo, own_hi) : 0.0;
+        }
+#pragma unroll
+        for (int j = 0; j < U; ++j)
+            if (j0 + j < np) {
+                const int k = 2 * (j0 + j);
+                if (k == kd) acc = diag(acc);
+                acc += vv[j].x * x0[j];
+                if (k + 1 == kd) acc = diag(acc);
+                acc += vv[j].y * x1[j];
+            }
+    }
+    if (w1 & 1) {
+        const int64_t t = p0 + (int64_t)np * 128 + lane;
+        const double xt = ldx_col<SC1>(x, base + (int)ucl[w1 - 1], own_lo, own_hi);
+        if (kd == w1 - 1) acc = diag(acc);
+        acc += vals[t] * xt;
+    }
+    if (kd == w1) acc = diag(acc);
+    return acc;
+}
+
+template <int U, int SC1, class Diag>
+__device__ __forceinline__ double sell_row_pair_od(int64_t s, int lane, const int64_t* __restrict__ slice_ptr,
+                                                   const int16_t* __restrict__ cols, const double* __restrict__ vals,
+                                                   const double* __restrict__ x, const int32_t* __restrict__ uoff,
+                                                   const int16_t* __restrict__ ucol, const Diag& diag) {
+    const int64_t p0 = slice_ptr[s];
+    const int w = (int)((slice_ptr[s + 1] - p0) >> 6);
+    const int base = (int)(s * 64 + lane);
+    const int uo = __builtin_amdgcn_readfirstlane(uoff[s]);
+    if (uo >= 0) {
+        const int kdv = __builtin_amdgcn_readfirstlane((int)ucol[uo + 2 * w - 1]);
+        return sell_row_pair_od_body<U, SC1>(p0, w - (kdv >= 0), base, lane, ucol + uo, vals, x, 0, 0, kdv, diag);
+    }
+    return sell_row_pair_body<U, SC1, false>(p0, w, base, lane, cols, nullptr, vals, x, 0, 0);
+}
+
 template <int U, int SC1 = 0>
 __device__ __forceinline__ double sell_row_pair(int64_t s, int lane, const int64_t* __restrict__ slice_ptr,
                                                 const int16_t* __restrict__ cols, const double* __restrict__ vals,
diff --git a/cuda-powered-mesh-handling-and-iterative-solvers_amd/system.py b/cuda-powered-mesh-handling-and-iterative-solvers_amd/system.py
--- a/cuda-powered-mesh-handling-and-iterative-solvers_amd/system.py
+++ b/cuda-powered-mesh-handling-and-iterative-solvers_amd/system.py
@@ -1113,6 +1113,18 @@
     def uniform_slices(self, s_begin=0, s_end=-1):
         return uniform_slices(self.lib, self.h, s_begin, s_end)
 
+    def offdiag_slices(self):
+        c, n, nb = ctypes.c_int64(), ctypes.c_int64(), ctypes.c_int64()
+        C.check(self.lib.fem_pcg_offdiag_slices(self.h, ctypes.byref(c), ctypes.byref(n), ctypes.byref(nb)),
+                "fem_pcg_offdiag_slices")
+        return c.value, n.value, nb.value
+
+    def debug_offdiag_values(self):
+        A = self.A
+        out = torch.empty(max(A.g.sell_entries, 1), dtype=F64, device=A.device)
+        C.check(self.lib.fem_pcg_debug_offdiag(self.h, C.ptr(A.g.rowptr), C.ptr(out)), "fem_pcg_debug_offdiag")
+        return out
+
     def pipelined(self):
         on = ctypes.c_int()
         C.check(self.lib.fem_pcg_pipelined(self.h, ctypes.byref(on)), "fem_pcg_pipelined")
diff --git a/include/fem355.h b/include/fem355.h
--- a/include/fem355.h
+++ b/include/fem355.h
@@ -211,6 +211,8 @@
 int fem_pcg_get_schedule(fem_pcg* s);
 int fem_pcg_uniform_slices(fem_pcg* s, int64_t s_begin, int64_t s_end, int64_t* uniform, int64_t* nslices,
                            int64_t* index_bytes);
+int fem_pcg_offdiag_slices(fem_pcg* s, int64_t* od_slices, int64_t* nslices, int64_t* bytes);
+int fem_pcg_debug_offdiag(fem_pcg* s, const int32_t* rowptr, double* vals);
 int fem_sell_sl_pattern(int64_t nrows, const int64_t* slice_ptr, const int16_t* dcols, int G, int16_t* pcols,
                         int16_t* ucol, int32_t* uoff, int32_t* win, fem_stream_t stream);
 int fem_assemble_tet4_sl(const double* coords, const int64_t* conn, double E, double nu, int bs,
@@ -252,7 +254,7 @@
 enum { FEM_TUNE_REVERSE = 1, FEM_TUNE_PAIR = 2, FEM_TUNE_PK_SC1 = 4, FEM_TUNE_PK_PACK = 8, FEM_TUNE_C1F = 16,
        FEM_TUNE_PK_COOP = 32, FEM_TUNE_DIST_FINE = 64, FEM_TUNE_PK_UNI = 128, FEM_TUNE_PK_WIDE = 256,
        FEM_TUNE_DIST_DROP = 512, FEM_TUNE_UPD1 = 1024, FEM_TUNE_U2_HOLD = 2048, FEM_TUNE_U2_SMALL = 4096,
-       FEM_TUNE_MF_GATHER = 8192, FEM_TUNE_PK_GV = 16384 };
+       FEM_TUNE_MF_GATHER = 8192, FEM_TUNE_PK_GV = 16384, FEM_TUNE_PK_OFFDIAG = 32768 };
 int fem_pcg_set_tuning(fem_pcg* s, int flags);
 int fem_pcg_set_cols16(fem_pcg* s, const int16_t* dcols);
 int fem_pcg_finish(fem_pcg* s);
```

New measurement: 23670 CG iterations/s (median of 6 runs). 1.04x the previous value.
